# vlongle/pixie

Hardware: AMD Instinct MI355X
Metric: voxels/s (128^3 U-Net fwd) + MPM particle-steps/s (higher is better)
Workload: dtype f32 (operands split fp16 hi+lo, 3 f16 MFMAs/product, fp32 accumulate); 1 GPU; 128^3x64 feature grid -> SegmentationUNet+RegressionUNet forward (+argmax/one-hot combine), 1 scene per GPU per step; grid=128, feature_channels=64, parallelism=scene-parallel x1, executor=c+hip_graph

## Files before the change

include/pixie_hip.h:

```cpp
#ifndef PIXIE_HIP_H
#define PIXIE_HIP_H

#include <stdint.h>

#ifdef __cplusplus
extern "C" {
#endif

const char* pixie_last_error(void);
const char* pixie_build_arch(void);

typedef struct pixie_mpm pixie_mpm;

int pixie_mpm_create(pixie_mpm** out, int n_particles, int n_grid, double grid_lim);
int pixie_mpm_destroy(pixie_mpm* h);
int pixie_mpm_regrid(pixie_mpm* h, int n_grid, double grid_lim, void* stream);

int pixie_mpm_set_field(pixie_mpm* h, const char* name, const void* d_src, int64_t count, void* stream);
int pixie_mpm_get_field(pixie_mpm* h, const char* name, void* d_dst, int64_t count, void* stream);
int pixie_mpm_fill_field(pixie_mpm* h, const char* name, double value, void* stream);

int pixie_mpm_set_scalar(pixie_mpm* h, const char* key, double value);
int pixie_mpm_get_scalar(pixie_mpm* h, const char* key, double* value);

int pixie_mpm_update_mass(pixie_mpm* h, void* stream);
int pixie_mpm_finalize_mu_lam(pixie_mpm* h, int with_bulk, void* stream);
int pixie_mpm_apply_additional_params(pixie_mpm* h, const double point[3], const double size[3], double E,
                                      double nu, double density, int material, void* stream);
int pixie_mpm_apply_additional_params_batch(pixie_mpm* h, int64_t n_boxes, const float* d_boxes, const float* d_params,
                                            const int32_t* d_material, void* stream);

enum { PIXIE_BC_SURFACE = 0, PIXIE_BC_CUBOID = 1, PIXIE_BC_BBOX = 2 };
typedef struct pixie_bc_desc {
    int32_t type;
    int32_t surface_type;
    int32_t reset;
    int32_t pad_;
    double point[3], size[3], velocity[3], normal[3];
    double start_time, end_time, friction;
} pixie_bc_desc;
int pixie_mpm_add_bc(pixie_mpm* h, const pixie_bc_desc* bc);

enum { PIXIE_PM_IMPULSE = 0, PIXIE_PM_TRANSLATION = 1, PIXIE_PM_ROTATION = 2 };
typedef struct pixie_pmod_desc {
    int32_t type;
    int32_t pad_;
    double point[3], size[3];
    double force[3];
    double velocity[3];
    double normal[3], h1[3], h2[3];
    double half_height, radius, rotation_scale, translation_scale;
    double start_time, end_time;
} pixie_pmod_desc;
int pixie_mpm_add_particle_modifier(pixie_mpm* h, const pixie_pmod_desc* pm, void* stream);

int pixie_mpm_step(pixie_mpm* h, double dt, int n_substeps, void* stream);

typedef struct pixie_mpm_batch pixie_mpm_batch;
typedef struct pixie_batch_sched {
    double dt;
    int32_t steps_per_chunk;
    int32_t n_chunks;
    int32_t n_out;
    int32_t pad_;
    double shift[3], scale, mean[3];
    double inv_rotation[9];
    float* d_pos;
    float* d_cov;
} pixie_batch_sched;
int pixie_mpm_batch_create(pixie_mpm_batch** out, pixie_mpm* const* handles, int n_handles);
int pixie_mpm_batch_step(pixie_mpm_batch* b, double dt, int n_substeps, void* stream);
int pixie_mpm_batch_run(pixie_mpm_batch* b, const pixie_batch_sched* per_scene, int n_scenes, void* stream);
typedef struct pixie_batch_splat_out {
    float* d_log_scale;
    float* d_quat;
} pixie_batch_splat_out;
int pixie_mpm_batch_run_splats(pixie_mpm_batch* b, const pixie_batch_sched* per_scene, const pixie_batch_splat_out* splats ,
                               int n_scenes, void* stream);
int pixie_mpm_batch_destroy(pixie_mpm_batch* b);

int pixie_mpm_export_cov(pixie_mpm* h, float* d_cov , void* stream);
int pixie_mpm_export_R(pixie_mpm* h, float* d_R , void* stream);
int pixie_mpm_export_frame(pixie_mpm* h, int n_out, const double shift[3], double scale, const double mean[3],
                           const double inv_rotation[9], float* d_pos , float* d_cov ,
                           void* stream);
int pixie_splat_from_cov(const float* d_cov , int64_t n, float* d_log_scale , float* d_quat ,
                         void* stream);
int pixie_mpm_export_frame_splats(pixie_mpm* h, int n_out, const double shift[3], double scale, const double mean[3],
                                  const double inv_rotation[9], float* d_pos , float* d_cov ,
                                  float* d_log_scale , float* d_quat , void* stream);
int pixie_mpm_out_of_bounds(pixie_mpm* h, int64_t* count, void* stream);


typedef struct pixie_conv_desc {
    const float* d_in0; int32_t c0;
    const float* d_in1; int32_t c1;
    int32_t in_d, in_h, in_w;
    int32_t upsample;
    int32_t stride;
    int32_t ksize;
    const float* d_pro_a; const float* d_pro_b;
    const float* d_gamma; const float* d_beta;
    int32_t act;
    const float* d_w; const float* d_bias;
    int32_t c_out;
    const float* d_residual;
    float* d_out;
    const void* d_w16;
    const uint32_t* d_in_amax0; const uint32_t* d_in_amax1;
    float in_bound;
    float* d_out_stats;
    uint32_t* d_out_amax;
    void* d_workspace;
    int32_t out_d, out_h, out_w;
    const float* d_skip_in0; int32_t skip_c0;
    const float* d_skip_in1; int32_t skip_c1;
    const void* d_skip_w16; const float* d_skip_bias;
    const uint32_t* d_skip_amax0; const uint32_t* d_skip_amax1;
} pixie_conv_desc;

int pixie_conv_cout_padded(int c_out);
int pixie_conv_pack_weights(const float* d_w_oidhw, float* d_w_packed, int c_out, int c_in, int ksize, void* stream);
int64_t pixie_conv_packed16_bytes(int c_out, int c_in, int ksize);
int pixie_conv_pack_weights_f16x2(const float* d_w_oidhw, void* d_packed, int c_out, int c_in, int ksize, void* stream);
int pixie_conv3d_forward(const pixie_conv_desc* desc, void* stream);
int64_t pixie_conv_stats_floats(const pixie_conv_desc* desc);
int64_t pixie_conv_workspace_bytes(const pixie_conv_desc* desc);
int pixie_stats_finalize(const float* d_stats, const pixie_conv_desc* desc, double* d_sums, void* stream);
int pixie_conv_skip_foldable(const pixie_conv_desc* desc);

int pixie_channel_sums(const float* d_x, int channels, int64_t spatial, double* d_sums, void* stream);
int pixie_channel_stats(const float* d_x, int channels, int64_t spatial, double* d_sums, uint32_t* d_amax, void* stream);
int pixie_tensor_amax(const float* d_x, int64_t count, uint32_t* d_slot, void* stream);
int pixie_norm_finalize(const double* d_sums, int channels, int64_t spatial, int mode, int groups, double eps,
                        const float* d_weight, const float* d_bias, float* d_a, float* d_b, void* stream);

int pixie_attention_forward(const float* d_qkv, float* d_out, int channels, int tokens, void* stream);

int pixie_channel_affine(const float* d_x, const float* d_a, const float* d_b, float* d_y, int channels,
                         int64_t spatial, void* stream);

int pixie_voxel_grid_to_ncdhw(const void* d_feat_dhwc_f16, int d, int h, int w, int channels, float* d_out_cdhw, void* stream);

int pixie_projector_conv0(const void* d_feat_dhwc_f16, int64_t voxels, int channels, int n_networks, const void* const* d_w16,
                          const float* const* d_bias, float* const* d_out, int c_out, void* stream);

int pixie_pack_fields(const float* d_cont, const int32_t* d_seg_pred, int64_t n_scenes, int64_t spatial, void* d_wire, int64_t wire_bytes,
                      void* stream);

int pixie_combine_predictions(const float* d_logits, int num_classes, const float* d_cont, int64_t spatial,
                              float* d_combined, int32_t* d_argmax , void* stream);

int pixie_combine_class_ids(const int32_t* d_seg_pred, int num_classes, const float* d_cont, int64_t spatial, float* d_combined,
                            void* stream);

typedef struct pixie_unet pixie_unet;
typedef struct pixie_unet_config {
    int32_t feature_channels, cond_dim, model_channels, num_res_blocks;
    int32_t n_channel_mult; int32_t channel_mult[8];
    int32_t n_attention_resolutions; int32_t attention_resolutions[8];
    int32_t grid_size;
    int32_t out_channels;
    int32_t precision;
} pixie_unet_config;

int pixie_unet_create(pixie_unet** out, const pixie_unet_config* cfg);
int pixie_unet_destroy(pixie_unet* h);
int pixie_unet_param_count(const pixie_unet* h);
int pixie_unet_param_info(const pixie_unet* h, int index, const char** key, int64_t* numel, int32_t* ndim, int64_t shape[5]);
int pixie_unet_set_param(pixie_unet* h, const char* key, const float* d_values, int64_t numel);
int64_t pixie_unet_workspace_bytes(pixie_unet* h, int d, int hh, int w);
int pixie_unet_forward(pixie_unet* h, const float* d_feat, const float* d_proj0, int d, int hh, int w, float* d_out,
                       void* d_workspace, int64_t workspace_bytes, void* stream);
int pixie_unet_set_option(pixie_unet* h, const char* key, int value);

typedef struct pixie_field_desc {
    const float* d_pred;
    const uint8_t* d_mask;
    const float* d_axis_x; const float* d_axis_y; const float* d_axis_z;
    int32_t n_classes, d, h, w;
    double min_spacing;
    double density_min, density_max, E_min, E_max, nu_min, nu_max;
} pixie_field_desc;
int pixie_field_to_particles(const pixie_field_desc* field, const float* d_pos, int n, int k, double nn_distance_threshold,
                             int weighted, int default_material, int default_part_label, float* d_density, float* d_E,
                             float* d_nu, int32_t* d_material, int32_t* d_part_label, float* d_conf, float* d_nearest,
                             void* d_scratch, void* stream);

int pixie_unscale_prediction(const float* d_pred, int channels, int64_t spatial, double density_min, double density_max,
                             double E_min, double E_max, double nu_min, double nu_max, float* d_out, void* stream);
int64_t pixie_field_points_scratch_bytes(const pixie_field_desc* field);
int pixie_field_points(const pixie_field_desc* field, int64_t capacity, float* d_xyz , float* d_density, float* d_E,
                       float* d_nu, int32_t* d_material, float* d_conf, int64_t* d_count, void* d_scratch, void* stream);

int pixie_dbscan_roots(const float* d_pos_sorted, const int32_t* d_orig_index, const int32_t* d_cell_start, int n, int nx, int ny, int nz,
                       const double lo[3], double cell_size, double eps, int min_samples, int32_t* d_core_scratch,
                       int32_t* d_parent_scratch, int32_t* d_root, void* stream);

int pixie_fill_densify(const float* d_pos, const float* d_opacity, const float* d_cov6, int n, int grid_n, double grid_dx,
                       int32_t* d_grid_count, float* d_grid_density, void* stream);
int pixie_fill_dense_cells(int32_t* d_grid_count, const float* d_grid_density, int grid_n, double grid_dx, double density_thres,
                           int max_particles_per_cell, float* d_new_particles , int64_t max_samples,
                           uint64_t* d_counter, uint32_t seed, void* stream);
int pixie_fill_internal_cells(int32_t* d_grid_count, const float* d_grid_density, int grid_n, double grid_dx, int max_particles_per_cell,
                              int exclude_dir, int ray_cast_dir, double threshold, float* d_new_particles, int64_t max_samples,
                              uint64_t* d_counter, uint32_t seed, void* stream);
int pixie_particle_volume(const float* d_pos, int n, int grid_n, double grid_dx, int32_t* d_grid_count_scratch, float* d_vol, void* stream);
int pixie_nearest_particle(const float* d_pos, int n, const float* d_new_pos, int n_new, int32_t* d_nearest, void* stream);

#ifdef PIXIE_DIAG
int pixie_mpm_phase(pixie_mpm* h, int phase, double dt, void* stream);

int pixie_mpm_kernel_times(pixie_mpm* h, double* particle_ms, double* grid_ms, int64_t* n_launches);

int pixie_conv_kernel_variant(const pixie_conv_desc* desc, int* slices);
#endif

#ifdef __cplusplus
}
#endif
#endif
```

pixie_amd/_lib.py:

```python
from __future__ import annotations

import ctypes as C
import os

_HERE = os.path.dirname(os.path.abspath(__file__))
LIB_PATH = os.path.join(_HERE, "libpixie_hip.so")
DIAG_LIB_PATH = os.path.join(_HERE, "libpixie_hip_diag.so")


class PixieHipError(RuntimeError):
    pass


class BCDesc(C.Structure):
    _fields_ = [("type", C.c_int32), ("surface_type", C.c_int32), ("reset", C.c_int32), ("pad_", C.c_int32),
                ("point", C.c_double * 3), ("size", C.c_double * 3), ("velocity", C.c_double * 3),
                ("normal", C.c_double * 3), ("start_time", C.c_double), ("end_time", C.c_double),
                ("friction", C.c_double)]


class PModDesc(C.Structure):
    _fields_ = [("type", C.c_int32), ("pad_", C.c_int32),
                ("point", C.c_double * 3), ("size", C.c_double * 3), ("force", C.c_double * 3),
                ("velocity", C.c_double * 3), ("normal", C.c_double * 3), ("h1", C.c_double * 3),
                ("h2", C.c_double * 3), ("half_height", C.c_double), ("radius", C.c_double),
                ("rotation_scale", C.c_double), ("translation_scale", C.c_double),
                ("start_time", C.c_double), ("end_time", C.c_double)]


class ConvDesc(C.Structure):
    _fields_ = [("d_in0", C.c_void_p), ("c0", C.c_int32),
                ("d_in1", C.c_void_p), ("c1", C.c_int32),
                ("in_d", C.c_int32), ("in_h", C.c_int32), ("in_w", C.c_int32),
                ("upsample", C.c_int32), ("stride", C.c_int32), ("ksize", C.c_int32),
                ("d_pro_a", C.c_void_p), ("d_pro_b", C.c_void_p),
                ("d_gamma", C.c_void_p), ("d_beta", C.c_void_p),
                ("act", C.c_int32),
                ("d_w", C.c_void_p), ("d_bias", C.c_void_p),
                ("c_out", C.c_int32),
                ("d_residual", C.c_void_p), ("d_out", C.c_void_p),
                ("d_w16", C.c_void_p), ("d_in_amax0", C.c_void_p), ("d_in_amax1", C.c_void_p),
                ("in_bound", C.c_float),
                ("d_out_stats", C.c_void_p), ("d_out_amax", C.c_void_p),
                ("d_workspace", C.c_void_p),
                ("out_d", C.c_int32), ("out_h", C.c_int32), ("out_w", C.c_int32),
                ("d_skip_in0", C.c_void_p), ("skip_c0", C.c_int32),
                ("d_skip_in1", C.c_void_p), ("skip_c1", C.c_int32),
                ("d_skip_w16", C.c_void_p), ("d_skip_bias", C.c_void_p),
                ("d_skip_amax0", C.c_void_p), ("d_skip_amax1", C.c_void_p)]


class UNetConfigC(C.Structure):
    _fields_ = [("feature_channels", C.c_int32), ("cond_dim", C.c_int32), ("model_channels", C.c_int32), ("num_res_blocks", C.c_int32),
                ("n_channel_mult", C.c_int32), ("channel_mult", C.c_int32 * 8),
                ("n_attention_resolutions", C.c_int32), ("attention_resolutions", C.c_int32 * 8),
                ("grid_size", C.c_int32), ("out_channels", C.c_int32), ("precision", C.c_int32)]


class BatchSched(C.Structure):
    _fields_ = [("dt", C.c_double), ("steps_per_chunk", C.c_int32), ("n_chunks", C.c_int32), ("n_out", C.c_int32), ("pad_", C.c_int32),
                ("shift", C.c_double * 3), ("scale", C.c_double), ("mean", C.c_double * 3), ("inv_rotation", C.c_double * 9),
                ("d_pos", C.c_void_p), ("d_cov", C.c_void_p)]


class BatchSplatOut(C.Structure):
    _fields_ = [("d_log_scale", C.c_void_p), ("d_quat", C.c_void_p)]


class FieldDesc(C.Structure):
    _fields_ = [("d_pred", C.c_void_p), ("d_mask", C.c_void_p),
                ("d_axis_x", C.c_void_p), ("d_axis_y", C.c_void_p), ("d_axis_z", C.c_void_p),
                ("n_classes", C.c_int32), ("d", C.c_int32), ("h", C.c_int32), ("w", C.c_int32),
                ("min_spacing", C.c_double),
                ("density_min", C.c_double), ("density_max", C.c_double), ("E_min", C.c_double), ("E_max", C.c_double),
                ("nu_min", C.c_double), ("nu_max", C.c_double)]


_VP, _I, _I64, _D, _S = C.c_void_p, C.c_int, C.c_int64, C.c_double, C.c_char_p
_D3 = C.POINTER(C.c_double)
SIGNATURES = {
    "pixie_last_error": (C.c_char_p, []),
    "pixie_build_arch": (C.c_char_p, []),
    "pixie_mpm_create": (_I, [C.POINTER(_VP), _I, _I, _D]),
    "pixie_mpm_destroy": (_I, [_VP]),
    "pixie_mpm_regrid": (_I, [_VP, _I, _D, _VP]),
    "pixie_mpm_set_field": (_I, [_VP, _S, _VP, _I64, _VP]),
    "pixie_mpm_get_field": (_I, [_VP, _S, _VP, _I64, _VP]),
    "pixie_mpm_fill_field": (_I, [_VP, _S, _D, _VP]),
    "pixie_mpm_set_scalar": (_I, [_VP, _S, _D]),
    "pixie_mpm_get_scalar": (_I, [_VP, _S, C.POINTER(_D)]),
    "pixie_mpm_update_mass": (_I, [_VP, _VP]),
    "pixie_mpm_finalize_mu_lam": (_I, [_VP, _I, _VP]),
    "pixie_mpm_apply_additional_params": (_I, [_VP, _D3, _D3, _D, _D, _D, _I, _VP]),
    "pixie_mpm_apply_additional_params_batch": (_I, [_VP, _I64, _VP, _VP, _VP, _VP]),
    "pixie_mpm_add_bc": (_I, [_VP, C.POINTER(BCDesc)]),
    "pixie_mpm_add_particle_modifier": (_I, [_VP, C.POINTER(PModDesc), _VP]),
    "pixie_mpm_step": (_I, [_VP, _D, _I, _VP]),
    "pixie_mpm_export_cov": (_I, [_VP, _VP, _VP]),
    "pixie_mpm_export_R": (_I, [_VP, _VP, _VP]),
    "pixie_mpm_export_frame": (_I, [_VP, _I, _D3, _D, _D3, C.POINTER(C.c_double), _VP, _VP, _VP]),
    "pixie_mpm_out_of_bounds": (_I, [_VP, C.POINTER(_I64), _VP]),
    "pixie_mpm_batch_create": (_I, [C.POINTER(_VP), C.POINTER(_VP), _I]),
    "pixie_mpm_batch_step": (_I, [_VP, _D, _I, _VP]),
    "pixie_mpm_batch_run": (_I, [_VP, C.POINTER(BatchSched), _I, _VP]),
    "pixie_mpm_batch_run_splats": (_I, [_VP, C.POINTER(BatchSched), C.POINTER(BatchSplatOut), _I, _VP]),
    "pixie_splat_from_cov": (_I, [_VP, _I64, _VP, _VP, _VP]),
    "pixie_mpm_export_frame_splats": (_I, [_VP, _I, _D3, _D, _D3, C.POINTER(C.c_double), _VP, _VP, _VP, _VP, _VP]),
    "pixie_mpm_batch_destroy": (_I, [_VP]),
    "pixie_pack_fields": (_I, [_VP, _VP, _I64, _I64, _VP, _I64, _VP]),
    "pixie_conv_cout_padded": (_I, [_I]),
    "pixie_conv_pack_weights": (_I, [_VP, _VP, _I, _I, _I, _VP]),
    "pixie_conv_packed16_bytes": (_I64, [_I, _I, _I]),
    "pixie_conv_pack_weights_f16x2": (_I, [_VP, _VP, _I, _I, _I, _VP]),
    "pixie_conv3d_forward": (_I, [C.POINTER(ConvDesc), _VP]),
    "pixie_conv_stats_floats": (_I64, [C.POINTER(ConvDesc)]),
    "pixie_conv_workspace_bytes": (_I64, [C.POINTER(ConvDesc)]),
    "pixie_stats_finalize": (_I, [_VP, C.POINTER(ConvDesc), _VP, _VP]),
    "pixie_channel_stats": (_I, [_VP, _I, _I64, _VP, _VP, _VP]),
    "pixie_tensor_amax": (_I, [_VP, _I64, _VP, _VP]),
    "pixie_channel_sums": (_I, [_VP, _I, _I64, _VP, _VP]),
    "pixie_norm_finalize": (_I, [_VP, _I, _I64, _I, _I, _D, _VP, _VP, _VP, _VP, _VP]),
    "pixie_attention_forward": (_I, [_VP, _VP, _I, _I, _VP]),
    "pixie_channel_affine": (_I, [_VP, _VP, _VP, _VP, _I, _I64, _VP]),
    "pixie_projector_conv0": (_I, [_VP, _I64, _I, _I, C.POINTER(_VP), C.POINTER(_VP), C.POINTER(_VP), _I, _VP]),
    "pixie_conv_skip_foldable": (_I, [C.POINTER(ConvDesc)]),
    "pixie_unet_create": (_I, [C.POINTER(_VP), C.POINTER(UNetConfigC)]),
    "pixie_unet_destroy": (_I, [_VP]),
    "pixie_unet_param_count": (_I, [_VP]),
    "pixie_unet_param_info": (_I, [_VP, _I, C.POINTER(_S), C.POINTER(_I64), C.POINTER(C.c_int32), C.POINTER(_I64)]),
    "pixie_unet_set_param": (_I, [_VP, _S, _VP, _I64]),
    "pixie_unet_workspace_bytes": (_I64, [_VP, _I, _I, _I]),
    "pixie_unet_set_option": (_I, [_VP, _S, _I]),
    "pixie_unet_forward": (_I, [_VP, _VP, _VP, _I, _I, _I, _VP, _VP, _I64, _VP]),
    "pixie_combine_class_ids": (_I, [_VP, _I, _VP, _I64, _VP, _VP]),
    "pixie_combine_predictions": (_I, [_VP, _I, _VP, _I64, _VP, _VP, _VP]),
    "pixie_voxel_grid_to_ncdhw": (_I, [_VP, _I, _I, _I, _I, _VP, _VP]),
    "pixie_unscale_prediction": (_I, [_VP, _I, _I64, _D, _D, _D, _D, _D, _D, _VP, _VP]),
    "pixie_field_points_scratch_bytes": (_I64, [C.POINTER(FieldDesc)]),
    "pixie_field_points": (_I, [C.POINTER(FieldDesc), _I64, _VP, _VP, _VP, _VP, _VP, _VP, _VP, _VP, _VP]),
    "pixie_fill_densify": (_I, [_VP, _VP, _VP, _I, _I, _D, _VP, _VP, _VP]),
    "pixie_fill_dense_cells": (_I, [_VP, _VP, _I, _D, _D, _I, _VP, _I64, _VP, C.c_uint32, _VP]),
    "pixie_fill_internal_cells": (_I, [_VP, _VP, _I, _D, _I, _I, _I, _D, _VP, _I64, _VP, C.c_uint32, _VP]),
    "pixie_particle_volume": (_I, [_VP, _I, _I, _D, _VP, _VP, _VP]),
    "pixie_nearest_particle": (_I, [_VP, _I, _VP, _I, _VP, _VP]),
    "pixie_dbscan_roots": (_I, [_VP, _VP, _VP, _I, _I, _I, _I, C.POINTER(_D), _D, _D, _I, _VP, _VP, _VP, _VP]),
    "pixie_field_to_particles": (_I, [C.POINTER(FieldDesc), _VP, _I, _I, _D, _I, _I, _I, _VP, _VP, _VP, _VP, _VP, _VP, _VP, _VP, _VP]),
}

DIAG_SIGNATURES = {
    "pixie_mpm_phase": (_I, [_VP, _I, _D, _VP]),
    "pixie_mpm_kernel_times": (_I, [_VP, C.POINTER(_D), C.POINTER(_D), C.POINTER(_I64)]),
    "pixie_conv_kernel_variant": (C.c_int, [C.POINTER(ConvDesc), C.POINTER(C.c_int)]),
}

_libs = {}


def load(diag: bool = False):
    if diag in _libs:
        return _libs[diag]
    path = DIAG_LIB_PATH if diag else LIB_PATH
    if not os.path.exists(path):
        raise PixieHipError(
            f"{path} not found: build it with `python -m pixie_amd.build` (hipcc, gfx950). "
            "pixie_amd has no CPU fallback.")
    import torch
    lib = C.CDLL(path)
    for name, (res, args) in list(SIGNATURES.items()) + (list(DIAG_SIGNATURES.items()) if diag else []):
        fn = getattr(lib, name)
        fn.restype = res
        fn.argtypes = args
    _libs[diag] = lib
    return lib


def check(rc: int, what: str = "", lib=None):
    if rc != 0:
        msg = (lib or load()).pixie_last_error()
        raise PixieHipError(f"{what}: {msg.decode() if msg else 'unknown error'}")


def current_stream_ptr():
    import torch
    try:
        return C.c_void_p(torch._C._cuda_getCurrentRawStream(torch.cuda.current_device()))
    except AttributeError:
        return C.c_void_p(torch.cuda.current_stream().cuda_stream)


def d3(v):
    return (C.c_double * 3)(*[float(x) for x in v])
```

pixie_amd/csrc/conv3d_f16x3.hip:

```cpp
#include <hip/hip_runtime.h>

#include <cstdlib>
#include <map>
#include <string>
#include <type_traits>

#include "../../include/pixie_hip.h"
#include "common.h"

namespace pixie {

typedef float f32x16 __attribute__((ext_vector_type(16)));
typedef _Float16 f16x8 __attribute__((ext_vector_type(8)));

constexpr int kW16HeaderU4 = 4;

struct Conv16Args {
    const float* in0; const float* in1;
    int c0, cin;
    int ID, IH, IW;
    int LD, LH, LW;
    int ups;
    int stride;
    int OD, OH, OW;
    const float* pro_a; const float* pro_b; const float* gamma; const float* beta;
    int act;
    const uint4* w16;
    const float* wf;
    const float* bias;
    int cout, coutp;
    const float* residual; float* out;
    const unsigned* amax0; const unsigned* amax1;
    float in_bound;
    int TX, TY, TZ, lTX, lTY;
    int tiles_x, tiles_y, tiles_z, n_tiles;
    int HX, HY, HZ, HYX, CS;
    unsigned mHX, mHYX;
    float* stats; unsigned* out_amax;
    float* partial; int chunks_per_slice;
    int epi_lds;
    const float* sk_in0; const float* sk_in1;
    int sk_c0, sk_cin;
    const uint4* sk_w16; const float* sk_bias;
    const unsigned* sk_amax0; const unsigned* sk_amax1;
};

__device__ __forceinline__ int fast_div16(int n, int d, unsigned magic) {
    return (d == 1) ? n : (int)__umulhi((unsigned)n, magic);
}
__device__ __forceinline__ float act16(float t, int act) {
    if (act == 1) return t > 0.0f ? t : 0.02f * t;
    if (act == 2) return t / (1.0f + __expf(-t));
    return t;
}
__device__ __forceinline__ int scale_exponent(float bound) {
    const unsigned bits = __float_as_uint(bound);
    const int eb = (int)((bits >> 23) & 0xffu) - 127;
    if (!(bound > 0.0f) || eb > 100) return 0;
    int e = 14 - eb;
    return e > 100 ? 100 : (e < -100 ? -100 : e);
}
__device__ __forceinline__ float pow2i(int e) { return __uint_as_float((unsigned)(e + 127) << 23); }

template <int KS, int MB, int NB, bool EX = false>
__device__ __forceinline__ void conv3d_f16x3_body(const Conv16Args& A) {
    extern __shared__ uint4 smem16[];
    constexpr int PAD = (KS == 3) ? 1 : 0;
    constexpr int NW = 4, NT = 64 * NW;
    const int bufsz = 4 * A.CS;

    const int tid = threadIdx.x;
    const int lane = tid & 63;
    const int wave = tid >> 6;
    const int kh = lane >> 5;
    const int l31 = lane & 31;

    int t = blockIdx.x;
    {
        const int per = (A.n_tiles + 7) >> 3;
        const int cand = (t & 7) * per + (t >> 3);
        if ((A.n_tiles & 7) == 0) t = cand;
    }
    const int tx = t % A.tiles_x; t /= A.tiles_x;
    const int ty = t % A.tiles_y;
    const int tz = t / A.tiles_y;
    const int ox0 = tx * A.TX, oy0 = ty * A.TY, oz0 = tz * A.TZ;
    const int cout0 = blockIdx.y * (MB * 32);
    const int lx0 = ox0 * A.stride - PAD, ly0 = oy0 * A.stride - PAD, lz0 = oz0 * A.stride - PAD;
    const size_t ISP = (size_t)A.ID * A.IH * A.IW;
    const size_t OSP = (size_t)A.OD * A.OH * A.OW;

    int voff[NB];
    int ovox[NB];
    bool valid[NB];
#pragma unroll
    for (int nb = 0; nb < NB; ++nb) {
        const int j = (wave * NB + nb) * 32 + l31;
        int x = j & (A.TX - 1);
        int y = (j >> A.lTX) & (A.TY - 1);
        int z = j >> (A.lTX + A.lTY);
        const bool v = (z < A.TZ) && (ox0 + x < A.OW) && (oy0 + y < A.OH) && (oz0 + z < A.OD);
        if (!v) { x = 0; y = 0; z = 0; }
        voff[nb] = ((z * A.HY + y) * A.HX + x) * A.stride + kh * A.CS;
        ovox[nb] = ((oz0 + z) * A.OH + (oy0 + y)) * A.OW + ox0 + x;
        valid[nb] = v;
    }

    float bound = A.in_bound;
    if (A.amax0) {
        bound = __uint_as_float(*A.amax0);
        if (A.amax1) bound = fmaxf(bound, __uint_as_float(*A.amax1));
    }
    const int ex = EX ? 0 : scale_exponent(bound);
    const float sx = pow2i(ex);

    f32x16 acc[MB][NB];
#pragma unroll
    for (int mb = 0; mb < MB; ++mb)
#pragma unroll
        for (int nb = 0; nb < NB; ++nb)
#pragma unroll
            for (int r = 0; r < 16; ++r) acc[mb][nb][r] = 0.0f;

    const int KG = A.cin >> 3;
    const size_t tap_stride = (size_t)KG * A.coutp;
    const size_t plane = (size_t)(KS * KS * KS) * tap_stride;
    const uint4* wHi = A.w16 + kW16HeaderU4 + (size_t)kh * A.coutp + cout0 + l31;
    const uint4* wLo = wHi + plane;
    const float* wF = A.wf + (size_t)kh * A.coutp + cout0 + l31;

    constexpr int TAPS = KS * KS * KS;
    auto stage_chunk = [&](int c_base, uint4* buf, int stid, int nthr) {
        uint4* bHi = buf;
        uint4* bLo = buf + 2 * A.CS;
        float pa[16], pb[16];
        {
            float pv = 0.0f;
            if (A.pro_a) pv = (lane & 16) ? A.pro_b[c_base + (lane & 15)] : A.pro_a[c_base + (lane & 15)];
#pragma unroll
            for (int j = 0; j < 16; ++j) {
                pa[j] = __int_as_float(__builtin_amdgcn_readlane(__float_as_int(pv), j));
                pb[j] = __int_as_float(__builtin_amdgcn_readlane(__float_as_int(pv), 16 + j));
            }
        }
        const bool has_aff = A.gamma != nullptr;
        for (int v0 = stid; v0 < A.CS; v0 += 2 * nthr) {
            float val[2][16];
            float gm[2], bt[2];
            int sidx[2];
            bool ok[2];
#pragma unroll
            for (int u = 0; u < 2; ++u) {
                const int vox = v0 + u * nthr;
                int rem = vox;
                const int hz = fast_div16(rem, A.HYX, A.mHYX);
                rem -= hz * A.HYX;
                const int hy = fast_div16(rem, A.HX, A.mHX);
                const int hx = rem - hy * A.HX;
                const int lz = lz0 + hz, ly = ly0 + hy, lx = lx0 + hx;
                ok[u] = vox < A.CS && (unsigned)lz < (unsigned)A.LD && (unsigned)ly < (unsigned)A.LH && (unsigned)lx < (unsigned)A.LW;
                sidx[u] = ok[u] ? ((lz >> A.ups) * A.IH + (ly >> A.ups)) * A.IW + (lx >> A.ups) : 0;
            }
#pragma unroll
            for (int u = 0; u < 2; ++u) {
#pragma unroll
                for (int j = 0; j < 16; ++j) {
                    const int cg = c_base + j;
                    const float* src = (cg < A.c0) ? (A.in0 + (size_t)cg * ISP) : (A.in1 + (size_t)(cg - A.c0) * ISP);
                    val[u][j] = src[sidx[u]];
                }
                gm[u] = 1.0f; bt[u] = 0.0f;
                if (has_aff) { gm[u] = A.gamma[sidx[u]]; bt[u] = A.beta[sidx[u]]; }
            }
            auto convert = [&](auto has_pro, auto act_c) {
#pragma unroll
                for (int u = 0; u < 2; ++u) {
                    const int vox = v0 + u * nthr;
                    if (EX) {
                        float* bF = reinterpret_cast<float*>(buf);
#pragma unroll
                        for (int j = 0; j < 16; ++j) {
                            float t = val[u][j];
                            if (decltype(has_pro)::value) t = t * pa[j] + pb[j];
                            t = t * gm[u] + bt[u];
                            const float sc = ok[u] ? act16(t, decltype(act_c)::value) : 0.0f;
                            if (vox < A.CS) bF[j * A.CS + vox] = sc;
                        }
                        continue;
                    }
                    f16x8 vh[2], vl[2];
#pragma unroll
                    for (int j = 0; j < 16; ++j) {
                        float t = val[u][j];
                        if (decltype(has_pro)::value) t = t * pa[j] + pb[j];
                        t = t * gm[u] + bt[u];
                        const float sc = ok[u] ? act16(t, decltype(act_c)::value) * sx : 0.0f;
                        const _Float16 h = (_Float16)sc;
                        vh[j >> 3][j & 7] = h;
                        vl[j >> 3][j & 7] = (_Float16)(sc - (float)h);
                    }
                    if (vox < A.CS) {
                        bHi[vox] = __builtin_bit_cast(uint4, vh[0]);
                        bHi[A.CS + vox] = __builtin_bit_cast(uint4, vh[1]);
                        bLo[vox] = __builtin_bit_cast(uint4, vl[0]);
                        bLo[A.CS + vox] = __builtin_bit_cast(uint4, vl[1]);
                    }
                }
            };
            using T = std::true_type; using F = std::false_type;
            if (A.pro_a) {
                if (A.act == 1) convert(T{}, std::integral_constant<int, 1>{});
                else if (A.act == 2) convert(T{}, std::integral_constant<int, 2>{});
                else convert(T{}, std::integral_constant<int, 0>{});
            } else {
                if (A.act == 1) convert(F{}, std::integral_constant<int, 1>{});
                else if (A.act == 2) convert(F{}, std::integral_constant<int, 2>{});
                else convert(F{}, std::integral_constant<int, 0>{});
            }
        }
    };
    auto mfma_chunk = [&](int c_base, const uint4* buf) {
        __builtin_amdgcn_s_setprio(3);
        if constexpr (EX) {
            const float* ldsF = reinterpret_cast<const float*>(buf);
            const size_t tapw = (size_t)A.cin * A.coutp;
            const float* wc = wF + (size_t)c_base * A.coutp;
            float a[8][MB], an[8][MB];
#pragma unroll
            for (int kp = 0; kp < 8; ++kp)
#pragma unroll
                for (int mb = 0; mb < MB; ++mb) a[kp][mb] = wc[(size_t)(2 * kp) * A.coutp + mb * 32];
#pragma unroll 1
            for (int zy = 0; zy < KS * KS; ++zy) {
                const int dz = zy / KS, dy = zy - dz * KS;
                const int rowoff = (dz * A.HY + dy) * A.HX;
#pragma unroll
                for (int dx = 0; dx < KS; ++dx) {
                    const int tap = zy * KS + dx;
                    const int nxt = (tap + 1 < TAPS) ? tap + 1 : tap;
#pragma unroll
                    for (int kp = 0; kp < 8; ++kp)
#pragma unroll
                        for (int mb = 0; mb < MB; ++mb) an[kp][mb] = wc[(size_t)nxt * tapw + (size_t)(2 * kp) * A.coutp + mb * 32];
                    __builtin_amdgcn_sched_barrier(0);
#pragma unroll
                    for (int kp = 0; kp < 8; ++kp) {
                        float b[NB];
#pragma unroll
                        for (int nb = 0; nb < NB; ++nb) b[nb] = ldsF[voff[nb] + rowoff + dx + 2 * kp * A.CS];
#pragma unroll
                        for (int mb = 0; mb < MB; ++mb)
#pragma unroll
                            for (int nb = 0; nb < NB; ++nb)
                                acc[mb][nb] = __builtin_amdgcn_mfma_f32_32x32x2f32(a[kp][mb], b[nb], acc[mb][nb], 0, 0, 0);
                    }
#pragma unroll
                    for (int kp = 0; kp < 8; ++kp)
#pragma unroll
                        for (int mb = 0; mb < MB; ++mb) a[kp][mb] = an[kp][mb];
                }
            }
            __builtin_amdgcn_s_setprio(0);
            return;
        }
        const uint4* ldsHi = buf;
        const uint4* ldsLo = buf + 2 * A.CS;
        const uint4* wh = wHi + (size_t)(c_base >> 3) * A.coutp;
        const uint4* wl = wLo + (size_t)(c_base >> 3) * A.coutp;
        f16x8 ah[MB], al[MB];
#pragma unroll
        for (int mb = 0; mb < MB; ++mb) {
            ah[mb] = __builtin_bit_cast(f16x8, wh[mb * 32]);
            al[mb] = __builtin_bit_cast(f16x8, wl[mb * 32]);
        }
#pragma unroll 1
        for (int zy = 0; zy < KS * KS; ++zy) {
            const int dz = zy / KS, dy = zy - dz * KS;
            const int rowoff = (dz * A.HY + dy) * A.HX;
#pragma unroll
            for (int dx = 0; dx < KS; ++dx) {
                const int tap = zy * KS + dx;
                const int nxt = (tap + 1 < TAPS) ? tap + 1 : tap;
                f16x8 ahn[MB], aln[MB];
#pragma unroll
                for (int mb = 0; mb < MB; ++mb) {
                    ahn[mb] = __builtin_bit_cast(f16x8, wh[(size_t)nxt * tap_stride + mb * 32]);
                    aln[mb] = __builtin_bit_cast(f16x8, wl[(size_t)nxt * tap_stride + mb * 32]);
                }
                __builtin_amdgcn_sched_barrier(0);
                f16x8 bh[NB], bl[NB];
#pragma unroll
                for (int nb = 0; nb < NB; ++nb) {
                    bh[nb] = __builtin_bit_cast(f16x8, ldsHi[voff[nb] + rowoff + dx]);
                    bl[nb] = __builtin_bit_cast(f16x8, ldsLo[voff[nb] + rowoff + dx]);
                }
#pragma unroll
                for (int mb = 0; mb < MB; ++mb)
#pragma unroll
                    for (int nb = 0; nb < NB; ++nb)
                        acc[mb][nb] = __builtin_amdgcn_mfma_f32_32x32x16_f16(al[mb], bh[nb], acc[mb][nb], 0, 0, 0);
#pragma unroll
                for (int mb = 0; mb < MB; ++mb)
#pragma unroll
                    for (int nb = 0; nb < NB; ++nb)
                        acc[mb][nb] = __builtin_amdgcn_mfma_f32_32x32x16_f16(ah[mb], bl[nb], acc[mb][nb], 0, 0, 0);
#pragma unroll
                for (int mb = 0; mb < MB; ++mb)
#pragma unroll
                    for (int nb = 0; nb < NB; ++nb)
                        acc[mb][nb] = __builtin_amdgcn_mfma_f32_32x32x16_f16(ah[mb], bh[nb], acc[mb][nb], 0, 0, 0);
#pragma unroll
                for (int mb = 0; mb < MB; ++mb) { ah[mb] = ahn[mb]; al[mb] = aln[mb]; }
            }
        }
        __builtin_amdgcn_s_setprio(0);
    };

    float inv2 = 0.0f;
    {
        const int c_begin = A.partial ? (int)blockIdx.z * A.chunks_per_slice * 16 : 0;
        const int c_end = A.partial ? min(A.cin, c_begin + A.chunks_per_slice * 16) : A.cin;
        for (int c_base = c_begin; c_base < c_end; c_base += 16) {
            __syncthreads();
            stage_chunk(c_base, smem16, tid, NT);
            __syncthreads();
            mfma_chunk(c_base, smem16);
        }
        if (!EX && A.sk_w16) {
            float sb = __uint_as_float(*A.sk_amax0);
            if (A.sk_amax1) sb = fmaxf(sb, __uint_as_float(*A.sk_amax1));
            const int ex2 = scale_exponent(sb);
            const float sx2 = pow2i(ex2);
            const float inv_main = __uint_as_float(A.w16[0].x) * pow2i(-ex);
            inv2 = __uint_as_float(A.sk_w16[0].x) * pow2i(-ex2);
            const float ratio = inv_main / inv2;
#pragma unroll
            for (int mb = 0; mb < MB; ++mb)
#pragma unroll
                for (int nb = 0; nb < NB; ++nb)
#pragma unroll
                    for (int r = 0; r < 16; ++r) acc[mb][nb][r] *= ratio;
            const int KG2 = A.sk_cin >> 3;
            const uint4* w2Hi = A.sk_w16 + kW16HeaderU4 + (size_t)kh * A.coutp + cout0 + l31;
            const uint4* w2Lo = w2Hi + (size_t)KG2 * A.coutp;
            const int centre = (KS == 3) ? (A.HY + 1) * A.HX + 1 : 0;
            const int tvox = A.TX * A.TY * A.TZ;
            for (int c2 = 0; c2 < A.sk_cin; c2 += 16) {
                f16x8 ah[MB], al[MB];
#pragma unroll
                for (int mb = 0; mb < MB; ++mb) {
                    ah[mb] = __builtin_bit_cast(f16x8, w2Hi[(size_t)(c2 >> 3) * A.coutp + mb * 32]);
                    al[mb] = __builtin_bit_cast(f16x8, w2Lo[(size_t)(c2 >> 3) * A.coutp + mb * 32]);
                }
                __syncthreads();
                uint4* bHi = smem16;
                uint4* bLo = smem16 + 2 * A.CS;
                for (int j = tid; j < tvox; j += NT) {
                    const int x = j & (A.TX - 1), y = (j >> A.lTX) & (A.TY - 1), z = j >> (A.lTX + A.lTY);
                    const bool okv = (ox0 + x < A.OW) && (oy0 + y < A.OH) && (oz0 + z < A.OD);
                    const size_t sidx = okv ? ((size_t)(oz0 + z) * A.IH + (oy0 + y)) * A.IW + ox0 + x : 0;
                    float val[16];
#pragma unroll
                    for (int q = 0; q < 16; ++q) {
                        const int cg = c2 + q;
                        const float* src = (cg < A.sk_c0) ? (A.sk_in0 + (size_t)cg * ISP) : (A.sk_in1 + (size_t)(cg - A.sk_c0) * ISP);
                        val[q] = src[sidx];
                    }
                    f16x8 vh[2], vl[2];
#pragma unroll
                    for (int q = 0; q < 16; ++q) {
                        const float sc = okv ? val[q] * sx2 : 0.0f;
                        const _Float16 hq = (_Float16)sc;
                        vh[q >> 3][q & 7] = hq;
                        vl[q >> 3][q & 7] = (_Float16)(sc - (float)hq);
                    }
                    const int slot = (z * A.HY + y) * A.HX + x + centre;
                    bHi[slot] = __builtin_bit_cast(uint4, vh[0]);
                    bHi[A.CS + slot] = __builtin_bit_cast(uint4, vh[1]);
                    bLo[slot] = __builtin_bit_cast(uint4, vl[0]);
                    bLo[A.CS + slot] = __builtin_bit_cast(uint4, vl[1]);
                }
                __syncthreads();
                f16x8 bh[NB], bl[NB];
#pragma unroll
                for (int nb = 0; nb < NB; ++nb) {
                    bh[nb] = __builtin_bit_cast(f16x8, bHi[voff[nb] + centre]);
                    bl[nb] = __builtin_bit_cast(f16x8, bLo[voff[nb] + centre]);
                }
#pragma unroll
                for (int mb = 0; mb < MB; ++mb)
#pragma unroll
                    for (int nb = 0; nb < NB; ++nb)
                        acc[mb][nb] = __builtin_amdgcn_mfma_f32_32x32x16_f16(al[mb], bh[nb], acc[mb][nb], 0, 0, 0);
#pragma unroll
                for (int mb = 0; mb < MB; ++mb)
#pragma unroll
                    for (int nb = 0; nb < NB; ++nb)
                        acc[mb][nb] = __builtin_amdgcn_mfma_f32_32x32x16_f16(ah[mb], bl[nb], acc[mb][nb], 0, 0, 0);
#pragma unroll
                for (int mb = 0; mb < MB; ++mb)
#pragma unroll
                    for (int nb = 0; nb < NB; ++nb)
                        acc[mb][nb] = __builtin_amdgcn_mfma_f32_32x32x16_f16(ah[mb], bh[nb], acc[mb][nb], 0, 0, 0);
            }
        }
    }

    const float inv = EX ? 1.0f : (A.sk_w16 ? inv2 : __uint_as_float(A.w16[0].x) * pow2i(-ex));
    if (A.partial) {
        float* dst = A.partial + (size_t)blockIdx.z * A.cout * OSP;
#pragma unroll
        for (int mb = 0; mb < MB; ++mb)
#pragma unroll
            for (int r = 0; r < 16; ++r) {
                const int co = cout0 + mb * 32 + (r & 3) + 8 * (r >> 2) + 4 * kh;
                if (co < A.cout) {
#pragma unroll
                    for (int nb = 0; nb < NB; ++nb)
                        if (valid[nb]) dst[(size_t)co * OSP + ovox[nb]] = acc[mb][nb][r] * inv;
                }
            }
        return;
    }
    float* red = reinterpret_cast<float*>(smem16);
    float wmax = 0.0f;
    const bool full = A.epi_lds && cout0 + MB * 32 <= A.cout && (A.TX & 3) == 0 && (A.OW & 3) == 0 && NW * NB * 32 <= A.TX * A.TY * A.TZ &&
                      ox0 + A.TX <= A.OW && oy0 + A.TY <= A.OH && oz0 + A.TZ <= A.OD;
    if (full) {
        __syncthreads();
        constexpr int LDO = NB * 32 + 4;
        float* ldsO = reinterpret_cast<float*>(smem16) + wave * (32 * LDO);
        red = reinterpret_cast<float*>(smem16) + NW * 32 * LDO;
        constexpr int LPR = NB * 8;
        constexpr int RPI = 32 / LPR;
        const int rsub = l31 / LPR, colq = 4 * (l31 % LPR), nbq = colq >> 5;
        const int jq = (wave * NB + nbq) * 32 + (colq & 31);
        const int xq = jq & (A.TX - 1), yq = (jq >> A.lTX) & (A.TY - 1), zq = jq >> (A.lTX + A.lTY);
        const size_t ovq = ((size_t)(oz0 + zq) * A.OH + (oy0 + yq)) * A.OW + ox0 + xq;
        const bool has_res = A.residual != nullptr, has_stats = A.stats != nullptr;
#pragma unroll
        for (int mb = 0; mb < MB; ++mb) {
#pragma unroll
            for (int r = 0; r < 16; ++r)
#pragma unroll
                for (int nb = 0; nb < NB; ++nb) ldsO[((r & 3) + 8 * (r >> 2) + 4 * kh) * LDO + nb * 32 + l31] = acc[mb][nb][r];
#pragma unroll 4
            for (int it = 0; it < 16 / RPI; ++it) {
                const int rowl = (2 * it + kh) * RPI + rsub;
                const int co = cout0 + mb * 32 + rowl;
                const float4 a4 = *reinterpret_cast<const float4*>(ldsO + rowl * LDO + colq);
                const float bv = (A.bias ? A.bias[co] : 0.0f) + (A.sk_bias ? A.sk_bias[co] : 0.0f);
                const size_t o = (size_t)co * OSP + ovq;
                float4 v4;
                v4.x = a4.x * inv + bv; v4.y = a4.y * inv + bv; v4.z = a4.z * inv + bv; v4.w = a4.w * inv + bv;
                if (has_res) {
                    const float4 r4 = *reinterpret_cast<const float4*>(A.residual + o);
                    v4.x += r4.x; v4.y += r4.y; v4.z += r4.z; v4.w += r4.w;
                }
                *reinterpret_cast<float4*>(A.out + o) = v4;
                if (has_stats) {
                    float s1 = (v4.x + v4.y) + (v4.z + v4.w);
                    float s2 = (v4.x * v4.x + v4.y * v4.y) + (v4.z * v4.z + v4.w * v4.w);
                    wmax = fmaxf(fmaxf(wmax, fmaxf(fabsf(v4.x), fabsf(v4.y))), fmaxf(fabsf(v4.z), fabsf(v4.w)));
#pragma unroll
                    for (int off = LPR / 2; off > 0; off >>= 1) { s1 += __shfl_xor(s1, off, 64); s2 += __shfl_xor(s2, off, 64); }
                    if ((l31 % LPR) == 0) { red[(wave * MB * 32 + mb * 32 + rowl) * 2] = s1; red[(wave * MB * 32 + mb * 32 + rowl) * 2 + 1] = s2; }
                }
            }
        }
    } else {
    if (A.stats) __syncthreads();
#pragma unroll
    for (int mb = 0; mb < MB; ++mb) {
#pragma unroll
        for (int r = 0; r < 16; ++r) {
            const int row = mb * 32 + (r & 3) + 8 * (r >> 2) + 4 * kh;
            const int co = cout0 + row;
            float s1 = 0.0f, s2 = 0.0f;
            if (co < A.cout) {
                const float bv = (A.bias ? A.bias[co] : 0.0f) + (A.sk_bias ? A.sk_bias[co] : 0.0f);
#pragma unroll
                for (int nb = 0; nb < NB; ++nb) {
                    if (valid[nb]) {
                        const size_t o = (size_t)co * OSP + ovox[nb];
                        float val = acc[mb][nb][r] * inv + bv;
                        if (A.residual) val += A.residual[o];
                        A.out[o] = val;
                        s1 += val; s2 += val * val; wmax = fmaxf(wmax, fabsf(val));
                    }
                }
            }
            if (A.stats) {
#pragma unroll
                for (int off = 16; off > 0; off >>= 1) { s1 += __shfl_xor(s1, off, 64); s2 += __shfl_xor(s2, off, 64); }
                if (l31 == 0) { red[(wave * MB * 32 + row) * 2] = s1; red[(wave * MB * 32 + row) * 2 + 1] = s2; }
            }
        }
    }
    }
    if (A.stats) {
        __syncthreads();
        if (tid < MB * 32 * 2) {
            float t = red[tid];
#pragma unroll
            for (int w = 1; w < NW; ++w) t += red[w * MB * 64 + tid];
            A.stats[((size_t)blockIdx.x * A.coutp + cout0) * 2 + tid] = t;
        }
        if (A.out_amax) {
#pragma unroll
            for (int off = 32; off > 0; off >>= 1) wmax = fmaxf(wmax, __shfl_xor(wmax, off, 64));
            if (lane == 0 && wmax > 0.0f) atomicMax(A.out_amax, __float_as_uint(wmax));
        }
    }
}

template <int KS, int MB, int NB>
__global__ __launch_bounds__(256, 2) void conv3d_f16x3_kernel(Conv16Args A) {
    conv3d_f16x3_body<KS, MB, NB>(A);
}
template <int KS, int MB, int NB>
__global__ __launch_bounds__(256, 2) void conv3d_exact_kernel(Conv16Args A) {
    conv3d_f16x3_body<KS, MB, NB, true>(A);
}
__global__ __launch_bounds__(256, 2) void conv3d_f16x3_c64_fullres_kernel(Conv16Args A) {
    conv3d_f16x3_body<3, 2, 4>(A);
}

__global__ __launch_bounds__(256) void stats_finalize_kernel(const float* __restrict__ stats, int n_tiles, int coutp, double* __restrict__ sums) {
    const int c = blockIdx.x;
    double s1 = 0.0, s2 = 0.0;
    for (int t = threadIdx.x; t < n_tiles; t += 256) {
        const float2 v = *reinterpret_cast<const float2*>(stats + ((size_t)t * coutp + c) * 2);
        s1 += v.x; s2 += v.y;
    }
    for (int off = 32; off > 0; off >>= 1) { s1 += __shfl_down(s1, off, 64); s2 += __shfl_down(s2, off, 64); }
    __shared__ double r[8];
    if ((threadIdx.x & 63) == 0) { r[2 * (threadIdx.x >> 6)] = s1; r[2 * (threadIdx.x >> 6) + 1] = s2; }
    __syncthreads();
    if (threadIdx.x == 0) { sums[2 * c] = r[0] + r[2] + r[4] + r[6]; sums[2 * c + 1] = r[1] + r[3] + r[5] + r[7]; }
}

__global__ __launch_bounds__(256) void splitk_reduce_kernel(const float* __restrict__ partial, int slices, long n_elems, long osp,
                                                            const float* __restrict__ bias, const float* residual, float* out) {
    const long i = (long)blockIdx.x * 256 + threadIdx.x;
    if (i >= n_elems) return;
    float v = partial[i];
    for (int s = 1; s < slices; ++s) v += partial[(size_t)s * n_elems + i];
    if (bias) v += bias[i / osp];
    if (residual) v += residual[i];
    out[i] = v;
}

__global__ __launch_bounds__(256) void amax_kernel(const float* __restrict__ x, long n, unsigned* __restrict__ slot) {
    float m = 0.0f;
    const long stride = (long)gridDim.x * 256 * 4;
    long i = ((long)blockIdx.x * 256 + threadIdx.x) * 4;
    if ((reinterpret_cast<size_t>(x) & 15) == 0) {
        for (; i + 3 < n; i += stride) {
            const float4 v = *reinterpret_cast<const float4*>(x + i);
            m = fmaxf(fmaxf(m, fabsf(v.x)), fmaxf(fabsf(v.y), fmaxf(fabsf(v.z), fabsf(v.w))));
        }
        for (long k = i; k < n && k < i + 4; ++k) m = fmaxf(m, fabsf(x[k]));
    } else {
        for (long k = (long)blockIdx.x * 256 + threadIdx.x; k < n; k += (long)gridDim.x * 256) m = fmaxf(m, fabsf(x[k]));
    }
    for (int off = 32; off > 0; off >>= 1) m = fmaxf(m, __shfl_down(m, off, 64));
    if ((threadIdx.x & 63) == 0 && m > 0.0f) atomicMax(slot, __float_as_uint(m));
}

__global__ void pack_weights_f16x2_kernel(const float* __restrict__ src, uint4* __restrict__ dst, int cout, int cin, int taps,
                                          int coutp, const unsigned* __restrict__ amax_bits) {
    const int KG = cin >> 3;
    const long total = (long)taps * KG * coutp;
    const long i = (long)blockIdx.x * blockDim.x + threadIdx.x;
    const int e = scale_exponent(__uint_as_float(*amax_bits));
    if (i == 0) dst[0] = make_uint4(__float_as_uint(pow2i(-e)), (unsigned)cout, (unsigned)cin, (unsigned)taps);
    if (i >= total) return;
    const float s = pow2i(e);
    const int co = (int)(i % coutp);
    const long row = i / coutp;
    const int kg = (int)(row % KG);
    const int tap = (int)(row / KG);
    f16x8 vh, vl;
#pragma unroll
    for (int j = 0; j < 8; ++j) {
        float w = 0.0f;
        if (co < cout) w = src[((long)co * cin + kg * 8 + j) * taps + tap] * s;
        const _Float16 h = (_Float16)w;
        vh[j] = h;
        vl[j] = (_Float16)(w - (float)h);
    }
    dst[kW16HeaderU4 + i] = __builtin_bit_cast(uint4, vh);
    dst[kW16HeaderU4 + total + i] = __builtin_bit_cast(uint4, vl);
}

static unsigned magic_of16(int d) { return d <= 1 ? 0u : (unsigned)((0x100000000ull + (unsigned long long)d - 1) / (unsigned long long)d); }
static int ilog2_16(int v) { int l = 0; while ((1 << l) < v) ++l; return l; }
static int pow2_le16(int v, int cap) { int p = 1; while (p * 2 <= v && p * 2 <= cap) p *= 2; return p; }

template <int KS, int MB, int NB>
static int launch_f16x3(const Conv16Args& a, size_t lds_bytes, dim3 grid, hipStream_t st) {
    auto kern = conv3d_f16x3_kernel<KS, MB, NB>;
    PX_CHECK_HIP(allow_max_dynamic_lds(reinterpret_cast<const void*>(kern)));
    hipLaunchKernelGGL(kern, grid, dim3(256), lds_bytes, st, a);
    PX_CHECK_HIP(hipGetLastError());
    return 0;
}

static void conv16_tiling(const pixie_conv_desc* d, Conv16Args& a, int& MB_out, int& NB_out, int* slices_out = nullptr) {
    a.ID = d->in_d; a.IH = d->in_h; a.IW = d->in_w;
    a.ups = d->upsample;
    a.LD = a.ID << a.ups; a.LH = a.IH << a.ups; a.LW = a.IW << a.ups;
    const int pad = d->ksize == 3 ? 1 : 0;
    a.stride = d->stride;
    a.OD = (a.LD + 2 * pad - d->ksize) / a.stride + 1; a.OH = (a.LH + 2 * pad - d->ksize) / a.stride + 1; a.OW = (a.LW + 2 * pad - d->ksize) / a.stride + 1;
    if (d->out_d > 0) a.OD = std::min(a.OD, (int)d->out_d);
    if (d->out_h > 0) a.OH = std::min(a.OH, (int)d->out_h);
    if (d->out_w > 0) a.OW = std::min(a.OW, (int)d->out_w);
    a.cout = d->c_out; a.coutp = pixie_conv_cout_padded(d->c_out);
    const long ovol = (long)a.OD * a.OH * a.OW;
    int MB = (a.coutp >= 64) ? 2 : 1;
    int NB = (a.stride == 2) ? 1 : 4;
    auto n_wg = [&](int mb, int nb) {
        const long tiles = (ovol + 128L * nb - 1) / (128L * nb);
        return tiles * ((a.coutp + mb * 32 - 1) / (mb * 32));
    };
    int slices = 1;
    const int chunks = (d->c0 + d->c1) / 16;
    const int smax = d->d_workspace ? std::min(8, chunks / 2) : 1;
    if (smax >= 2 && n_wg(MB, NB) < 512) {
        bool found = false;
        for (int nb = NB; nb >= 1 && !found; nb /= 2) {
            for (int sl = 1; sl <= smax; sl *= 2)
                if (n_wg(MB, nb) * sl >= 512) { NB = nb; slices = sl; found = true; break; }
        }
        if (!found) { NB = 1; slices = 1; while (slices * 2 <= smax) slices *= 2; }
    } else {
        while (n_wg(MB, NB) < 512 && NB > 1) NB /= 2;
        if (n_wg(MB, NB) < 512 && MB > 1) MB = 1;
    }
    if (slices_out) *slices_out = slices;
    const int tile_vox = 128 * NB;
    a.TX = pow2_le16(a.OW, 32);
    a.TY = pow2_le16(a.OH, std::max(1, std::min(4, tile_vox / a.TX)));
    a.TZ = std::max(1, std::min(a.OD, tile_vox / (a.TX * a.TY)));
    a.lTX = ilog2_16(a.TX); a.lTY = ilog2_16(a.TY);
    a.tiles_x = (a.OW + a.TX - 1) / a.TX; a.tiles_y = (a.OH + a.TY - 1) / a.TY; a.tiles_z = (a.OD + a.TZ - 1) / a.TZ;
    a.n_tiles = a.tiles_x * a.tiles_y * a.tiles_z;
    a.HX = (a.TX - 1) * a.stride + d->ksize; a.HY = (a.TY - 1) * a.stride + d->ksize; a.HZ = (a.TZ - 1) * a.stride + d->ksize;
    a.HYX = a.HY * a.HX; a.CS = a.HZ * a.HYX;
    a.mHX = magic_of16(a.HX); a.mHYX = magic_of16(a.HYX);

    MB_out = MB; NB_out = NB;
}

int conv3d_f16x3_forward(const pixie_conv_desc* d, hipStream_t st) {
    PX_REQUIRE(d->stride == 1 || (d->stride == 2 && d->ksize == 3 && !d->upsample), "f16x3 conv: stride must be 1, or 2 for a 3^3 kernel");
    const int cin = d->c0 + d->c1;
    PX_REQUIRE(cin % 16 == 0 && d->c0 % 8 == 0, "f16x3 conv: c_in must be a multiple of 16 (got %d+%d)", d->c0, d->c1);
    PX_REQUIRE(d->d_in_amax0 != nullptr || d->in_bound > 0.0f, "f16x3 conv: needs d_in_amax0 or a positive in_bound");
    PX_REQUIRE(d->c1 == 0 || d->d_in_amax0 == nullptr || d->d_in_amax1 != nullptr, "f16x3 conv: second input needs its own amax slot");
    Conv16Args a{};
    a.in0 = d->d_in0; a.in1 = d->d_in1; a.c0 = d->c0; a.cin = cin;
    a.ID = d->in_d; a.IH = d->in_h; a.IW = d->in_w;
    a.ups = d->upsample;
    a.LD = a.ID << a.ups; a.LH = a.IH << a.ups; a.LW = a.IW << a.ups;
    const int pad = d->ksize == 3 ? 1 : 0;
    a.stride = d->stride;
    a.OD = (a.LD + 2 * pad - d->ksize) / a.stride + 1; a.OH = (a.LH + 2 * pad - d->ksize) / a.stride + 1; a.OW = (a.LW + 2 * pad - d->ksize) / a.stride + 1;
    if (d->out_d > 0) a.OD = std::min(a.OD, (int)d->out_d);
    if (d->out_h > 0) a.OH = std::min(a.OH, (int)d->out_h);
    if (d->out_w > 0) a.OW = std::min(a.OW, (int)d->out_w);
    a.pro_a = d->d_pro_a; a.pro_b = d->d_pro_b; a.gamma = d->d_gamma; a.beta = d->d_beta; a.act = d->act;
    a.w16 = reinterpret_cast<const uint4*>(d->d_w16); a.bias = d->d_bias; a.cout = d->c_out; a.coutp = pixie_conv_cout_padded(d->c_out);
    a.residual = d->d_residual; a.out = d->d_out;
    a.amax0 = d->d_in_amax0; a.amax1 = (d->c1 > 0) ? d->d_in_amax1 : nullptr; a.in_bound = d->in_bound;
    a.stats = d->d_out_stats; a.out_amax = d->d_out_amax;

    int MB = 0, NB = 0, slices = 1;
    conv16_tiling(d, a, MB, NB, &slices);
    if (d->d_skip_w16) {
        const int scin = d->skip_c0 + d->skip_c1;
        PX_REQUIRE(pixie_conv_skip_foldable(d), "f16x3 conv: this launch cannot fold a skip convolution (pixie_conv_skip_foldable)");
        PX_REQUIRE(d->d_skip_in0 && d->d_skip_amax0 && (d->skip_c1 == 0 || (d->d_skip_in1 && d->d_skip_amax1)), "f16x3 conv: folded skip needs its inputs and their amax slots");
        a.sk_in0 = d->d_skip_in0; a.sk_in1 = d->d_skip_in1; a.sk_c0 = d->skip_c0; a.sk_cin = scin;
        a.sk_w16 = reinterpret_cast<const uint4*>(d->d_skip_w16); a.sk_bias = d->d_skip_bias;
        a.sk_amax0 = d->d_skip_amax0; a.sk_amax1 = d->skip_c1 > 0 ? d->d_skip_amax1 : nullptr;
    }
    if (slices > 1) {
        a.partial = static_cast<float*>(d->d_workspace);
        a.chunks_per_slice = (cin / 16 + slices - 1) / slices;
        a.stats = nullptr; a.out_amax = nullptr;
    }

    size_t lds = (size_t)4 * a.CS * sizeof(uint4);
    PX_REQUIRE(lds <= 160 * 1024, "f16x3 conv: tile needs %zu B of LDS", lds);
    {
        const size_t epi = ((size_t)4 * 32 * (NB * 32 + 4) + (size_t)4 * MB * 32 * 2) * sizeof(float);
        if (slices == 1 && epi <= 80 * 1024) { a.epi_lds = 1; if (lds < epi) lds = epi; }
    }
    const dim3 grid((unsigned)a.n_tiles, (unsigned)((a.coutp + MB * 32 - 1) / (MB * 32)), (unsigned)slices);
    if (slices > 1) {
        int rc = 1;
#define PX_CONV16_SK(KS_, MB_, NB_) \
        if (d->ksize == KS_ && MB == MB_ && NB == NB_) rc = launch_f16x3<KS_, MB_, NB_>(a, lds, grid, st);
        PX_CONV16_SK(3, 2, 4) PX_CONV16_SK(3, 2, 2) PX_CONV16_SK(3, 2, 1) PX_CONV16_SK(3, 1, 4) PX_CONV16_SK(3, 1, 2) PX_CONV16_SK(3, 1, 1)
        PX_CONV16_SK(1, 2, 4) PX_CONV16_SK(1, 2, 2) PX_CONV16_SK(1, 2, 1) PX_CONV16_SK(1, 1, 4) PX_CONV16_SK(1, 1, 2) PX_CONV16_SK(1, 1, 1)
#undef PX_CONV16_SK
        if (rc) return rc;
        const long osp = (long)a.OD * a.OH * a.OW, n_elems = (long)a.cout * osp;
        hipLaunchKernelGGL(splitk_reduce_kernel, dim3((unsigned)((n_elems + 255) / 256)), dim3(256), 0, st, a.partial, slices, n_elems, osp,
                           a.bias, a.residual, a.out);
        PX_CHECK_HIP(hipGetLastError());
        return 0;
    }
    if (d->ksize == 3 && MB == 2 && NB == 4 && cin == 64 && d->c_out == 64 && d->stride == 1 && !d->upsample && d->c1 == 0 && !a.sk_w16 &&
        (long)a.OD * a.OH * a.OW >= 128L * 128 * 128) {
        auto kern = conv3d_f16x3_c64_fullres_kernel;
        PX_CHECK_HIP(allow_max_dynamic_lds(reinterpret_cast<const void*>(kern)));
        hipLaunchKernelGGL(kern, grid, dim3(256), lds, st, a);
        PX_CHECK_HIP(hipGetLastError());
        return 0;
    }
#define PX_CONV16_CASE(KS_, MB_, NB_) \
    if (d->ksize == KS_ && MB == MB_ && NB == NB_) return launch_f16x3<KS_, MB_, NB_>(a, lds, grid, st);
    PX_CONV16_CASE(3, 2, 4) PX_CONV16_CASE(3, 2, 2) PX_CONV16_CASE(3, 2, 1)
    PX_CONV16_CASE(3, 1, 4) PX_CONV16_CASE(3, 1, 2) PX_CONV16_CASE(3, 1, 1)
    PX_CONV16_CASE(1, 2, 4) PX_CONV16_CASE(1, 2, 2) PX_CONV16_CASE(1, 2, 1)
    PX_CONV16_CASE(1, 1, 4) PX_CONV16_CASE(1, 1, 2) PX_CONV16_CASE(1, 1, 1)
#undef PX_CONV16_CASE
    return set_error("f16x3 conv: no kernel variant for ksize=%d MB=%d NB=%d", d->ksize, MB, NB);
}

template <int KS, int MB, int NB>
static int launch_exact(const Conv16Args& a, size_t lds_bytes, dim3 grid, hipStream_t st) {
    auto kern = conv3d_exact_kernel<KS, MB, NB>;
    PX_CHECK_HIP(allow_max_dynamic_lds(reinterpret_cast<const void*>(kern)));
    hipLaunchKernelGGL(kern, grid, dim3(256), lds_bytes, st, a);
    PX_CHECK_HIP(hipGetLastError());
    return 0;
}

bool conv3d_exact_tiled_ok(const pixie_conv_desc* d) {
    const int cin = d->c0 + d->c1;
    return cin % 16 == 0 && (d->stride == 1 || (d->stride == 2 && d->ksize == 3 && !d->upsample)) && getenv("PIXIE_CONV_EXACT_V1") == nullptr;
}

int conv3d_exact_forward(const pixie_conv_desc* d, hipStream_t st) {
    Conv16Args a{};
    a.in0 = d->d_in0; a.in1 = d->d_in1; a.c0 = d->c0; a.cin = d->c0 + d->c1;
    a.pro_a = d->d_pro_a; a.pro_b = d->d_pro_b; a.gamma = d->d_gamma; a.beta = d->d_beta; a.act = d->act;
    a.wf = d->d_w; a.bias = d->d_bias;
    a.residual = d->d_residual; a.out = d->d_out;
    a.in_bound = 1.0f;
    pixie_conv_desc probe = *d;
    probe.d_workspace = nullptr;
    int MB = 0, NB = 0, slices = 1;
    conv16_tiling(&probe, a, MB, NB, &slices);
    size_t lds = (size_t)4 * a.CS * sizeof(uint4);
    PX_REQUIRE(lds <= 160 * 1024, "exact conv: tile needs %zu B of LDS", lds);
    {
        const size_t epi = ((size_t)4 * 32 * (NB * 32 + 4) + (size_t)4 * MB * 32 * 2) * sizeof(float);
        if (epi <= 80 * 1024) { a.epi_lds = 1; if (lds < epi) lds = epi; }
    }
    const dim3 grid((unsigned)a.n_tiles, (unsigned)((a.coutp + MB * 32 - 1) / (MB * 32)), 1u);
#define PX_CONVEX_CASE(KS_, MB_, NB_) \
    if (d->ksize == KS_ && MB == MB_ && NB == NB_) return launch_exact<KS_, MB_, NB_>(a, lds, grid, st);
    PX_CONVEX_CASE(3, 2, 4) PX_CONVEX_CASE(3, 2, 2) PX_CONVEX_CASE(3, 2, 1)
    PX_CONVEX_CASE(3, 1, 4) PX_CONVEX_CASE(3, 1, 2) PX_CONVEX_CASE(3, 1, 1)
    PX_CONVEX_CASE(1, 2, 4) PX_CONVEX_CASE(1, 2, 2) PX_CONVEX_CASE(1, 2, 1)
    PX_CONVEX_CASE(1, 1, 4) PX_CONVEX_CASE(1, 1, 2) PX_CONVEX_CASE(1, 1, 1)
#undef PX_CONVEX_CASE
    return set_error("exact conv: no kernel variant for ksize=%d MB=%d NB=%d", d->ksize, MB, NB);
}

}

using namespace pixie;

extern "C" int64_t pixie_conv_stats_floats(const pixie_conv_desc* d) {
    if (!d || !d->d_w16 || !(d->stride == 1 || (d->stride == 2 && d->ksize == 3)) || (d->ksize != 1 && d->ksize != 3)) return 0;
    Conv16Args a{};
    int MB = 0, NB = 0, slices = 1;
    conv16_tiling(d, a, MB, NB, &slices);
    return slices > 1 ? 0 : (int64_t)a.n_tiles * a.coutp * 2;
}

extern "C" int64_t pixie_conv_workspace_bytes(const pixie_conv_desc* d) {
    if (!d || !d->d_w16 || !(d->stride == 1 || (d->stride == 2 && d->ksize == 3)) || (d->ksize != 1 && d->ksize != 3)) return 0;
    pixie_conv_desc probe = *d;
    probe.d_workspace = reinterpret_cast<void*>(1);
    Conv16Args a{};
    int MB = 0, NB = 0, slices = 1;
    conv16_tiling(&probe, a, MB, NB, &slices);
    return slices > 1 ? (int64_t)slices * a.cout * a.OD * a.OH * a.OW * (int64_t)sizeof(float) : 0;
}

#ifdef PIXIE_DIAG
extern "C" int pixie_conv_kernel_variant(const pixie_conv_desc* d, int* slices_out) {
    if (slices_out) *slices_out = 1;
    if (!d || !d->d_w16 || !(d->stride == 1 || (d->stride == 2 && d->ksize == 3)) || (d->ksize != 1 && d->ksize != 3)) return 0;
    Conv16Args a{};
    int MB = 0, NB = 0, slices = 1;
    conv16_tiling(d, a, MB, NB, &slices);
    if (slices_out) *slices_out = slices;
    if (d->ksize == 3 && MB == 2 && NB == 4 && d->c0 + d->c1 == 64 && d->c_out == 64 && d->stride == 1 && !d->upsample && d->c1 == 0 && !d->d_skip_w16 &&
        (long)a.OD * a.OH * a.OW >= 128L * 128 * 128)
        return 9324;
    return d->ksize * 100 + MB * 10 + NB;
}
#endif

extern "C" int pixie_conv_skip_foldable(const pixie_conv_desc* d) {
    if (!d || !d->d_w16 || d->stride != 1 || d->upsample || (d->ksize != 1 && d->ksize != 3)) return 0;
    const int scin = d->skip_c0 + d->skip_c1;
    if (scin <= 0 || scin % 16 != 0 || d->skip_c0 % 8 != 0 || (d->c0 + d->c1) % 16 != 0 || d->c0 % 8 != 0) return 0;
    Conv16Args a{};
    int MB = 0, NB = 0, slices = 1;
    conv16_tiling(d, a, MB, NB, &slices);
    return slices == 1 ? 1 : 0;
}

extern "C" int pixie_stats_finalize(const float* d_stats, const pixie_conv_desc* d, double* d_sums, void* stream) {
    PX_REQUIRE(d_stats && d && d_sums, "pixie_stats_finalize: null argument");
    Conv16Args a{};
    int MB = 0, NB = 0;
    conv16_tiling(d, a, MB, NB);
    hipLaunchKernelGGL(stats_finalize_kernel, dim3((unsigned)d->c_out), dim3(256), 0, as_stream(stream), d_stats, a.n_tiles, a.coutp, d_sums);
    PX_CHECK_HIP(hipGetLastError());
    return 0;
}

extern "C" int64_t pixie_conv_packed16_bytes(int c_out, int c_in, int ksize) {
    if (c_out <= 0 || c_in <= 0 || c_in % 8 != 0 || (ksize != 1 && ksize != 3)) return 0;
    const int64_t taps = (int64_t)ksize * ksize * ksize;
    return ((int64_t)kW16HeaderU4 + 2 * taps * (c_in / 8) * pixie_conv_cout_padded(c_out)) * (int64_t)sizeof(uint4);
}

extern "C" int pixie_tensor_amax(const float* d_x, int64_t count, uint32_t* d_slot, void* stream) {
    PX_REQUIRE(d_x && d_slot && count > 0, "pixie_tensor_amax: bad arguments");
    const int blocks = (int)std::min<int64_t>(2048, (count + 1023) / 1024);
    hipLaunchKernelGGL(amax_kernel, dim3(blocks), dim3(256), 0, as_stream(stream), d_x, (long)count, d_slot);
    PX_CHECK_HIP(hipGetLastError());
    return 0;
}

extern "C" int pixie_conv_pack_weights_f16x2(const float* d_w, void* d_packed, int c_out, int c_in, int ksize, void* stream) {
    PX_REQUIRE(d_w && d_packed && c_out > 0 && c_in > 0 && c_in % 8 == 0 && (ksize == 1 || ksize == 3),
               "pixie_conv_pack_weights_f16x2: bad arguments (c_in must be a multiple of 8)");
    hipStream_t st = as_stream(stream);
    const int taps = ksize * ksize * ksize;
    const int coutp = pixie_conv_cout_padded(c_out);
    unsigned* slot = reinterpret_cast<unsigned*>(d_packed) + 15;
    PX_CHECK_HIP(hipMemsetAsync(d_packed, 0, kW16HeaderU4 * sizeof(uint4), st));
    if (pixie_tensor_amax(d_w, (int64_t)c_out * c_in * taps, slot, stream)) return 1;
    const long total = (long)taps * (c_in / 8) * coutp;
    hipLaunchKernelGGL(pack_weights_f16x2_kernel, dim3(cdiv(total, 256)), dim3(256), 0, st, d_w, reinterpret_cast<uint4*>(d_packed), c_out,
                       c_in, taps, coutp, slot);
    PX_CHECK_HIP(hipGetLastError());
    return 0;
}
```

pixie_amd/csrc/conv3d_mfma.hip:

```cpp
#include <hip/hip_runtime.h>

#include "../../include/pixie_hip.h"
#include "common.h"

namespace pixie {

typedef float f32x16 __attribute__((ext_vector_type(16)));

struct ConvArgs {
    const float* in0; const float* in1;
    int c0, cin;
    int ID, IH, IW;
    int LD, LH, LW;
    int ups;
    int stride;
    int OD, OH, OW;
    const float* pro_a; const float* pro_b; const float* gamma; const float* beta;
    int act;
    const float* w; const float* bias;
    int cout, coutp;
    const float* residual; float* out;
    int TX, TY, TZ, lTX, lTY;
    int tiles_x, tiles_y, tiles_z;
    int HX, HY, HZ, HYX, CS;
    unsigned mHX, mHYX, mCS;
};

__device__ __forceinline__ int fast_div(int n, int d, unsigned magic) {
    return (d == 1) ? n : (int)__umulhi((unsigned)n, magic);
}

__device__ __forceinline__ float apply_act(float t, int act) {
    if (act == 1) return t > 0.0f ? t : 0.02f * t;
    if (act == 2) return t / (1.0f + __expf(-t));
    return t;
}

template <int KS, int MB, int NB, int CK>
__global__ __launch_bounds__(256, 2) void conv3d_mfma_kernel(ConvArgs A) {
    extern __shared__ __attribute__((aligned(16))) float smem[];
    constexpr int MBW = MB * 32;
    constexpr int TAPS = KS * KS * KS;
    constexpr int PAD = (KS == 3) ? 1 : 0;
    float* ldsX = smem;
    float* ldsW = smem + ((CK * A.CS + 3) & ~3);

    const int tid = threadIdx.x;
    const int lane = tid & 63;
    const int wave = tid >> 6;
    const int half = lane >> 5;
    const int l31 = lane & 31;

    int t = blockIdx.x;
    const int tx = t % A.tiles_x; t /= A.tiles_x;
    const int ty = t % A.tiles_y;
    const int tz = t / A.tiles_y;
    const int ox0 = tx * A.TX, oy0 = ty * A.TY, oz0 = tz * A.TZ;
    const int cout0 = blockIdx.y * MBW;
    const int lx0 = ox0 * A.stride - PAD, ly0 = oy0 * A.stride - PAD, lz0 = oz0 * A.stride - PAD;
    const size_t ISP = (size_t)A.ID * A.IH * A.IW;
    const size_t OSP = (size_t)A.OD * A.OH * A.OW;

    int voff[NB];
    int ovox[NB];
    bool valid[NB];
#pragma unroll
    for (int nb = 0; nb < NB; ++nb) {
        const int j = (wave * NB + nb) * 32 + l31;
        int x = j & (A.TX - 1);
        int y = (j >> A.lTX) & (A.TY - 1);
        int z = j >> (A.lTX + A.lTY);
        const bool v = (z < A.TZ) && (ox0 + x < A.OW) && (oy0 + y < A.OH) && (oz0 + z < A.OD);
        if (!v) { x = 0; y = 0; z = 0; }
        voff[nb] = ((z * A.stride) * A.HY + y * A.stride) * A.HX + x * A.stride + half * A.CS;
        ovox[nb] = ((oz0 + z) * A.OH + (oy0 + y)) * A.OW + ox0 + x;
        valid[nb] = v;
    }
    const int laneA = half * MBW + l31;

    f32x16 acc[MB][NB];
#pragma unroll
    for (int mb = 0; mb < MB; ++mb)
#pragma unroll
        for (int nb = 0; nb < NB; ++nb)
#pragma unroll
            for (int r = 0; r < 16; ++r) acc[mb][nb][r] = 0.0f;

    const int tileX = CK * A.CS;
    for (int c_base = 0; c_base < A.cin; c_base += CK) {
        __syncthreads();
        for (int idx = tid; idx < tileX; idx += 256) {
            const int c = fast_div(idx, A.CS, A.mCS);
            int rem = idx - c * A.CS;
            const int hz = fast_div(rem, A.HYX, A.mHYX);
            rem -= hz * A.HYX;
            const int hy = fast_div(rem, A.HX, A.mHX);
            const int hx = rem - hy * A.HX;
            const int lz = lz0 + hz, ly = ly0 + hy, lx = lx0 + hx;
            const int cg = c_base + c;
            float val = 0.0f;
            if (cg < A.cin && (unsigned)lz < (unsigned)A.LD && (unsigned)ly < (unsigned)A.LH && (unsigned)lx < (unsigned)A.LW) {
                const int sidx = ((lz >> A.ups) * A.IH + (ly >> A.ups)) * A.IW + (lx >> A.ups);
                const float* src = (cg < A.c0) ? (A.in0 + (size_t)cg * ISP) : (A.in1 + (size_t)(cg - A.c0) * ISP);
                val = src[sidx];
                if (A.pro_a) val = val * A.pro_a[cg] + A.pro_b[cg];
                if (A.gamma) val = val * A.gamma[sidx] + A.beta[sidx];
                val = apply_act(val, A.act);
            }
            ldsX[idx] = val;
        }
        constexpr int WE4 = TAPS * CK * MBW / 4;
        for (int i4 = tid; i4 < WE4; i4 += 256) {
            const int idx = i4 * 4;
            const int m = idx & (MBW - 1);
            const int row = idx / MBW;
            const int c = row % CK;
            const int tap = row / CK;
            const int cg = c_base + c;
            const int co = cout0 + m;
            float4 wv = make_float4(0.f, 0.f, 0.f, 0.f);
            if (cg < A.cin && co < A.coutp)
                wv = *reinterpret_cast<const float4*>(A.w + ((size_t)tap * A.cin + cg) * A.coutp + co);
            *reinterpret_cast<float4*>(ldsW + idx) = wv;
        }
        __syncthreads();
#pragma unroll 1
        for (int dz = 0; dz < KS; ++dz) {
#pragma unroll 1
            for (int dy = 0; dy < KS; ++dy) {
#pragma unroll
                for (int dx = 0; dx < KS; ++dx) {
                    const int tap = (dz * KS + dy) * KS + dx;
                    const int tapoff = (dz * A.HY + dy) * A.HX + dx;
#pragma unroll
                    for (int kp = 0; kp < CK / 2; ++kp) {
                        float a[MB], b[NB];
#pragma unroll
                        for (int mb = 0; mb < MB; ++mb) a[mb] = ldsW[(tap * CK + 2 * kp) * MBW + mb * 32 + laneA];
#pragma unroll
                        for (int nb = 0; nb < NB; ++nb) b[nb] = ldsX[voff[nb] + 2 * kp * A.CS + tapoff];
#pragma unroll
                        for (int mb = 0; mb < MB; ++mb)
#pragma unroll
                            for (int nb = 0; nb < NB; ++nb)
                                acc[mb][nb] = __builtin_amdgcn_mfma_f32_32x32x2f32(a[mb], b[nb], acc[mb][nb], 0, 0, 0);
                    }
                }
            }
        }
    }

#pragma unroll
    for (int mb = 0; mb < MB; ++mb) {
#pragma unroll
        for (int r = 0; r < 16; ++r) {
            const int co = cout0 + mb * 32 + (r & 3) + 8 * (r >> 2) + 4 * half;
            if (co < A.cout) {
                const float bv = A.bias ? A.bias[co] : 0.0f;
#pragma unroll
                for (int nb = 0; nb < NB; ++nb) {
                    if (valid[nb]) {
                        const size_t o = (size_t)co * OSP + ovox[nb];
                        float val = acc[mb][nb][r] + bv;
                        if (A.residual) val += A.residual[o];
                        A.out[o] = val;
                    }
                }
            }
        }
    }
}

__global__ void pack_weights_kernel(const float* __restrict__ src, float* __restrict__ dst, int cout, int cin, int taps, int coutp) {
    const long total = (long)taps * cin * coutp;
    const long i = (long)blockIdx.x * blockDim.x + threadIdx.x;
    if (i >= total) return;
    const int co = (int)(i % coutp);
    const long row = i / coutp;
    const int ci = (int)(row % cin);
    const int tap = (int)(row / cin);
    dst[i] = (co < cout) ? src[((long)co * cin + ci) * taps + tap] : 0.0f;
}

static unsigned magic_of(int d) { return d <= 1 ? 0u : (unsigned)((0x100000000ull + (unsigned long long)d - 1) / (unsigned long long)d); }
static int ilog2(int v) { int l = 0; while ((1 << l) < v) ++l; return l; }
static int pow2_le(int v, int cap) { int p = 1; while (p * 2 <= v && p * 2 <= cap) p *= 2; return p; }

template <int KS, int MB, int NB, int CK>
static int launch_variant(const ConvArgs& a, size_t lds_bytes, dim3 grid, hipStream_t st) {
    auto kern = conv3d_mfma_kernel<KS, MB, NB, CK>;
    PX_CHECK_HIP(allow_max_dynamic_lds(reinterpret_cast<const void*>(kern)));
    hipLaunchKernelGGL(kern, grid, dim3(256), lds_bytes, st, a);
    PX_CHECK_HIP(hipGetLastError());
    return 0;
}

}

namespace pixie {
int conv3d_f16x3_forward(const pixie_conv_desc* d, hipStream_t st);
bool conv3d_exact_tiled_ok(const pixie_conv_desc* d);
int conv3d_exact_forward(const pixie_conv_desc* d, hipStream_t st);
}
using namespace pixie;

extern "C" int pixie_conv_cout_padded(int c_out) { return (c_out + 31) / 32 * 32; }

extern "C" int pixie_conv_pack_weights(const float* d_w, float* d_packed, int c_out, int c_in, int ksize, void* stream) {
    PX_REQUIRE(d_w && d_packed && c_out > 0 && c_in > 0 && (ksize == 1 || ksize == 3), "pixie_conv_pack_weights: bad arguments");
    const int taps = ksize * ksize * ksize;
    const int coutp = pixie_conv_cout_padded(c_out);
    const long total = (long)taps * c_in * coutp;
    hipLaunchKernelGGL(pack_weights_kernel, dim3(cdiv(total, 256)), dim3(256), 0, as_stream(stream), d_w, d_packed, c_out, c_in, taps, coutp);
    PX_CHECK_HIP(hipGetLastError());
    return 0;
}

extern "C" int pixie_conv3d_forward(const pixie_conv_desc* d, void* stream) {
    PX_REQUIRE(d && d->d_in0 && (d->d_w || d->d_w16) && d->d_out, "pixie_conv3d_forward: null pointer in descriptor");
    PX_REQUIRE(d->ksize == 1 || d->ksize == 3, "pixie_conv3d_forward: ksize must be 1 or 3 (got %d)", d->ksize);
    PX_REQUIRE(d->stride == 1 || d->stride == 2, "pixie_conv3d_forward: stride must be 1 or 2 (got %d)", d->stride);
    PX_REQUIRE(d->upsample == 0 || d->upsample == 1, "pixie_conv3d_forward: upsample must be 0 or 1");
    PX_REQUIRE(d->c0 > 0 && d->c1 >= 0 && (d->c1 == 0 || d->d_in1), "pixie_conv3d_forward: bad channel split");
    PX_REQUIRE(d->c_out > 0 && d->in_d > 0 && d->in_h > 0 && d->in_w > 0, "pixie_conv3d_forward: bad sizes");
    PX_REQUIRE((d->d_pro_a == nullptr) == (d->d_pro_b == nullptr), "pixie_conv3d_forward: pro_a/pro_b must come together");
    PX_REQUIRE((d->d_gamma == nullptr) == (d->d_beta == nullptr), "pixie_conv3d_forward: gamma/beta must come together");
    PX_REQUIRE(!(d->d_gamma && d->upsample), "pixie_conv3d_forward: spatial affine with upsample is not in the reference graph");

    if (d->d_w16) return conv3d_f16x3_forward(d, as_stream(stream));
    PX_REQUIRE(!d->d_skip_w16, "pixie_conv3d_forward: a folded skip convolution needs the f16x3 path (d_w16)");
    if (conv3d_exact_tiled_ok(d)) return conv3d_exact_forward(d, as_stream(stream));

    ConvArgs a{};
    a.in0 = d->d_in0; a.in1 = d->d_in1; a.c0 = d->c0; a.cin = d->c0 + d->c1;
    a.ID = d->in_d; a.IH = d->in_h; a.IW = d->in_w;
    a.ups = d->upsample;
    a.LD = a.ID << a.ups; a.LH = a.IH << a.ups; a.LW = a.IW << a.ups;
    a.stride = d->stride;
    const int pad = d->ksize == 3 ? 1 : 0;
    a.OD = (a.LD + 2 * pad - d->ksize) / a.stride + 1;
    a.OH = (a.LH + 2 * pad - d->ksize) / a.stride + 1;
    a.OW = (a.LW + 2 * pad - d->ksize) / a.stride + 1;
    if (d->out_d > 0) a.OD = std::min(a.OD, (int)d->out_d);
    if (d->out_h > 0) a.OH = std::min(a.OH, (int)d->out_h);
    if (d->out_w > 0) a.OW = std::min(a.OW, (int)d->out_w);
    a.pro_a = d->d_pro_a; a.pro_b = d->d_pro_b; a.gamma = d->d_gamma; a.beta = d->d_beta; a.act = d->act;
    a.w = d->d_w; a.bias = d->d_bias; a.cout = d->c_out; a.coutp = pixie_conv_cout_padded(d->c_out);
    a.residual = d->d_residual; a.out = d->d_out;

    const long ovol = (long)a.OD * a.OH * a.OW;
    int MB = (a.coutp >= 64) ? 2 : 1;
    int NB = 4;
    auto n_wg = [&](int mb, int nb) {
        const long tiles = (ovol + 128L * nb - 1) / (128L * nb);
        return tiles * ((a.coutp + mb * 32 - 1) / (mb * 32));
    };
    while (n_wg(MB, NB) < 512 && NB > 1) NB /= 2;
    if (n_wg(MB, NB) < 512 && MB > 1) MB = 1;
    if (a.stride == 2 && NB > 2) NB = 2;

    const int tile_vox = 128 * NB;
    a.TX = pow2_le(a.OW, 32);
    a.TY = pow2_le(a.OH, std::max(1, tile_vox / a.TX));
    a.TZ = std::max(1, std::min(a.OD, tile_vox / (a.TX * a.TY)));
    a.lTX = ilog2(a.TX); a.lTY = ilog2(a.TY);
    a.tiles_x = (a.OW + a.TX - 1) / a.TX; a.tiles_y = (a.OH + a.TY - 1) / a.TY; a.tiles_z = (a.OD + a.TZ - 1) / a.TZ;
    a.HX = (a.TX - 1) * a.stride + d->ksize; a.HY = (a.TY - 1) * a.stride + d->ksize; a.HZ = (a.TZ - 1) * a.stride + d->ksize;
    a.HYX = a.HY * a.HX; a.CS = a.HZ * a.HYX;
    a.mHX = magic_of(a.HX); a.mHYX = magic_of(a.HYX); a.mCS = magic_of(a.CS);

    const int CK = d->ksize == 3 ? 4 : 16;
    const int taps = d->ksize * d->ksize * d->ksize;
    const size_t lds = ((size_t)((CK * a.CS + 3) & ~3) + (size_t)taps * CK * MB * 32) * sizeof(float);
    PX_REQUIRE(lds <= 160 * 1024, "pixie_conv3d_forward: tile needs %zu B of LDS", lds);
    const dim3 grid((unsigned)(a.tiles_x * a.tiles_y * a.tiles_z), (unsigned)((a.coutp + MB * 32 - 1) / (MB * 32)));
    hipStream_t st = as_stream(stream);

#define PX_CONV_CASE(KS_, MB_, NB_, CK_) \
    if (d->ksize == KS_ && MB == MB_ && NB == NB_) return launch_variant<KS_, MB_, NB_, CK_>(a, lds, grid, st);
    PX_CONV_CASE(3, 2, 4, 4) PX_CONV_CASE(3, 2, 2, 4) PX_CONV_CASE(3, 2, 1, 4)
    PX_CONV_CASE(3, 1, 4, 4) PX_CONV_CASE(3, 1, 2, 4) PX_CONV_CASE(3, 1, 1, 4)
    PX_CONV_CASE(1, 2, 4, 16) PX_CONV_CASE(1, 2, 2, 16) PX_CONV_CASE(1, 2, 1, 16)
    PX_CONV_CASE(1, 1, 4, 16) PX_CONV_CASE(1, 1, 2, 16) PX_CONV_CASE(1, 1, 1, 16)
#undef PX_CONV_CASE
    return set_error("pixie_conv3d_forward: no kernel variant for ksize=%d MB=%d NB=%d", d->ksize, MB, NB);
}
```

pixie_amd/csrc/unet_exec.hip:

```cpp
#include <hip/hip_runtime.h>

#include <algorithm>
#include <cmath>
#include <cstdlib>
#include <cstring>
#include <map>
#include <memory>
#include <stdexcept>
#include <string>
#include <tuple>
#include <unordered_map>
#include <vector>

#include "../../include/pixie_hip.h"
#include "common.h"

namespace pixie {
int channel_stats_prezeroed(const float* d_x, int channels, int64_t spatial, double* d_sums, uint32_t* d_amax, hipStream_t st);
int norm_finalize_cat(const double* d_sums0, int c0, const double* d_sums1, int c1, int64_t spatial, int mode, int groups, double eps,
                      const float* d_weight, const float* d_bias, float* d_a, float* d_b, hipStream_t st);
namespace {

enum { ACT_NONE = 0, ACT_LEAKY = 1, ACT_SILU = 2 };
enum Kind { CONV_IN, RES, DOWN, ATTN, UP };

struct Blk { Kind kind; std::string prefix; int cin, cout, sp; };
struct Plan {
    std::vector<std::vector<Blk>> in_blocks, out_blocks;
    std::vector<Blk> middle;
    int out_sp = 0;
};

struct Err : std::runtime_error { using std::runtime_error::runtime_error; };
[[noreturn]] void fail(const char* fmt, ...) {
    char buf[512];
    va_list ap; va_start(ap, fmt); vsnprintf(buf, sizeof buf, fmt, ap); va_end(ap);
    throw Err(buf);
}
void ok(int rc, const char* what) { if (rc != 0) fail("%s: %s", what, pixie_last_error()); }

bool has(const std::vector<int>& v, int x) { for (int e : v) if (e == x) return true; return false; }

struct Cfg {
    int feature_channels, cond_dim, model_channels, num_res_blocks;
    std::vector<int> mult, attn;
    int grid_size, out_channels, precision;
    bool has_projector() const { return feature_channels != cond_dim; }
    int projector_hidden() const { return feature_channels > cond_dim ? 128 : 0; }
};

Plan build_plan(const Cfg& c) {
    Plan p;
    const int mc = c.model_channels, nrb = c.num_res_blocks;
    auto name = [](const char* part, int idx, int sub) { return std::string("unet.") + part + "." + std::to_string(idx) + "." + std::to_string(sub); };
    p.in_blocks.push_back({Blk{CONV_IN, "unet.input_blocks.0.0", c.cond_dim, mc, c.grid_size}});
    std::vector<int> chans{mc}, sizes{c.grid_size};
    int ch = mc, ds = 1, sp = c.grid_size;
    for (size_t level = 0; level < c.mult.size(); ++level) {
        const int m = c.mult[level];
        for (int r = 0; r < nrb; ++r) {
            const int idx = (int)p.in_blocks.size();
            std::vector<Blk> seq{Blk{RES, name("input_blocks", idx, 0), ch, m * mc, sp}};
            ch = m * mc;
            if (has(c.attn, ds)) seq.push_back(Blk{ATTN, name("input_blocks", idx, 1), ch, ch, sp});
            p.in_blocks.push_back(seq);
            chans.push_back(ch);
        }
        if (level + 1 != c.mult.size()) {
            const int idx = (int)p.in_blocks.size();
            p.in_blocks.push_back({Blk{DOWN, name("input_blocks", idx, 0), ch, ch, sp}});
            chans.push_back(ch);
            sizes.push_back(sp);
            ds *= 2;
            sp = (sp + 1) / 2;
        }
    }
    p.middle = {Blk{RES, "unet.middle_block.0", ch, ch, sp}, Blk{ATTN, "unet.middle_block.1", ch, ch, sp}, Blk{RES, "unet.middle_block.2", ch, ch, sp}};
    for (int level = (int)c.mult.size() - 1; level >= 0; --level) {
        const int m = c.mult[level];
        for (int i = 0; i <= nrb; ++i) {
            const int idx = (int)p.out_blocks.size();
            const int ich = chans.back(); chans.pop_back();
            std::vector<Blk> seq{Blk{RES, name("output_blocks", idx, 0), ch + ich, mc * m, sp}};
            ch = mc * m;
            if (has(c.attn, ds)) seq.push_back(Blk{ATTN, name("output_blocks", idx, (int)seq.size()), ch, ch, sp});
            if (level && i == nrb) {
                seq.push_back(Blk{UP, name("output_blocks", idx, (int)seq.size()), ch, ch, sp});
                ds /= 2;
                sp = sizes.back(); sizes.pop_back();
            }
            p.out_blocks.push_back(seq);
        }
    }
    p.out_sp = sp;
    return p;
}

struct Param {
    std::string key;
    std::vector<int64_t> shape;
    int64_t numel = 1;
    bool norm = false;
    const float* d = nullptr;
    uint64_t version = 0;
};

std::vector<Param> param_table(const Cfg& c, const Plan& plan) {
    std::vector<Param> out;
    auto add = [&](const std::string& key, std::vector<int64_t> shape, bool norm) {
        Param p; p.key = key; p.shape = shape; p.norm = norm;
        for (int64_t s : shape) p.numel *= s;
        out.push_back(p);
    };
    auto conv = [&](const std::string& prefix, int cout, int cin, int k, int dims = 3) {
        std::vector<int64_t> s{cout, cin};
        for (int i = 0; i < dims; ++i) s.push_back(k);
        add(prefix + ".weight", s, false);
        add(prefix + ".bias", {cout}, false);
    };
    auto norm = [&](const std::string& prefix, std::vector<int64_t> shape) {
        add(prefix + ".weight", shape, true);
        add(prefix + ".bias", shape, true);
    };
    if (c.has_projector()) {
        const int hid = c.projector_hidden();
        if (!hid) {
            conv("projector.net.0", c.cond_dim, c.feature_channels, 1);
            norm("projector.net.1", {c.cond_dim});
        } else {
            conv("projector.net.0", hid, c.feature_channels, 1);
            norm("projector.net.1", {hid});
            conv("projector.net.3", hid, hid, 3);
            norm("projector.net.4", {hid});
            conv("projector.net.6", c.cond_dim, hid, 1);
            norm("projector.net.7", {c.cond_dim});
        }
    }
    auto emit = [&](const Blk& b) {
        const std::vector<int64_t> vol{b.sp, b.sp, b.sp};
        switch (b.kind) {
            case CONV_IN: conv(b.prefix, b.cout, b.cin, 3); break;
            case RES:
                norm(b.prefix + ".in_layers.0", vol);
                conv(b.prefix + ".in_layers.2", b.cout, b.cin, 3);
                norm(b.prefix + ".out_layers.0", vol);
                conv(b.prefix + ".out_layers.3", b.cout, b.cout, 3);
                if (b.cin != b.cout) conv(b.prefix + ".skip_connection", b.cout, b.cin, 1);
                break;
            case DOWN: conv(b.prefix + ".op", b.cout, b.cin, 3); break;
            case UP:   conv(b.prefix + ".conv", b.cout, b.cin, 3); break;
            case ATTN:
                norm(b.prefix + ".norm", {b.cin});
                conv(b.prefix + ".qkv", 3 * b.cin, b.cin, 1, 1);
                conv(b.prefix + ".proj_out", b.cin, b.cin, 1, 1);
                break;
        }
    };
    for (auto& seq : plan.in_blocks) for (auto& b : seq) emit(b);
    for (auto& b : plan.middle) emit(b);
    for (auto& seq : plan.out_blocks) for (auto& b : seq) emit(b);
    norm("unet.out.0", {plan.out_sp, plan.out_sp, plan.out_sp});
    conv("unet.out.2", c.out_channels, c.model_channels, 3);
    return out;
}

struct Arena {
    static constexpr int64_t kAlign = 256;
    char* base = nullptr;
    int64_t capacity = 0, peak = 0;
    std::map<int64_t, int64_t> free_;
    std::map<int64_t, int64_t> used_;

    void reset(char* b, int64_t cap) {
        base = b; capacity = cap; peak = 0;
        free_.clear(); used_.clear();
        free_[0] = cap;
    }
    int64_t alloc(int64_t bytes) {
        bytes = (bytes + kAlign - 1) / kAlign * kAlign;
        if (bytes == 0) bytes = kAlign;
        for (auto it = free_.begin(); it != free_.end(); ++it) {
            if (it->second < bytes) continue;
            const int64_t off = it->first, rest = it->second - bytes;
            free_.erase(it);
            if (rest > 0) free_[off + bytes] = rest;
            used_[off] = bytes;
            if (off + bytes > peak) peak = off + bytes;
            return off;
        }
        fail("pixie_unet_forward: the workspace is too small (%lld bytes; ask pixie_unet_workspace_bytes for this grid size)", (long long)capacity);
    }
    void release(int64_t off) {
        auto u = used_.find(off);
        if (u == used_.end()) return;
        int64_t size = u->second;
        used_.erase(u);
        auto next = free_.lower_bound(off);
        if (next != free_.end() && off + size == next->first) { size += next->second; next = free_.erase(next); }
        if (next != free_.begin()) {
            auto prev = std::prev(next);
            if (prev->first + prev->second == off) { prev->second += size; return; }
        }
        free_[off] = size;
    }
    template <class T> T* ptr(int64_t off) const { return reinterpret_cast<T*>(base + off); }
};

struct Exec;
struct Tens {
    Exec* ex = nullptr;
    float* p = nullptr;
    int64_t off = -1;
    int c = 0, d = 0, h = 0, w = 0;
    int64_t sums_off = -1;
    bool has_sums = false;
    double* sums = nullptr;
    uint32_t* slot = nullptr;
    int64_t spatial() const { return (int64_t)d * h * w; }
    ~Tens();
};
using TP = std::shared_ptr<Tens>;

struct Packed { void* d = nullptr; uint64_t version = ~0ull; };
struct Sized { int64_t bytes; int slots; int64_t zsum_doubles; };
struct Bound { float wmax = 0, bmax = 0; uint64_t wver = ~0ull, bver = ~0ull; };

}
}

using namespace pixie;

struct pixie_unet {
    Cfg cfg;
    Plan plan;
    std::vector<Param> params;
    std::unordered_map<std::string, int> index;
    std::unordered_map<std::string, Packed> packed32, packed16;
    std::unordered_map<std::string, Bound> bounds;
    uint32_t* d_bound_slots = nullptr;
    std::vector<uint32_t> h_bound_slots;
    std::map<std::tuple<int, int, int, bool>, Sized> sized;
    bool fuse_stats = true, split_k = true, fold_skip = true;
    struct Replay { const float* feat; const float* proj0; float* out; void* ws; int d; uint64_t epoch; hipGraph_t graph; hipGraphExec_t exec; };
    bool use_graph = false;
    uint64_t epoch = 0;
    std::vector<Replay> replays;
    static constexpr size_t kMaxReplays = 4;
    void drop_replay(size_t i) {
        (void)hipGraphExecDestroy(replays[i].exec);
        (void)hipGraphDestroy(replays[i].graph);
        replays.erase(replays.begin() + (long)i);
    }

    const Param& param(const std::string& key) const {
        auto it = index.find(key);
        if (it == index.end()) fail("pixie_unet: no parameter named '%s'", key.c_str());
        return params[it->second];
    }
};

namespace pixie {
namespace {

struct Exec {
    pixie_unet* net = nullptr;
    Arena arena;
    bool dry = false;
    void* stream = nullptr;
    uint32_t* slots = nullptr;
    int slot_next = 0, slot_cap = 0;
    double* zsums = nullptr;
    int64_t zsum_next = 0, zsum_cap = 0;

    TP make(int c, int d, int h, int w) {
        auto t = std::make_shared<Tens>();
        t->ex = this; t->c = c; t->d = d; t->h = h; t->w = w;
        t->off = arena.alloc((int64_t)c * d * h * w * sizeof(float));
        t->p = arena.ptr<float>(t->off);
        return t;
    }
    TP external(const float* p, int c, int d, int h, int w) {
        auto t = std::make_shared<Tens>();
        t->ex = this; t->p = const_cast<float*>(p); t->c = c; t->d = d; t->h = h; t->w = w;
        return t;
    }
    uint32_t* new_slot() {
        if (!dry && slot_next >= slot_cap) fail("pixie_unet_forward: out of |x|max slots (internal sizing error)");
        return dry ? (slot_next++, nullptr) : slots + slot_next++;
    }
    struct Scratch {
        Exec* ex; int64_t off;
        Scratch(Exec* e, int64_t bytes) : ex(e), off(e->arena.alloc(bytes)) {}
        ~Scratch() { ex->arena.release(off); }
        template <class T> T* as() const { return ex->arena.ptr<T>(off); }
    };

    const float* P(const std::string& key) {
        const Param& p = net->param(key);
        if (!dry && !p.d) fail("pixie_unet_forward: parameter '%s' was never set", key.c_str());
        return p.d;
    }
    const void* w16(const std::string& key) {
        const Param& p = net->param(key + ".weight");
        if (dry) return nullptr;
        Packed& e = net->packed16[key];
        if (e.version != p.version) {
            const int cout = (int)p.shape[0], cin = (int)p.shape[1], k = (int)p.shape[2];
            const int64_t nb = pixie_conv_packed16_bytes(cout, cin, k);
            if (nb <= 0) fail("pixie_unet: '%s' cannot take the f16x3 packing (c_in %d)", key.c_str(), cin);
            if (!e.d && hipMalloc(&e.d, (size_t)nb) != hipSuccess) fail("pixie_unet: hipMalloc of %lld bytes failed", (long long)nb);
            if (!p.d) fail("pixie_unet_forward: parameter '%s.weight' was never set", key.c_str());
            ok(pixie_conv_pack_weights_f16x2(p.d, e.d, cout, cin, k, stream), "pixie_conv_pack_weights_f16x2");
            e.version = p.version;
        }
        return e.d;
    }
    const float* w32(const std::string& key) {
        const Param& p = net->param(key + ".weight");
        if (dry) return nullptr;
        Packed& e = net->packed32[key];
        if (e.version != p.version) {
            const int cout = (int)p.shape[0], cin = (int)p.shape[1], k = (int)p.shape[2];
            int64_t taps = 1;
            for (size_t i = 2; i < p.shape.size(); ++i) taps *= p.shape[i];
            const int64_t nb = taps * cin * pixie_conv_cout_padded(cout) * (int64_t)sizeof(float);
            if (!e.d && hipMalloc(&e.d, (size_t)nb) != hipSuccess) fail("pixie_unet: hipMalloc of %lld bytes failed", (long long)nb);
            if (!p.d) fail("pixie_unet_forward: parameter '%s.weight' was never set", key.c_str());
            ok(pixie_conv_pack_weights(p.d, static_cast<float*>(e.d), cout, cin, k, stream), "pixie_conv_pack_weights");
            e.version = p.version;
        }
        return static_cast<const float*>(e.d);
    }
    float norm_bound(const std::string& key, int64_t count) {
        if (dry) return 1.0f;
        const Bound& b = net->bounds[key];
        return (float)(std::sqrt((double)count) * (double)b.wmax + (double)b.bmax + 1e-30);
    }

    void stats(const TP& t) {
        if (t->has_sums) return;
        t->has_sums = true;
        if (!dry && zsum_next + 2 * t->c > zsum_cap) fail("pixie_unet_forward: out of statistics space (internal sizing error)");
        t->sums = dry ? nullptr : zsums + zsum_next;
        zsum_next += 2 * t->c;
        t->slot = new_slot();
        if (!dry) ok(channel_stats_prezeroed(t->p, t->c, t->spatial(), t->sums, t->slot, as_stream(stream)), "pixie_channel_stats");
    }
    struct AB { std::shared_ptr<Scratch> mem; float* a; float* b; };
    AB norm_finalize(const double* sums, int c, int64_t spatial, int mode, int groups, const float* w, const float* b) {
        AB r;
        const int cpad = (c + 63) / 64 * 64;
        r.mem = std::make_shared<Scratch>(this, (int64_t)(cpad + c) * sizeof(float));
        r.a = r.mem->as<float>();
        r.b = r.a + cpad;
        if (!dry) ok(pixie_norm_finalize(sums, c, spatial, mode, groups, 1e-5, w, b, r.a, r.b, stream), "pixie_norm_finalize");
        return r;
    }

    bool f16_ok(const std::vector<TP>& parts, int stride) const {
        int cin = 0;
        for (auto& t : parts) cin += t->c;
        return net->cfg.precision == 0 && (stride == 1 || stride == 2) && cin % 16 == 0 && parts[0]->c % 8 == 0;
    }
    bool skip_foldable(const TP& x, int cout, int ksize, const std::vector<TP>& sp) const {
        pixie_conv_desc d;
        std::memset(&d, 0, sizeof d);
        d.c0 = x->c; d.in_d = x->d; d.in_h = x->h; d.in_w = x->w;
        d.stride = 1; d.ksize = ksize; d.c_out = cout;
        d.d_w16 = reinterpret_cast<const void*>(0x100);
        d.d_workspace = net->split_k ? reinterpret_cast<void*>(0x100) : nullptr;
        d.skip_c0 = sp[0]->c; d.skip_c1 = sp.size() > 1 ? sp[1]->c : 0;
        return pixie_conv_skip_foldable(&d) != 0;
    }

    struct ConvOpt {
        int stride = 1; bool upsample = false;
        const AB* pro = nullptr; std::string affine_store;
        int act = ACT_NONE; TP residual; float bound = 0.0f;
        int out_d = 0, out_h = 0, out_w = 0;
        float* out_ptr = nullptr;
        const std::vector<TP>* skip_parts = nullptr; std::string skip_key;
    };
    TP conv(const std::vector<TP>& parts, const std::string& wkey, int cout, int ksize, const ConvOpt& o) {
        const TP& x0 = parts[0];
        const Tens* x1 = parts.size() > 1 ? parts[1].get() : nullptr;
        const int up = o.upsample ? 2 : 1, pad = ksize == 3 ? 1 : 0;
        int od = (x0->d * up + 2 * pad - ksize) / o.stride + 1;
        int oh = (x0->h * up + 2 * pad - ksize) / o.stride + 1;
        int ow = (x0->w * up + 2 * pad - ksize) / o.stride + 1;
        pixie_conv_desc desc;
        std::memset(&desc, 0, sizeof desc);
        if (o.out_d) {
            od = std::min(od, o.out_d); oh = std::min(oh, o.out_h); ow = std::min(ow, o.out_w);
            desc.out_d = od; desc.out_h = oh; desc.out_w = ow;
        }
        const bool f16 = f16_ok(parts, o.stride);
        const bool raw = !o.pro && o.affine_store.empty();
        if (f16 && raw) for (auto& t : parts) stats(t);

        TP out = o.out_ptr ? external(o.out_ptr, cout, od, oh, ow) : make(cout, od, oh, ow);
        desc.d_in0 = x0->p; desc.c0 = x0->c;
        desc.d_in1 = x1 ? x1->p : nullptr; desc.c1 = x1 ? x1->c : 0;
        desc.in_d = x0->d; desc.in_h = x0->h; desc.in_w = x0->w;
        desc.upsample = o.upsample ? 1 : 0;
        desc.stride = o.stride;
        desc.ksize = ksize;
        if (o.pro) { desc.d_pro_a = o.pro->a; desc.d_pro_b = o.pro->b; }
        if (!o.affine_store.empty()) { desc.d_gamma = P(o.affine_store + ".weight"); desc.d_beta = P(o.affine_store + ".bias"); }
        desc.act = o.act;
        desc.d_bias = P(wkey + ".bias");
        desc.c_out = cout;
        desc.d_residual = o.residual ? o.residual->p : nullptr;
        desc.d_out = out->p;
        if (!f16) {
            desc.d_w = w32(wkey);
            if (!dry) ok(pixie_conv3d_forward(&desc, stream), "pixie_conv3d_forward");
            return out;
        }
        desc.d_w16 = w16(wkey);
        if (o.skip_parts) {
            const std::vector<TP>& sp = *o.skip_parts;
            desc.d_skip_in0 = sp[0]->p; desc.skip_c0 = sp[0]->c;
            desc.d_skip_in1 = sp.size() > 1 ? sp[1]->p : nullptr; desc.skip_c1 = sp.size() > 1 ? sp[1]->c : 0;
            desc.d_skip_w16 = w16(o.skip_key);
            desc.d_skip_bias = P(o.skip_key + ".bias");
            desc.d_skip_amax0 = sp[0]->slot; desc.d_skip_amax1 = sp.size() > 1 ? sp[1]->slot : nullptr;
            if (dry) desc.d_skip_w16 = reinterpret_cast<const void*>(0x100);
        }
        if (raw) {
            desc.d_in_amax0 = parts[0]->slot;
            desc.d_in_amax1 = x1 ? parts[1]->slot : nullptr;
        } else {
            desc.in_bound = o.bound;
        }
        std::unique_ptr<Scratch> workspace, tile_stats;
        if (dry) { desc.d_w16 = reinterpret_cast<const void*>(0x100); }
        if (net->split_k) {
            const int64_t wsb = pixie_conv_workspace_bytes(&desc);
            if (wsb > 0) { workspace.reset(new Scratch(this, wsb)); desc.d_workspace = workspace->as<void>(); if (dry) desc.d_workspace = reinterpret_cast<void*>(0x100); }
        }
        bool have_stats = false;
        if (net->fuse_stats) {
            uint32_t* slot = new_slot();
            const int64_t nfl = pixie_conv_stats_floats(&desc);
            if (nfl > 0) {
                tile_stats.reset(new Scratch(this, nfl * (int64_t)sizeof(float)));
                desc.d_out_stats = tile_stats->as<float>();
                desc.d_out_amax = slot;
                have_stats = true;
                out->slot = slot;
            }
        }
        if (!dry) ok(pixie_conv3d_forward(&desc, stream), "pixie_conv3d_forward");
        if (have_stats) {
            out->sums_off = arena.alloc((int64_t)cout * 2 * sizeof(double));
            out->sums = arena.ptr<double>(out->sums_off);
            out->has_sums = true;
            if (!dry) ok(pixie_stats_finalize(desc.d_out_stats, &desc, out->sums, stream), "pixie_stats_finalize");
        }
        return out;
    }

    AB norm_finalize_parts(const std::vector<TP>& parts, int64_t spatial) {
        for (auto& t : parts) stats(t);
        if (parts.size() == 1) return norm_finalize(parts[0]->sums, parts[0]->c, spatial, 0, 1, nullptr, nullptr);
        const int c0 = parts[0]->c, c1 = parts[1]->c, c = c0 + c1;
        AB r;
        const int cpad = (c + 63) / 64 * 64;
        r.mem = std::make_shared<Scratch>(this, (int64_t)(cpad + c) * sizeof(float));
        r.a = r.mem->as<float>();
        r.b = r.a + cpad;
        if (!dry) ok(norm_finalize_cat(parts[0]->sums, c0, parts[1]->sums, c1, spatial, 0, 1, 1e-5, nullptr, nullptr, r.a, r.b, as_stream(stream)),
                     "pixie_norm_finalize");
        return r;
    }
    TP res(const Blk& b, const std::vector<TP>& parts) {
        const std::string& p = b.prefix;
        const int64_t spatial = parts[0]->spatial();
        AB pro = norm_finalize_parts(parts, spatial);
        ConvOpt o1; o1.pro = &pro; o1.affine_store = p + ".in_layers.0"; o1.act = ACT_LEAKY; o1.bound = norm_bound(p + ".in_layers.0", spatial);
        TP h = conv(parts, p + ".in_layers.2", b.cout, 3, o1);
        stats(h);
        AB pro2 = norm_finalize(h->sums, b.cout, spatial, 0, 1, nullptr, nullptr);
        TP skip = parts[0];
        ConvOpt o2; o2.pro = &pro2; o2.affine_store = p + ".out_layers.0"; o2.act = ACT_LEAKY; o2.bound = norm_bound(p + ".out_layers.0", spatial);
        if (b.cin != b.cout) {
            if (net->fold_skip && f16_ok({h}, 1) && f16_ok(parts, 1) && skip_foldable(h, b.cout, 3, parts)) {
                skip.reset();
                for (auto& t : parts) stats(t);
                o2.skip_parts = &parts; o2.skip_key = p + ".skip_connection";
            } else {
                skip = conv(parts, p + ".skip_connection", b.cout, 1, ConvOpt{});
            }
        }
        o2.residual = skip;
        return conv({h}, p + ".out_layers.3", b.cout, 3, o2);
    }
    TP attn(const Blk& b, const TP& x) {
        const std::string& p = b.prefix;
        const int c = x->c;
        const int64_t spatial = x->spatial();
        stats(x);
        AB pro = norm_finalize(x->sums, c, spatial, 1, 32, P(p + ".norm.weight"), P(p + ".norm.bias"));
        ConvOpt o; o.pro = &pro; o.bound = norm_bound(p + ".norm", spatial * (c / 32));
        TP qkv = conv({x}, p + ".qkv", 3 * c, 1, o);
        TP att = make(c, x->d, x->h, x->w);
        if (!dry) ok(pixie_attention_forward(qkv->p, att->p, c, (int)spatial, stream), "pixie_attention_forward");
        qkv.reset();
        ConvOpt o2; o2.residual = x;
        return conv({att}, p + ".proj_out", c, 1, o2);
    }
    TP block(const Blk& b, const std::vector<TP>& parts, const Tens* up_to) {
        if (b.kind == RES) return res(b, parts);
        const TP& x = parts[0];
        if (b.kind == ATTN) return attn(b, x);
        if (b.kind == DOWN) { ConvOpt o; o.stride = 2; return conv({x}, b.prefix + ".op", b.cout, 3, o); }
        if (b.kind == UP) {
            ConvOpt o; o.upsample = true;
            if (up_to) { o.out_d = up_to->d; o.out_h = up_to->h; o.out_w = up_to->w; }
            return conv({x}, b.prefix + ".conv", b.cout, 3, o);
        }
        fail("pixie_unet: unexpected block kind");
    }

    TP forward(const float* d_feat, const float* d_proj0, int D, int H, int W, float* d_out) {
        const Cfg& c = net->cfg;
        const int64_t spatial = (int64_t)D * H * W;
        TP x;
        AB pro_in; const AB* pro_in_p = nullptr;
        int act_in = ACT_NONE; float bound_in = 0.0f;
        if (c.has_projector()) {
            const std::string q = "projector.net.";
            const int hid = c.projector_hidden();
            if (!hid) {
                const int g = std::max(c.cond_dim / 2, 1);
                x = conv({external(d_feat, c.feature_channels, D, H, W)}, q + "0", c.cond_dim, 1, ConvOpt{});
                stats(x);
                pro_in = norm_finalize(x->sums, c.cond_dim, spatial, 1, g, P(q + "1.weight"), P(q + "1.bias"));
                act_in = ACT_SILU;
                bound_in = norm_bound(q + "1", spatial * (c.cond_dim / g));
            } else {
                if (d_proj0) x = external(d_proj0, hid, D, H, W);
                else x = conv({external(d_feat, c.feature_channels, D, H, W)}, q + "0", hid, 1, ConvOpt{});
                stats(x);
                AB pro = norm_finalize(x->sums, hid, spatial, 1, 32, P(q + "1.weight"), P(q + "1.bias"));
                ConvOpt o; o.pro = &pro; o.act = ACT_SILU; o.bound = norm_bound(q + "1", spatial * (hid / 32));
                x = conv({x}, q + "3", hid, 3, o);
                stats(x);
                AB pro2 = norm_finalize(x->sums, hid, spatial, 1, 32, P(q + "4.weight"), P(q + "4.bias"));
                ConvOpt o2; o2.pro = &pro2; o2.act = ACT_SILU; o2.bound = norm_bound(q + "4", spatial * (hid / 32));
                x = conv({x}, q + "6", c.cond_dim, 1, o2);
                stats(x);
                pro_in = norm_finalize(x->sums, c.cond_dim, spatial, 1, 32, P(q + "7.weight"), P(q + "7.bias"));
                bound_in = norm_bound(q + "7", spatial * std::max(c.cond_dim / 32, 1));
            }
            pro_in_p = &pro_in;
        } else {
            x = external(d_feat, c.feature_channels, D, H, W);
        }
        const Plan& plan = net->plan;
        std::vector<TP> hs;
        const Blk& first = plan.in_blocks[0][0];
        ConvOpt of; of.pro = pro_in_p; of.act = act_in; of.bound = bound_in;
        TP h = conv({x}, first.prefix, first.cout, 3, of);
        x.reset();
        pro_in = AB{};
        hs.push_back(h);
        for (size_t i = 1; i < plan.in_blocks.size(); ++i) {
            for (const Blk& b : plan.in_blocks[i]) h = block(b, {h}, nullptr);
            hs.push_back(h);
        }
        for (const Blk& b : plan.middle) h = block(b, {h}, nullptr);
        for (auto& seq : plan.out_blocks) {
            TP skip = hs.back(); hs.pop_back();
            if (skip->d != h->d || skip->h != h->h || skip->w != h->w) fail("pixie_unet_forward: skip tensor and decoder tensor differ in size");
            std::vector<TP> parts{h, skip};
            h.reset(); skip.reset();
            for (const Blk& b : seq) {
                TP nh = block(b, parts, (b.kind == UP && !hs.empty()) ? hs.back().get() : nullptr);
                parts.clear();
                parts.push_back(nh);
            }
            h = parts[0];
        }
        stats(h);
        AB pro = norm_finalize(h->sums, h->c, h->spatial(), 0, 1, nullptr, nullptr);
        ConvOpt oo; oo.pro = &pro; oo.affine_store = "unet.out.0"; oo.act = ACT_LEAKY; oo.bound = norm_bound("unet.out.0", h->spatial());
        oo.out_ptr = d_out;
        return conv({h}, "unet.out.2", c.out_channels, 3, oo);
    }
};

Tens::~Tens() {
    if (!ex) return;
    if (off >= 0) ex->arena.release(off);
    if (sums_off >= 0) ex->arena.release(sums_off);
}

void refresh_bounds(pixie_unet* net, void* stream) {
    std::vector<std::pair<std::string, int>> todo;
    int n_norm = 0;
    for (const Param& p : net->params) {
        if (!p.norm || p.key.size() < 7 || p.key.compare(p.key.size() - 7, 7, ".weight") != 0) continue;
        const std::string key = p.key.substr(0, p.key.size() - 7);
        const Param& pb = net->param(key + ".bias");
        Bound& b = net->bounds[key];
        if (b.wver != p.version || b.bver != pb.version) todo.push_back({key, 2 * n_norm});
        ++n_norm;
    }
    if (todo.empty()) return;
    const size_t bytes = (size_t)2 * n_norm * sizeof(uint32_t);
    if (!net->d_bound_slots && hipMalloc(&net->d_bound_slots, bytes) != hipSuccess) fail("pixie_unet: hipMalloc failed");
    net->h_bound_slots.assign((size_t)2 * n_norm, 0u);
    hipStream_t s = as_stream(stream);
    if (hipMemsetAsync(net->d_bound_slots, 0, bytes, s) != hipSuccess) fail("pixie_unet: hipMemsetAsync failed");
    for (auto& t : todo) {
        const Param& pw = net->param(t.first + ".weight");
        const Param& pb = net->param(t.first + ".bias");
        if (!pw.d || !pb.d) fail("pixie_unet_forward: parameter '%s' was never set", t.first.c_str());
        ok(pixie_tensor_amax(pw.d, pw.numel, net->d_bound_slots + t.second, stream), "pixie_tensor_amax");
        ok(pixie_tensor_amax(pb.d, pb.numel, net->d_bound_slots + t.second + 1, stream), "pixie_tensor_amax");
    }
    if (hipMemcpyAsync(net->h_bound_slots.data(), net->d_bound_slots, bytes, hipMemcpyDeviceToHost, s) != hipSuccess ||
        hipStreamSynchronize(s) != hipSuccess)
        fail("pixie_unet: reading the normalisation bounds back failed: %s", hipGetErrorString(hipGetLastError()));
    for (auto& t : todo) {
        Bound& b = net->bounds[t.first];
        std::memcpy(&b.wmax, &net->h_bound_slots[t.second], 4);
        std::memcpy(&b.bmax, &net->h_bound_slots[t.second + 1], 4);
        b.wver = net->param(t.first + ".weight").version;
        b.bver = net->param(t.first + ".bias").version;
    }
}

__global__ void zero_head_kernel(uint4* p, int64_t n16) {
    const int64_t i = (int64_t)blockIdx.x * 256 + threadIdx.x;
    if (i < n16) p[i] = make_uint4(0u, 0u, 0u, 0u);
}

constexpr int64_t kSlotAlign = 256;
int64_t slot_region_bytes(int n_slots) { return ((int64_t)n_slots * 4 + kSlotAlign - 1) / kSlotAlign * kSlotAlign; }
int64_t zsum_region_bytes(int64_t n_doubles) { return (n_doubles * 8 + kSlotAlign - 1) / kSlotAlign * kSlotAlign; }

Sized size_pass(pixie_unet* net, int D, int H, int W, bool from_proj0) {
    auto key = std::make_tuple(D, H, W, from_proj0);
    auto it = net->sized.find(key);
    if (it != net->sized.end()) return it->second;
    Exec ex;
    ex.net = net; ex.dry = true; ex.stream = nullptr;
    ex.arena.reset(reinterpret_cast<char*>(0x10000000), (int64_t)1 << 50);
    {
        const float* fake = reinterpret_cast<const float*>(0x100);
        TP out = ex.forward(from_proj0 ? nullptr : fake, from_proj0 ? fake : nullptr, D, H, W, reinterpret_cast<float*>(0x100));
    }
    Sized r{ex.arena.peak + slot_region_bytes(ex.slot_next) + zsum_region_bytes(ex.zsum_next), ex.slot_next, ex.zsum_next};
    net->sized[key] = r;
    return r;
}

template <class F> int guarded(F f) {
    try { return f(); }
    catch (const std::exception& e) { return set_error("%s", e.what()); }
}

}
}

extern "C" int pixie_unet_create(pixie_unet** out, const pixie_unet_config* c) {
    PX_REQUIRE(out && c, "pixie_unet_create: null argument");
    PX_REQUIRE(c->n_channel_mult >= 1 && c->n_channel_mult <= 8 && c->n_attention_resolutions >= 0 && c->n_attention_resolutions <= 8,
               "pixie_unet_create: channel_mult needs 1..8 entries, attention_resolutions 0..8");
    PX_REQUIRE(c->feature_channels > 0 && c->cond_dim > 0 && c->model_channels > 0 && c->num_res_blocks > 0 && c->grid_size > 0 && c->out_channels > 0,
               "pixie_unet_create: non-positive size");
    PX_REQUIRE(c->precision == 0 || c->precision == 1, "pixie_unet_create: precision is 0 (f16x3) or 1 (exact fp32)");
    return guarded([&] {
        std::unique_ptr<pixie_unet> n(new pixie_unet);
        n->cfg.feature_channels = c->feature_channels; n->cfg.cond_dim = c->cond_dim; n->cfg.model_channels = c->model_channels;
        n->cfg.num_res_blocks = c->num_res_blocks; n->cfg.grid_size = c->grid_size; n->cfg.out_channels = c->out_channels;
        n->cfg.precision = c->precision;
        n->cfg.mult.assign(c->channel_mult, c->channel_mult + c->n_channel_mult);
        n->cfg.attn.assign(c->attention_resolutions, c->attention_resolutions + c->n_attention_resolutions);
        n->plan = build_plan(n->cfg);
        n->params = param_table(n->cfg, n->plan);
        for (size_t i = 0; i < n->params.size(); ++i) n->index[n->params[i].key] = (int)i;
        const char* fs = getenv("PIXIE_FUSE_STATS"); n->fuse_stats = !(fs && fs[0] == '0');
        const char* sk = getenv("PIXIE_CONV_SPLIT_K"); n->split_k = !(sk && sk[0] == '0');
        const char* fk = getenv("PIXIE_FOLD_SKIP"); n->fold_skip = !(fk && fk[0] == '0');
        *out = n.release();
        return 0;
    });
}

extern "C" int pixie_unet_destroy(pixie_unet* h) {
    if (!h) return 0;
    for (auto& kv : h->packed16) if (kv.second.d) (void)hipFree(kv.second.d);
    for (auto& kv : h->packed32) if (kv.second.d) (void)hipFree(kv.second.d);
    if (h->d_bound_slots) (void)hipFree(h->d_bound_slots);
    while (!h->replays.empty()) h->drop_replay(0);
    delete h;
    return 0;
}

extern "C" int pixie_unet_param_count(const pixie_unet* h) { return h ? (int)h->params.size() : 0; }

extern "C" int pixie_unet_param_info(const pixie_unet* h, int i, const char** key, int64_t* numel, int32_t* ndim, int64_t shape[5]) {
    PX_REQUIRE(h && i >= 0 && i < (int)h->params.size(), "pixie_unet_param_info: index out of range");
    const Param& p = h->params[i];
    if (key) *key = p.key.c_str();
    if (numel) *numel = p.numel;
    if (ndim) *ndim = (int32_t)p.shape.size();
    if (shape) for (size_t k = 0; k < p.shape.size() && k < 5; ++k) shape[k] = p.shape[k];
    return 0;
}

extern "C" int pixie_unet_set_param(pixie_unet* h, const char* key, const float* d_values, int64_t numel) {
    PX_REQUIRE(h && key && d_values, "pixie_unet_set_param: null argument");
    auto it = h->index.find(key);
    PX_REQUIRE(it != h->index.end(), "pixie_unet_set_param: unexpected key '%s' (the reference's load_state_dict(strict=True) raises here too)", key);
    Param& p = h->params[it->second];
    PX_REQUIRE(numel == p.numel, "pixie_unet_set_param: '%s' has %lld elements, got %lld", key, (long long)p.numel, (long long)numel);
    p.d = d_values;
    ++p.version;
    ++h->epoch;
    return 0;
}

extern "C" int64_t pixie_unet_workspace_bytes(pixie_unet* h, int d, int hh, int w) {
    if (!h || d <= 0 || hh <= 0 || w <= 0) { set_error("pixie_unet_workspace_bytes: bad argument"); return -1; }
    int64_t bytes = -1;
    const int rc = guarded([&] {
        bytes = size_pass(h, d, hh, w, false).bytes;
        if (h->cfg.projector_hidden() > 0) bytes = std::max(bytes, size_pass(h, d, hh, w, true).bytes);
        return 0;
    });
    return rc == 0 ? bytes : -1;
}

extern "C" int pixie_unet_forward(pixie_unet* h, const float* d_feat, const float* d_proj0, int d, int hh, int w, float* d_out,
                                  void* d_workspace, int64_t workspace_bytes, void* stream) {
    PX_REQUIRE(h && d_out && d_workspace && (d_feat || d_proj0), "pixie_unet_forward: null argument");
    PX_REQUIRE(d == h->cfg.grid_size && hh == d && w == d,
               "pixie_unet_forward: the network was built for a %d^3 grid (its LayerNorm parameters have that shape), got %d x %d x %d", h->cfg.grid_size, d, hh, w);
    PX_REQUIRE(!d_proj0 || h->cfg.projector_hidden() > 0, "pixie_unet_forward: d_proj0 needs the hidden-128 projector (feature_channels > cond_dim)");
    PX_REQUIRE(d_feat || (d_proj0 && h->cfg.has_projector()), "pixie_unet_forward: d_feat is null");
    return guarded([&] {
        const auto sized = size_pass(h, d, hh, w, d_proj0 != nullptr);
        if (workspace_bytes < sized.bytes)
            fail("pixie_unet_forward: workspace of %lld bytes, this grid needs %lld (pixie_unet_workspace_bytes)", (long long)workspace_bytes, (long long)sized.bytes);
        auto launch_all = [&] {
            Exec ex;
            ex.net = h; ex.dry = false; ex.stream = stream;
            const int64_t slot_bytes = slot_region_bytes(sized.slots), head_bytes = slot_bytes + zsum_region_bytes(sized.zsum_doubles);
            ex.slots = static_cast<uint32_t*>(d_workspace);
            ex.slot_cap = sized.slots;
            ex.zsums = reinterpret_cast<double*>(static_cast<char*>(d_workspace) + slot_bytes);
            ex.zsum_cap = sized.zsum_doubles;
            hipLaunchKernelGGL(zero_head_kernel, dim3((unsigned)((head_bytes / 16 + 255) / 256)), dim3(256), 0, as_stream(stream),
                               static_cast<uint4*>(d_workspace), head_bytes / 16);
            if (hipGetLastError() != hipSuccess) fail("pixie_unet_forward: clearing the workspace head failed");
            ex.arena.reset(static_cast<char*>(d_workspace) + head_bytes, workspace_bytes - head_bytes);
            TP out = ex.forward(d_feat, d_proj0, d, hh, w, d_out);
        };
        if (h->use_graph) {
            for (size_t i = 0; i < h->replays.size(); ++i) {
                const pixie_unet::Replay& r = h->replays[i];
                if (r.feat != d_feat || r.proj0 != d_proj0 || r.out != d_out || r.ws != d_workspace || r.d != d) continue;
                if (r.epoch != h->epoch) { h->drop_replay(i); break; }
                if (hipGraphLaunch(r.exec, as_stream(stream)) != hipSuccess) fail("pixie_unet_forward: hipGraphLaunch failed: %s", hipGetErrorString(hipGetLastError()));
                if (i + 1 != h->replays.size()) std::rotate(h->replays.begin() + (long)i, h->replays.begin() + (long)i + 1, h->replays.end());
                return 0;
            }
        }
        if (h->use_graph && as_stream(stream) == nullptr)
            fail("pixie_unet_forward: option \"graph\" needs a non-default stream (the legacy stream cannot be captured); pass a created stream or set graph = 0");
        refresh_bounds(h, stream);
        launch_all();
        if (h->use_graph) {
            hipStream_t st = as_stream(stream);
            if (hipStreamBeginCapture(st, hipStreamCaptureModeThreadLocal) != hipSuccess)
                fail("pixie_unet_forward: cannot capture on this stream (graph replay needs a non-default stream): %s", hipGetErrorString(hipGetLastError()));
            hipGraph_t graph = nullptr;
            try { launch_all(); }
            catch (...) { (void)hipStreamEndCapture(st, &graph); if (graph) (void)hipGraphDestroy(graph); throw; }
            if (hipStreamEndCapture(st, &graph) != hipSuccess || !graph) fail("pixie_unet_forward: hipStreamEndCapture failed: %s", hipGetErrorString(hipGetLastError()));
            hipGraphExec_t exec = nullptr;
            if (hipGraphInstantiate(&exec, graph, nullptr, nullptr, 0) != hipSuccess) { (void)hipGraphDestroy(graph); fail("pixie_unet_forward: hipGraphInstantiate failed"); }
            if (h->replays.size() >= pixie_unet::kMaxReplays) h->drop_replay(0);
            h->replays.push_back(pixie_unet::Replay{d_feat, d_proj0, d_out, d_workspace, d, h->epoch, graph, exec});
        }
        return 0;
    });
}

extern "C" int pixie_unet_set_option(pixie_unet* h, const char* key, int value) {
    PX_REQUIRE(h && key, "pixie_unet_set_option: null argument");
    const std::string k(key);
    if (k == "graph") {
        h->use_graph = value != 0;
        if (!h->use_graph) while (!h->replays.empty()) h->drop_replay(0);
        return 0;
    }
    return set_error("pixie_unet_set_option: unknown key '%s' (known: graph)", key);
}
```

pixie_amd/unet.py:

```python
from __future__ import annotations

import ctypes as C
import math
import os
import warnings
import weakref
from typing import Dict, List, Optional, Sequence, Tuple

import torch
import torch.nn as nn

from . import _lib
from ._lib import ConvDesc, check
from .unet_plan import Block, UNetConfig, UNetPlan, build_plan, param_shapes, is_norm_key

ACT_NONE, ACT_LEAKY, ACT_SILU = 0, 1, 2
DEFAULT_PRECISION = os.environ.get("PIXIE_CONV_PRECISION", "f16x3")
_ZERO_INIT_SUFFIXES = (".out_layers.3.weight", ".out_layers.3.bias", ".proj_out.weight", ".proj_out.bias",
                       "unet.out.2.weight", "unet.out.2.bias")


def _ptr(t: Optional[torch.Tensor]):
    return C.c_void_p(t.data_ptr()) if t is not None else C.c_void_p(0)


class HipOps:

    def __init__(self, device: torch.device):
        if device.type != "cuda":
            raise _lib.PixieHipError("pixie_amd U-Net operators run on a HIP device only (no CPU fallback)")
        self.device = device
        self.lib = _lib.load()
        self.split_k = os.environ.get("PIXIE_CONV_SPLIT_K", "1") != "0"
        self.record_variant = False
        self.last_variant = (0, 1)

    @property
    def stream(self):
        return _lib.current_stream_ptr()

    def pack_conv(self, weight: torch.Tensor) -> torch.Tensor:
        cout, cin = weight.shape[0], weight.shape[1]
        k = weight.shape[2]
        coutp = self.lib.pixie_conv_cout_padded(cout)
        w = weight.detach().to(self.device, torch.float32).contiguous()
        taps = 1
        for s in weight.shape[2:]:
            taps *= int(s)
        packed = torch.empty((taps, cin, coutp), device=self.device, dtype=torch.float32)
        check(self.lib.pixie_conv_pack_weights(_ptr(w), _ptr(packed), cout, cin, k, self.stream), "pixie_conv_pack_weights")
        return packed

    def pack_conv16(self, weight: torch.Tensor) -> torch.Tensor:
        cout, cin, k = weight.shape[0], weight.shape[1], weight.shape[2]
        nbytes = self.lib.pixie_conv_packed16_bytes(cout, cin, k)
        if nbytes <= 0:
            raise _lib.PixieHipError(f"f16x3 packing needs c_in % 8 == 0 (got {cin})")
        w = weight.detach().to(self.device, torch.float32).contiguous()
        packed = torch.empty(nbytes, device=self.device, dtype=torch.uint8)
        check(self.lib.pixie_conv_pack_weights_f16x2(_ptr(w), _ptr(packed), cout, cin, k, self.stream), "pixie_conv_pack_weights_f16x2")
        return packed

    @staticmethod
    def f16x3_ok(parts: Sequence[torch.Tensor], stride: int) -> bool:
        cin = sum(int(p.shape[0]) for p in parts)
        return stride in (1, 2) and cin % 16 == 0 and int(parts[0].shape[0]) % 8 == 0

    def conv(self, parts: Sequence[torch.Tensor], packed_w: Optional[torch.Tensor], bias: Optional[torch.Tensor], cout: int, ksize: int,
             stride: int = 1, upsample: bool = False, pro: Optional[Tuple[torch.Tensor, torch.Tensor]] = None,
             affine: Optional[Tuple[torch.Tensor, torch.Tensor]] = None, act: int = ACT_NONE,
             residual: Optional[torch.Tensor] = None, w16: Optional[torch.Tensor] = None,
             in_amax: Optional[Sequence[torch.Tensor]] = None, in_bound: float = 0.0,
             out_amax: Optional[torch.Tensor] = None, out_size: Optional[Tuple[int, int, int]] = None,
             skip: Optional[dict] = None):
        x0 = parts[0]
        x1 = parts[1] if len(parts) > 1 else None
        cin0, d, h, w = x0.shape
        up = 2 if upsample else 1
        pad = 1 if ksize == 3 else 0
        od = (d * up + 2 * pad - ksize) // stride + 1
        oh = (h * up + 2 * pad - ksize) // stride + 1
        ow = (w * up + 2 * pad - ksize) // stride + 1
        desc = ConvDesc()
        if out_size is not None:
            od, oh, ow = min(od, int(out_size[0])), min(oh, int(out_size[1])), min(ow, int(out_size[2]))
            desc.out_d, desc.out_h, desc.out_w = od, oh, ow
        out = torch.empty((cout, od, oh, ow), device=self.device, dtype=torch.float32)
        desc.d_in0 = x0.data_ptr(); desc.c0 = cin0
        desc.d_in1 = x1.data_ptr() if x1 is not None else None
        desc.c1 = x1.shape[0] if x1 is not None else 0
        desc.in_d, desc.in_h, desc.in_w = d, h, w
        desc.upsample = 1 if upsample else 0
        desc.stride = stride
        desc.ksize = ksize
        desc.d_pro_a = pro[0].data_ptr() if pro is not None else None
        desc.d_pro_b = pro[1].data_ptr() if pro is not None else None
        desc.d_gamma = affine[0].data_ptr() if affine is not None else None
        desc.d_beta = affine[1].data_ptr() if affine is not None else None
        desc.act = act
        desc.d_w = packed_w.data_ptr() if packed_w is not None else None
        desc.d_w16 = w16.data_ptr() if w16 is not None else None
        desc.d_in_amax0 = in_amax[0].data_ptr() if in_amax else None
        desc.d_in_amax1 = in_amax[1].data_ptr() if in_amax and len(in_amax) > 1 else None
        desc.in_bound = float(in_bound)
        desc.d_bias = bias.data_ptr() if bias is not None else None
        desc.c_out = cout
        desc.d_residual = residual.data_ptr() if residual is not None else None
        desc.d_out = out.data_ptr()
        if skip is not None:
            sp = skip["parts"]
            desc.d_skip_in0 = sp[0].data_ptr(); desc.skip_c0 = sp[0].shape[0]
            desc.d_skip_in1 = sp[1].data_ptr() if len(sp) > 1 else None
            desc.skip_c1 = sp[1].shape[0] if len(sp) > 1 else 0
            desc.d_skip_w16 = skip["w16"].data_ptr()
            desc.d_skip_bias = skip["bias"].data_ptr() if skip["bias"] is not None else None
            desc.d_skip_amax0 = skip["amax"][0].data_ptr()
            desc.d_skip_amax1 = skip["amax"][1].data_ptr() if len(sp) > 1 else None
        sums = None
        if w16 is not None and self.split_k:
            wsb = self.lib.pixie_conv_workspace_bytes(C.byref(desc))
            if wsb > 0:
                workspace = torch.empty(wsb, device=self.device, dtype=torch.uint8)
                desc.d_workspace = workspace.data_ptr()
        if out_amax is not None and w16 is not None:
            nfl = self.lib.pixie_conv_stats_floats(C.byref(desc))
            if nfl > 0:
                stats = torch.empty(nfl, device=self.device, dtype=torch.float32)
                desc.d_out_stats = stats.data_ptr()
                desc.d_out_amax = out_amax.data_ptr()
        if self.record_variant:
            sl = C.c_int(1)
            self.last_variant = (int(_lib.load(diag=True).pixie_conv_kernel_variant(C.byref(desc), C.byref(sl))), int(sl.value))
        check(self.lib.pixie_conv3d_forward(C.byref(desc), self.stream), "pixie_conv3d_forward")
        if desc.d_out_stats:
            sums = torch.empty((cout, 2), device=self.device, dtype=torch.float64)
            check(self.lib.pixie_stats_finalize(_ptr(stats), C.byref(desc), _ptr(sums), self.stream), "pixie_stats_finalize")
        if out_amax is not None:
            return out, sums
        return out

    def skip_foldable(self, x: torch.Tensor, cout: int, ksize: int, skip_parts: Sequence[torch.Tensor]) -> bool:
        desc = ConvDesc()
        desc.c0 = x.shape[0]
        desc.in_d, desc.in_h, desc.in_w = (int(v) for v in x.shape[1:])
        desc.stride, desc.ksize, desc.c_out = 1, ksize, cout
        desc.d_w16 = 1
        desc.d_workspace = 1 if self.split_k else None
        desc.skip_c0 = skip_parts[0].shape[0]
        desc.skip_c1 = skip_parts[1].shape[0] if len(skip_parts) > 1 else 0
        return bool(self.lib.pixie_conv_skip_foldable(C.byref(desc)))

    def channel_sums(self, x: torch.Tensor) -> torch.Tensor:
        c = x.shape[0]
        spatial = x.numel() // c
        sums = torch.empty((c, 2), device=self.device, dtype=torch.float64)
        check(self.lib.pixie_channel_sums(_ptr(x), c, spatial, _ptr(sums), self.stream), "pixie_channel_sums")
        return sums

    def channel_stats(self, x: torch.Tensor, amax_slot: torch.Tensor) -> torch.Tensor:
        c = x.shape[0]
        spatial = x.numel() // c
        sums = torch.empty((c, 2), device=self.device, dtype=torch.float64)
        check(self.lib.pixie_channel_stats(_ptr(x), c, spatial, _ptr(sums), _ptr(amax_slot), self.stream), "pixie_channel_stats")
        return sums

    def norm_finalize(self, sums: torch.Tensor, spatial: int, mode: int, groups: int = 1, eps: float = 1e-5,
                      weight: Optional[torch.Tensor] = None, bias: Optional[torch.Tensor] = None):
        c = sums.shape[0]
        a = torch.empty(c, device=self.device, dtype=torch.float32)
        b = torch.empty(c, device=self.device, dtype=torch.float32)
        check(self.lib.pixie_norm_finalize(_ptr(sums), c, spatial, mode, groups, eps, _ptr(weight), _ptr(bias), _ptr(a), _ptr(b),
                                           self.stream), "pixie_norm_finalize")
        return a, b

    def attention(self, qkv: torch.Tensor, channels: int, tokens: int) -> torch.Tensor:
        out = torch.empty((channels, tokens), device=self.device, dtype=torch.float32)
        check(self.lib.pixie_attention_forward(_ptr(qkv), _ptr(out), channels, tokens, self.stream), "pixie_attention_forward")
        return out

    def projector_conv0(self, grid_dhwc_f16: torch.Tensor, nets: Sequence[Tuple[torch.Tensor, Optional[torch.Tensor]]], cout: int):
        d, h, w, c = (int(v) for v in grid_dhwc_f16.shape)
        g = grid_dhwc_f16.contiguous()
        outs = [torch.empty((cout, d, h, w), device=self.device, dtype=torch.float32) for _ in nets]
        n = len(nets)
        w_arr = (C.c_void_p * n)(*[t[0].data_ptr() for t in nets])
        b_arr = (C.c_void_p * n)(*[(t[1].data_ptr() if t[1] is not None else None) for t in nets])
        o_arr = (C.c_void_p * n)(*[o.data_ptr() for o in outs])
        check(self.lib.pixie_projector_conv0(_ptr(g), d * h * w, c, n, w_arr, b_arr, o_arr, cout, self.stream), "pixie_projector_conv0")
        return outs

    def combine(self, logits: torch.Tensor, cont: torch.Tensor):
        ncls = logits.shape[0]
        spatial = logits.numel() // ncls
        combined = torch.empty((3 + ncls,) + tuple(logits.shape[1:]), device=self.device, dtype=torch.float32)
        amax = torch.empty(tuple(logits.shape[1:]), device=self.device, dtype=torch.int32)
        check(self.lib.pixie_combine_predictions(_ptr(logits), ncls, _ptr(cont), spatial, _ptr(combined), _ptr(amax), self.stream),
              "pixie_combine_predictions")
        return combined, amax


class UNetRunner:

    def __init__(self, cfg: UNetConfig, params: Dict[str, torch.Tensor], ops, precision: Optional[str] = None):
        self.cfg = cfg
        self.plan: UNetPlan = build_plan(cfg)
        self.p = params
        self.ops = ops
        self.precision = precision or DEFAULT_PRECISION
        if self.precision not in ("f16x3", "f32"):
            raise ValueError(f"unknown conv precision {self.precision!r}")
        self._packed: Dict[str, Tuple[int, int, torch.Tensor]] = {}
        self._packed16: Dict[str, Tuple[int, int, torch.Tensor]] = {}
        self._bounds: Dict[str, Tuple[int, int, float, float]] = {}
        self.fuse_stats = os.environ.get("PIXIE_FUSE_STATS", "1") != "0"
        self.fold_skip = os.environ.get("PIXIE_FOLD_SKIP", "1") != "0"

    @property
    def _f16x3(self) -> bool:
        return self.precision == "f16x3" and hasattr(self.ops, "pack_conv16")

    def _w(self, key: str) -> torch.Tensor:
        t = self.p[key + ".weight"]
        ent = self._packed.get(key)
        if ent is None or ent[0] != t.data_ptr() or ent[1] != t._version:
            self._packed[key] = (t.data_ptr(), t._version, self.ops.pack_conv(t))
        return self._packed[key][2]

    def _w16(self, key: str) -> torch.Tensor:
        t = self.p[key + ".weight"]
        ent = self._packed16.get(key)
        if ent is None or ent[0] != t.data_ptr() or ent[1] != t._version:
            self._packed16[key] = (t.data_ptr(), t._version, self.ops.pack_conv16(t))
        return self._packed16[key][2]

    def _b(self, key: str) -> torch.Tensor:
        return self.p[key + ".bias"]

    def _absmax(self, key: str) -> Tuple[float, float]:
        w, bb = self.p[key + ".weight"], self.p[key + ".bias"]
        ent = self._bounds.get(key)
        if ent is None or ent[0] != w._version or ent[1] != bb._version:
            self._bounds[key] = (w._version, bb._version, float(w.abs().max()), float(bb.abs().max()))
            ent = self._bounds[key]
        return ent[2], ent[3]

    def _norm_bound(self, key: str, count: int) -> float:
        wmax, bmax = self._absmax(key)
        return math.sqrt(float(count)) * wmax + bmax + 1e-30

    _SLOT_POOL = 1024

    @classmethod
    def _new_slot(cls, cache: dict, device) -> torch.Tensor:
        pool = cache.get("_slots")
        if pool is None or cache["_next"] >= pool.numel():
            pool = cache["_slots"] = torch.zeros(cls._SLOT_POOL, dtype=torch.int32, device=device)
            cache["_next"] = 0
        i = cache["_next"]
        cache["_next"] = i + 1
        return pool[i:i + 1]

    @staticmethod
    def _remember(cache: dict, t: torch.Tensor, sums, slot) -> None:
        k = id(t)
        cache[k] = (sums, slot)
        weakref.finalize(t, cache.pop, k, None)

    def _stats(self, cache: dict, t: torch.Tensor):
        k = id(t)
        if k not in cache:
            if hasattr(self.ops, "channel_stats"):
                slot = self._new_slot(cache, t.device)
                self._remember(cache, t, self.ops.channel_stats(t, slot), slot)
            else:
                self._remember(cache, t, self.ops.channel_sums(t), None)
        return cache[k]

    def _sums(self, cache: dict, t: torch.Tensor) -> torch.Tensor:
        return self._stats(cache, t)[0]

    def _amax(self, cache: dict, t: torch.Tensor) -> torch.Tensor:
        return self._stats(cache, t)[1]

    def _conv(self, cache: dict, parts: List[torch.Tensor], wkey: str, cout: int, ksize: int, *, stride: int = 1,
              upsample: bool = False, pro=None, affine_key: Optional[str] = None, act: int = ACT_NONE,
              residual: Optional[torch.Tensor] = None, bound: float = 0.0, out_size=None, skip=None) -> torch.Tensor:
        ops = self.ops
        affine = (self.p[affine_key + ".weight"], self.p[affine_key + ".bias"]) if affine_key else None
        if not (self._f16x3 and ops.f16x3_ok(parts, stride)):
            return ops.conv(parts, self._w(wkey), self._b(wkey), cout, ksize, stride=stride, upsample=upsample, pro=pro,
                            affine=affine, act=act, residual=residual, **({"out_size": out_size} if out_size is not None else {}))
        if pro is None and affine is None:
            kw = dict(in_amax=[self._amax(cache, t) for t in parts])
        else:
            kw = dict(in_bound=bound)
        if out_size is not None:
            kw["out_size"] = out_size
        if skip is not None:
            kw["skip"] = skip
        if self.fuse_stats:
            slot = self._new_slot(cache, parts[0].device)
            out, sums = ops.conv(parts, None, self._b(wkey), cout, ksize, stride=stride, upsample=upsample, pro=pro, affine=affine,
                                 act=act, residual=residual, w16=self._w16(wkey), out_amax=slot, **kw)
            if sums is not None:
                self._remember(cache, out, sums, slot)
            return out
        return ops.conv(parts, None, self._b(wkey), cout, ksize, stride=stride, upsample=upsample, pro=pro, affine=affine,
                        act=act, residual=residual, w16=self._w16(wkey), **kw)

    def _res(self, b: Block, parts: List[torch.Tensor], cache: dict) -> torch.Tensor:
        ops, p = self.ops, b.prefix
        spatial = parts[0][0].numel()
        sums = torch.cat([self._sums(cache, t) for t in parts], dim=0) if len(parts) > 1 else self._sums(cache, parts[0])
        pro = ops.norm_finalize(sums, spatial, 0)
        h = self._conv(cache, parts, p + ".in_layers.2", b.cout, 3, pro=pro, affine_key=p + ".in_layers.0", act=ACT_LEAKY,
                       bound=self._norm_bound(p + ".in_layers.0", spatial))
        pro2 = ops.norm_finalize(self._sums(cache, h), spatial, 0)
        fold = None
        if b.cin != b.cout:
            if (self.fold_skip and self._f16x3 and ops.f16x3_ok([h], 1) and ops.f16x3_ok(parts, 1)
                    and ops.skip_foldable(h, b.cout, 3, parts)):
                skip = None
                fold = dict(parts=parts, w16=self._w16(p + ".skip_connection"), bias=self._b(p + ".skip_connection"),
                            amax=[self._amax(cache, t) for t in parts])
            else:
                skip = self._conv(cache, parts, p + ".skip_connection", b.cout, 1)
        else:
            skip = parts[0]
        return self._conv(cache, [h], p + ".out_layers.3", b.cout, 3, pro=pro2, affine_key=p + ".out_layers.0", act=ACT_LEAKY,
                          residual=skip, bound=self._norm_bound(p + ".out_layers.0", spatial), skip=fold)

    def _attn(self, b: Block, x: torch.Tensor, cache: dict) -> torch.Tensor:
        ops, p = self.ops, b.prefix
        c = x.shape[0]
        spatial = x[0].numel()
        pro = ops.norm_finalize(self._sums(cache, x), spatial, 1, groups=32, weight=self.p[p + ".norm.weight"],
                                bias=self.p[p + ".norm.bias"])
        qkv = self._conv(cache, [x], p + ".qkv", 3 * c, 1, pro=pro, bound=self._norm_bound(p + ".norm", spatial * (c // 32)))
        att = ops.attention(qkv.reshape(3 * c, spatial), c, spatial).reshape(x.shape)
        return self._conv(cache, [att], p + ".proj_out", c, 1, residual=x)

    def _block(self, b: Block, parts: List[torch.Tensor], cache: dict, up_size=None) -> torch.Tensor:
        if b.kind == "res":
            return self._res(b, parts, cache)
        assert len(parts) == 1
        x = parts[0]
        if b.kind == "attn":
            return self._attn(b, x, cache)
        if b.kind == "down":
            return self._conv(cache, [x], b.prefix + ".op", b.cout, 3, stride=2)
        if b.kind == "up":
            return self._conv(cache, [x], b.prefix + ".conv", b.cout, 3, upsample=True, out_size=up_size)
        raise ValueError(b.kind)

    def _stem(self, feat: Optional[torch.Tensor], cache: dict, proj0: Optional[torch.Tensor] = None) -> torch.Tensor:
        cfg, ops = self.cfg, self.ops
        spatial = (proj0 if proj0 is not None else feat)[0].numel()
        x = feat
        pro_in, act_in, bound_in = None, ACT_NONE, 0.0
        if cfg.has_projector:
            q = "projector.net."
            if cfg.projector_hidden is None:
                g = max(cfg.cond_dim // 2, 1)
                x = self._conv(cache, [x], q + "0", cfg.cond_dim, 1)
                pro_in = ops.norm_finalize(self._sums(cache, x), spatial, 1, groups=g,
                                           weight=self.p[q + "1.weight"], bias=self.p[q + "1.bias"])
                act_in = ACT_SILU
                bound_in = self._norm_bound(q + "1", spatial * (cfg.cond_dim // g))
            else:
                hid = cfg.projector_hidden
                x = proj0 if proj0 is not None else self._conv(cache, [x], q + "0", hid, 1)
                pro = ops.norm_finalize(self._sums(cache, x), spatial, 1, groups=32, weight=self.p[q + "1.weight"], bias=self.p[q + "1.bias"])
                x = self._conv(cache, [x], q + "3", hid, 3, pro=pro, act=ACT_SILU, bound=self._norm_bound(q + "1", spatial * (hid // 32)))
                pro = ops.norm_finalize(self._sums(cache, x), spatial, 1, groups=32, weight=self.p[q + "4.weight"], bias=self.p[q + "4.bias"])
                x = self._conv(cache, [x], q + "6", cfg.cond_dim, 1, pro=pro, act=ACT_SILU, bound=self._norm_bound(q + "4", spatial * (hid // 32)))
                pro_in = ops.norm_finalize(self._sums(cache, x), spatial, 1, groups=32, weight=self.p[q + "7.weight"], bias=self.p[q + "7.bias"])
                bound_in = self._norm_bound(q + "7", spatial * max(cfg.cond_dim // 32, 1))
        first = self.plan.input_blocks[0][0]
        return self._conv(cache, [x], first.prefix, first.cout, 3, pro=pro_in, act=act_in, bound=bound_in)

    def _head(self, h: torch.Tensor, cache: dict) -> torch.Tensor:
        pro = self.ops.norm_finalize(self._sums(cache, h), h[0].numel(), 0)
        return self._conv(cache, [h], "unet.out.2", self.cfg.out_channels, 3, pro=pro, affine_key="unet.out.0", act=ACT_LEAKY,
                          bound=self._norm_bound("unet.out.0", h[0].numel()))

    def forward(self, feat: Optional[torch.Tensor], taps: Optional[dict] = None, proj0: Optional[torch.Tensor] = None) -> torch.Tensor:
        cache: dict = {}
        only = set(taps) if taps else None

        def tap(key, t):
            if taps is not None and (only is None or key in only):
                taps[key] = t

        plan = self.plan
        hs: List[torch.Tensor] = []
        h = self._stem(feat, cache, proj0)
        hs.append(h)
        tap("unet.input_blocks.0", h)
        for seq in plan.input_blocks[1:]:
            for b in seq:
                h = self._block(b, [h], cache)
            hs.append(h)
            tap(seq[0].prefix.rsplit(".", 1)[0], h)
        for b in plan.middle:
            h = self._block(b, [h], cache)
            tap(b.prefix, h)
        for seq in plan.output_blocks:
            skip = hs.pop()
            assert tuple(skip.shape[1:]) == tuple(h.shape[1:]), (skip.shape, h.shape)
            parts = [h, skip]
            for b in seq:
                h = self._block(b, parts, cache, up_size=tuple(hs[-1].shape[1:]) if (b.kind == "up" and hs) else None)
                parts = [h]
            tap(seq[0].prefix.rsplit(".", 1)[0], h)
        return self._head(h, cache)


class UNetHandle:

    def __init__(self, cfg: UNetConfig, precision: str, device: torch.device):
        if device.type != "cuda":
            raise _lib.PixieHipError("pixie_amd U-Net runs on a HIP device only (no CPU fallback)")
        if precision not in ("f16x3", "f32"):
            raise ValueError(f"unknown conv precision {precision!r}")
        self.lib = _lib.load()
        self.cfg, self.precision, self.device = cfg, precision, device
        c = _lib.UNetConfigC()
        c.feature_channels, c.cond_dim, c.model_channels, c.num_res_blocks = cfg.feature_channels, cfg.cond_dim, cfg.model_channels, cfg.num_res_blocks
        c.n_channel_mult = len(cfg.channel_mult)
        for i, m in enumerate(cfg.channel_mult):
            c.channel_mult[i] = int(m)
        c.n_attention_resolutions = len(cfg.attention_resolutions)
        for i, m in enumerate(cfg.attention_resolutions):
            c.attention_resolutions[i] = int(m)
        c.grid_size, c.out_channels, c.precision = cfg.grid_size, cfg.out_channels, 0 if precision == "f16x3" else 1
        self._h = C.c_void_p()
        check(self.lib.pixie_unet_create(C.byref(self._h), C.byref(c)), "pixie_unet_create")
        weakref.finalize(self, self.lib.pixie_unet_destroy, self._h)
        self._seen: Dict[str, Tuple[int, int]] = {}
        self._keep: Dict[str, torch.Tensor] = {}

    def keys(self) -> List[str]:
        out = []
        for i in range(self.lib.pixie_unet_param_count(self._h)):
            key = C.c_char_p()
            check(self.lib.pixie_unet_param_info(self._h, i, C.byref(key), None, None, None), "pixie_unet_param_info")
            out.append(key.value.decode())
        return out

    def load(self, params: Dict[str, torch.Tensor]) -> None:
        for key, t in params.items():
            tag = (t.data_ptr(), t._version)
            if self._seen.get(key) == tag:
                continue
            v = t.detach()
            if v.device != self.device or v.dtype != torch.float32 or not v.is_contiguous():
                v = v.to(self.device, torch.float32).contiguous()
            self._keep[key] = v
            check(self.lib.pixie_unet_set_param(self._h, key.encode(), _ptr(v), v.numel()), "pixie_unet_set_param")
            self._seen[key] = tag

    def workspace_bytes(self, d: int, h: int, w: int) -> int:
        n = int(self.lib.pixie_unet_workspace_bytes(self._h, d, h, w))
        if n < 0:
            raise _lib.PixieHipError(self.lib.pixie_last_error().decode())
        return n

    def forward(self, feat: Optional[torch.Tensor], proj0: Optional[torch.Tensor] = None, workspace: Optional[torch.Tensor] = None) -> torch.Tensor:
        src = proj0 if proj0 is not None else feat
        d, h, w = (int(v) for v in src.shape[1:])
        out = torch.empty((self.cfg.out_channels, d, h, w), device=self.device, dtype=torch.float32)
        nbytes = self.workspace_bytes(d, h, w)
        if workspace is None:
            workspace = torch.empty(nbytes, device=self.device, dtype=torch.uint8)
        elif workspace.dtype != torch.uint8 or workspace.device != self.device or workspace.numel() < nbytes or not workspace.is_contiguous():
            raise ValueError(f"workspace must be a contiguous uint8 tensor of >= {nbytes} bytes on {self.device}")
        check(self.lib.pixie_unet_forward(self._h, _ptr(feat), _ptr(proj0), d, h, w, _ptr(out), _ptr(workspace), nbytes,
                                          _lib.current_stream_ptr()), "pixie_unet_forward")
        return out


class _Node(nn.Module):
    """Empty container used to reproduce the reference's state_dict key hierarchy."""


class _PixieUNet(nn.Module):
    def __init__(self, cfg: UNetConfig):
        super().__init__()
        self.cfg = cfg
        shapes = param_shapes(cfg)
        gen = torch.Generator().manual_seed(0)
        for key, shape in shapes.items():
            parts = key.split(".")
            node = self
            for name in parts[:-1]:
                if name not in node._modules:
                    node.add_module(name, _Node())
                node = node._modules[name]
            node.register_parameter(parts[-1], nn.Parameter(self._init(key, shape, shapes, gen), requires_grad=False))
        self._runner: Optional[UNetRunner] = None
        self._handle: Optional[UNetHandle] = None
        self.executor = os.environ.get("PIXIE_UNET_EXECUTOR", "c")
        self.conv_precision = DEFAULT_PRECISION
        self.use_graph = os.environ.get("PIXIE_UNET_GRAPH", "1") == "1"
        self._graphs: dict = {}
        self._plist = None

    @staticmethod
    def _init(key, shape, shapes, gen) -> torch.Tensor:
        if is_norm_key(key):
            return torch.ones(shape) if key.endswith(".weight") else torch.zeros(shape)
        if key.endswith(_ZERO_INIT_SUFFIXES):
            return torch.zeros(shape)
        wshape = shapes[key[: key.rfind(".")] + ".weight"]
        bound = 1.0 / math.sqrt(float(torch.tensor(wshape[1:]).prod()))
        return (torch.rand(shape, generator=gen) * 2.0 - 1.0) * bound

    def _params(self) -> Dict[str, torch.Tensor]:
        return {k: v for k, v in self.named_parameters()}

    def load_numpy_state(self, sd) -> None:
        self.load_state_dict({k: torch.from_numpy(v) for k, v in sd.items()}, strict=True)

    @torch.no_grad()
    def forward(self, feat_grid: torch.Tensor, taps: Optional[dict] = None) -> torch.Tensor:
        if feat_grid.dim() != 5 or feat_grid.shape[1] != self.cfg.feature_channels:
            raise ValueError(f"expected (N,{self.cfg.feature_channels},D,H,W), got {tuple(feat_grid.shape)}")
        dev = next(self.parameters()).device
        if dev.type != "cuda" or feat_grid.device != dev:
            raise _lib.PixieHipError("model and input must live on the same HIP device (no CPU fallback)")
        with torch.cuda.device(dev):
            self._prepare(dev)
            x = feat_grid.detach().to(torch.float32).contiguous()
            if self.use_graph and taps is None:
                return torch.stack([self._forward_graphed(x[n]) for n in range(x.shape[0])], dim=0)
            outs = [self._forward_one(x[n], taps=taps if n == 0 else None) for n in range(x.shape[0])]
            return torch.stack(outs, dim=0)

    def _prepare(self, dev) -> None:
        params = self._params()
        if self._runner is None or self._runner.ops.device != dev or self._runner.precision != self.conv_precision:
            self._runner = UNetRunner(self.cfg, params, HipOps(dev), precision=self.conv_precision)
        else:
            self._runner.p = params
        if self.executor == "c":
            if self._handle is None or self._handle.device != dev or self._handle.precision != self.conv_precision:
                self._handle = UNetHandle(self.cfg, self.conv_precision, dev)
            self._handle.load(params)
        elif self.executor != "python":
            raise ValueError(f"unknown executor {self.executor!r} (PIXIE_UNET_EXECUTOR is 'c' or 'python')")

    def _forward_one(self, x: Optional[torch.Tensor], taps: Optional[dict] = None, proj0: Optional[torch.Tensor] = None) -> torch.Tensor:
        if self.executor == "c" and taps is None:
            return self._handle.forward(x, proj0)
        return self._runner.forward(x, taps, proj0)

    def _apply(self, fn, *args, **kwargs):
        self._plist = None
        return super()._apply(fn, *args, **kwargs)

    def _param_list(self) -> List[torch.Tensor]:
        refs = self.__dict__.get("_plist")
        if refs is None:
            refs = self._plist = [(m._parameters, name) for m in self.modules() for name, p in m._parameters.items() if p is not None]
        return [d[name] for d, name in refs]

    def load_state_dict(self, state_dict, strict: bool = True, assign: bool = False):
        self._plist = None
        return super().load_state_dict(state_dict, strict=strict, assign=assign)

    def _forward_graphed(self, x: Optional[torch.Tensor], proj0: Optional[torch.Tensor] = None) -> torch.Tensor:
        src = proj0 if proj0 is not None else x
        base = (tuple(src.shape), tuple(src.stride()), src.dtype, proj0 is not None, self.executor, self.conv_precision, src.device.index,
                tuple((id(p), p.data_ptr(), p._version) for p in self._param_list()))
        run = (lambda t: self._forward_one(None, proj0=t)) if proj0 is not None else (lambda t: self._forward_one(t))
        if self._graphs.get("base") != base:
            self._graphs = {"base": base, "first_ptr": None}
        ent = self._graphs.get(src.data_ptr()) or self._graphs.get("copy")
        if ent is None:
            out = run(src)
            if self._graphs["first_ptr"] is None:
                self._graphs["first_ptr"] = src.data_ptr()
                return out
            in_place = (proj0 is None and self._graphs["first_ptr"] == src.data_ptr() and "copy" not in self._graphs
                        and os.environ.get("PIXIE_UNET_GRAPH_INPLACE", "1") == "1")
            try:
                static_in = src if in_place else src.clone()
                side = torch.cuda.Stream(src.device)
                side.wait_stream(torch.cuda.current_stream())
                with torch.cuda.stream(side):
                    run(static_in)
                torch.cuda.current_stream().wait_stream(side)
                graph = torch.cuda.CUDAGraph()
                with torch.cuda.graph(graph, capture_error_mode="thread_local"):
                    static_out = run(static_in)
            except RuntimeError as exc:
                warnings.warn(f"pixie_amd: HIP-graph capture of the U-Net forward failed ({exc}); continuing with eager launches",
                              RuntimeWarning)
                self.use_graph = False
                return out
            if in_place:
                ent = self._graphs[src.data_ptr()] = (graph, None, static_out)
            else:
                ent = self._graphs["copy"] = (graph, static_in, static_out)
        graph, static_in, static_out = ent
        if static_in is not None:
            static_in.copy_(src)
        graph.replay()
        return static_out.clone()


class SegmentationUNet(_PixieUNet):

    def __init__(self, feature_channels: int, cond_dim: int, model_channels: int, num_res_blocks: int,
                 channel_mult: Tuple[int, ...], attention_resolutions: Tuple[int, ...], grid_size: int, num_classes: int):
        super().__init__(UNetConfig(feature_channels, cond_dim, model_channels, num_res_blocks, tuple(channel_mult),
                                    tuple(attention_resolutions), grid_size, num_classes))


class RegressionUNet(_PixieUNet):

    def __init__(self, feature_channels: int, cond_dim: int, model_channels: int, num_res_blocks: int,
                 channel_mult: Tuple[int, ...], attention_resolutions: Tuple[int, ...], grid_size: int, out_channels: int = 3):
        super().__init__(UNetConfig(feature_channels, cond_dim, model_channels, num_res_blocks, tuple(channel_mult),
                                    tuple(attention_resolutions), grid_size, out_channels))


@torch.no_grad()
def predict_material_field_from_voxel_grid(seg_network: "SegmentationUNet", cont_network: "RegressionUNet", grid_dhwc_f16: torch.Tensor,
                                           dual_stream: Optional[bool] = None):
    dev = next(seg_network.parameters()).device
    g = grid_dhwc_f16
    if g.dim() != 4 or g.dtype != torch.float16 or g.device != dev or dev.type != "cuda":
        raise ValueError("expected a (D, H, W, C) float16 tensor on the networks' HIP device")
    nets = (seg_network, cont_network)
    for net in nets:
        if net.cfg.projector_hidden is None or net.cfg.feature_channels != g.shape[3] or net.conv_precision != "f16x3":
            raise ValueError("the fused grid path needs the hidden-128 projector, matching feature_channels and conv_precision 'f16x3'")
        net._prepare(dev)
    ops = seg_network._runner.ops
    q = "projector.net.0"
    packed = [(net._runner._w16(q), net._runner._b(q)) for net in nets]
    x_seg, x_cont = ops.projector_conv0(g, packed, seg_network.cfg.projector_hidden)
    if dual_stream is None:
        dual_stream = _dual_stream_default(seg_network, cont_network, int(g.shape[0]) * int(g.shape[1]) * int(g.shape[2]))

    def fwd(net, p0):
        return net._forward_graphed(None, p0) if net.use_graph else net._forward_one(None, proj0=p0)

    if dual_stream:
        cur = torch.cuda.current_stream()
        s1, s2 = _side_streams(dev)
        s1.wait_stream(cur); s2.wait_stream(cur)
        with torch.cuda.stream(s1):
            seg_logits = fwd(seg_network, x_seg)[None]
        with torch.cuda.stream(s2):
            cont_pred = fwd(cont_network, x_cont)[None]
        x_seg.record_stream(s1); x_cont.record_stream(s2)
        cur.wait_stream(s1); cur.wait_stream(s2)
        seg_logits.record_stream(cur); cont_pred.record_stream(cur)
    else:
        seg_logits = fwd(seg_network, x_seg)[None]
        cont_pred = fwd(cont_network, x_cont)[None]
    combined, seg_pred = ops.combine(seg_logits[0].contiguous(), cont_pred[0].contiguous())
    return combined[None], seg_pred[None], seg_logits, cont_pred


_SIDE_STREAMS: Dict[str, Tuple[torch.cuda.Stream, torch.cuda.Stream]] = {}


def _dual_stream_default(seg_network, cont_network, voxels: int) -> bool:
    env = os.environ.get("PIXIE_DUAL_STREAM")
    if env is not None:
        return env == "1"
    return not (seg_network.use_graph and cont_network.use_graph and voxels >= 128 ** 3)


def _side_streams(device):
    key = str(device)
    if key not in _SIDE_STREAMS:
        _SIDE_STREAMS[key] = (torch.cuda.Stream(device), torch.cuda.Stream(device))
    return _SIDE_STREAMS[key]


@torch.no_grad()
def predict_material_field(seg_network: SegmentationUNet, cont_network: RegressionUNet, feat_grid: torch.Tensor,
                           dual_stream: Optional[bool] = None):
    if feat_grid.is_cuda and feat_grid.device.index != torch.cuda.current_device():
        with torch.cuda.device(feat_grid.device):
            return predict_material_field(seg_network, cont_network, feat_grid, dual_stream)
    if dual_stream is None:
        dual_stream = _dual_stream_default(seg_network, cont_network, int(feat_grid[0, 0].numel()))
    if dual_stream and feat_grid.is_cuda:
        cur = torch.cuda.current_stream()
        s1, s2 = _side_streams(feat_grid.device)
        s1.wait_stream(cur); s2.wait_stream(cur)
        with torch.cuda.stream(s1):
            seg_logits = seg_network(feat_grid)
        with torch.cuda.stream(s2):
            cont_pred = cont_network(feat_grid)
        feat_grid.record_stream(s1); feat_grid.record_stream(s2)
        cur.wait_stream(s1); cur.wait_stream(s2)
        seg_logits.record_stream(cur); cont_pred.record_stream(cur)
    else:
        seg_logits = seg_network(feat_grid)
        cont_pred = cont_network(feat_grid)
    ops = seg_network._runner.ops
    combined, seg_pred = [], []
    for n in range(feat_grid.shape[0]):
        cmb, am = ops.combine(seg_logits[n].contiguous(), cont_pred[n].contiguous())
        combined.append(cmb)
        seg_pred.append(am)
    return torch.stack(combined), torch.stack(seg_pred), seg_logits, cont_pred
```

Measured before the change: 23.48 million voxels/s.

## Fold nearest-upsample into 3x3x3 conv via sub-pixel 2x2x2 weight decomposition

Adds a sub-pixel path for the conv that follows a 2x nearest upsample. Each output parity class becomes a 2x2x2 convolution on the low-resolution input, with per-parity summed weights packed into f16 hi/lo form. This cuts the MAC count per output from 27 taps to 8 and avoids reading the upsampled grid. It adds a new kernel variant, a weight-packing kernel, a new tiling and epilogue mapping, and a desc field. It risks extra rounding from summed weights and exposure to edge-case bugs.

```diff
diff --git a/include/pixie_hip.h b/include/pixie_hip.h
--- a/include/pixie_hip.h
+++ b/include/pixie_hip.h
@@ -117,12 +117,15 @@
     const float* d_skip_in1; int32_t skip_c1;
     const void* d_skip_w16; const float* d_skip_bias;
     const uint32_t* d_skip_amax0; const uint32_t* d_skip_amax1;
+    int32_t w16_subpixel;
 } pixie_conv_desc;
 
 int pixie_conv_cout_padded(int c_out);
 int pixie_conv_pack_weights(const float* d_w_oidhw, float* d_w_packed, int c_out, int c_in, int ksize, void* stream);
 int64_t pixie_conv_packed16_bytes(int c_out, int c_in, int ksize);
 int pixie_conv_pack_weights_f16x2(const float* d_w_oidhw, void* d_packed, int c_out, int c_in, int ksize, void* stream);
+int64_t pixie_conv_subpixel_bytes(int c_out, int c_in);
+int pixie_conv_pack_weights_subpixel(const float* d_w_oidhw, void* d_packed, int c_out, int c_in, void* stream);
 int pixie_conv3d_forward(const pixie_conv_desc* desc, void* stream);
 int64_t pixie_conv_stats_floats(const pixie_conv_desc* desc);
 int64_t pixie_conv_workspace_bytes(const pixie_conv_desc* desc);
diff --git a/pixie_amd/_lib.py b/pixie_amd/_lib.py
--- a/pixie_amd/_lib.py
+++ b/pixie_amd/_lib.py
@@ -47,7 +47,8 @@
                 ("d_skip_in0", C.c_void_p), ("skip_c0", C.c_int32),
                 ("d_skip_in1", C.c_void_p), ("skip_c1", C.c_int32),
                 ("d_skip_w16", C.c_void_p), ("d_skip_bias", C.c_void_p),
-                ("d_skip_amax0", C.c_void_p), ("d_skip_amax1", C.c_void_p)]
+                ("d_skip_amax0", C.c_void_p), ("d_skip_amax1", C.c_void_p),
+                ("w16_subpixel", C.c_int32)]
 
 
 class UNetConfigC(C.Structure):
@@ -112,6 +113,8 @@
     "pixie_conv_pack_weights": (_I, [_VP, _VP, _I, _I, _I, _VP]),
     "pixie_conv_packed16_bytes": (_I64, [_I, _I, _I]),
     "pixie_conv_pack_weights_f16x2": (_I, [_VP, _VP, _I, _I, _I, _VP]),
+    "pixie_conv_subpixel_bytes": (_I64, [_I, _I]),
+    "pixie_conv_pack_weights_subpixel": (_I, [_VP, _VP, _I, _I, _VP]),
     "pixie_conv3d_forward": (_I, [C.POINTER(ConvDesc), _VP]),
     "pixie_conv_stats_floats": (_I64, [C.POINTER(ConvDesc)]),
     "pixie_conv_workspace_bytes": (_I64, [C.POINTER(ConvDesc)]),
diff --git a/pixie_amd/csrc/conv3d_f16x3.hip b/pixie_amd/csrc/conv3d_f16x3.hip
--- a/pixie_amd/csrc/conv3d_f16x3.hip
+++ b/pixie_amd/csrc/conv3d_f16x3.hip
@@ -62,8 +62,9 @@
 }
 __device__ __forceinline__ float pow2i(int e) { return __uint_as_float((unsigned)(e + 127) << 23); }
 
-template <int KS, int MB, int NB, bool EX = false>
+template <int KS, int MB, int NB, bool EX = false, bool SP = false>
 __device__ __forceinline__ void conv3d_f16x3_body(const Conv16Args& A) {
+    static_assert(!SP || (KS == 3 && NB == 4 && !EX), "sub-pixel path: 3^3, two x parities x two voxel blocks per wave");
     extern __shared__ uint4 smem16[];
     constexpr int PAD = (KS == 3) ? 1 : 0;
     constexpr int NW = 4, NT = 64 * NW;
@@ -81,12 +82,17 @@
         const int cand = (t & 7) * per + (t >> 3);
         if ((A.n_tiles & 7) == 0) t = cand;
     }
+    int par = 0;
+    if constexpr (SP) { par = t & 3; t >>= 2; }
+    const int py = par & 1, pz = par >> 1;
     const int tx = t % A.tiles_x; t /= A.tiles_x;
     const int ty = t % A.tiles_y;
     const int tz = t / A.tiles_y;
     const int ox0 = tx * A.TX, oy0 = ty * A.TY, oz0 = tz * A.TZ;
     const int cout0 = blockIdx.y * (MB * 32);
-    const int lx0 = ox0 * A.stride - PAD, ly0 = oy0 * A.stride - PAD, lz0 = oz0 * A.stride - PAD;
+    const int lx0 = SP ? ox0 - 1 : ox0 * A.stride - PAD;
+    const int ly0 = SP ? oy0 - 1 + py : oy0 * A.stride - PAD;
+    const int lz0 = SP ? oz0 - 1 + pz : oz0 * A.stride - PAD;
     const size_t ISP = (size_t)A.ID * A.IH * A.IW;
     const size_t OSP = (size_t)A.OD * A.OH * A.OW;
 
@@ -95,6 +101,20 @@
     bool valid[NB];
 #pragma unroll
     for (int nb = 0; nb < NB; ++nb) {
+        if constexpr (SP) {
+            const int px = nb >> 1;
+            const int j = (wave * 2 + (nb & 1)) * 32 + l31;
+            int x = j & (A.TX - 1);
+            int y = (j >> A.lTX) & (A.TY - 1);
+            int z = j >> (A.lTX + A.lTY);
+            const int gx = 2 * (ox0 + x) + px, gy = 2 * (oy0 + y) + py, gz = 2 * (oz0 + z) + pz;
+            const bool v = (z < A.TZ) && (gx < A.OW) && (gy < A.OH) && (gz < A.OD);
+            if (!v) { x = 0; y = 0; z = 0; }
+            voff[nb] = (z * A.HY + y) * A.HX + x + px + kh * A.CS;
+            ovox[nb] = v ? (gz * A.OH + gy) * A.OW + gx : 0;
+            valid[nb] = v;
+            continue;
+        }
         const int j = (wave * NB + nb) * 32 + l31;
         int x = j & (A.TX - 1);
         int y = (j >> A.lTX) & (A.TY - 1);
@@ -124,8 +144,8 @@
 
     const int KG = A.cin >> 3;
     const size_t tap_stride = (size_t)KG * A.coutp;
-    const size_t plane = (size_t)(KS * KS * KS) * tap_stride;
-    const uint4* wHi = A.w16 + kW16HeaderU4 + (size_t)kh * A.coutp + cout0 + l31;
+    const size_t plane = (size_t)(SP ? 64 : KS * KS * KS) * tap_stride;
+    const uint4* wHi = A.w16 + kW16HeaderU4 + (size_t)kh * A.coutp + cout0 + l31 + (size_t)(par * 16) * tap_stride;
     const uint4* wLo = wHi + plane;
     const float* wF = A.wf + (size_t)kh * A.coutp + cout0 + l31;
 
@@ -267,6 +287,56 @@
         const uint4* ldsLo = buf + 2 * A.CS;
         const uint4* wh = wHi + (size_t)(c_base >> 3) * A.coutp;
         const uint4* wl = wLo + (size_t)(c_base >> 3) * A.coutp;
+        if constexpr (SP) {
+            f16x8 ah[MB], al[MB];
+#pragma unroll
+            for (int mb = 0; mb < MB; ++mb) {
+                ah[mb] = __builtin_bit_cast(f16x8, wh[mb * 32]);
+                al[mb] = __builtin_bit_cast(f16x8, wl[mb * 32]);
+            }
+#pragma unroll 1
+            for (int zy = 0; zy < 4; ++zy) {
+                const int rowoff = ((zy >> 1) * A.HY + (zy & 1)) * A.HX;
+                const int zyn = zy < 3 ? zy + 1 : 3;
+#pragma unroll
+                for (int q = 0; q < 4; ++q) {
+                    const int ex = q >> 1, px = q & 1;
+                    const size_t nxt = (q < 3) ? (size_t)(((q + 1) & 1) * 8 + zy * 2 + ((q + 1) >> 1)) * tap_stride : (size_t)(zyn * 2) * tap_stride;
+                    f16x8 ahn[MB], aln[MB];
+#pragma unroll
+                    for (int mb = 0; mb < MB; ++mb) {
+                        ahn[mb] = __builtin_bit_cast(f16x8, wh[nxt + mb * 32]);
+                        aln[mb] = __builtin_bit_cast(f16x8, wl[nxt + mb * 32]);
+                    }
+                    __builtin_amdgcn_sched_barrier(0);
+                    f16x8 bh[2], bl[2];
+#pragma unroll
+                    for (int s = 0; s < 2; ++s) {
+                        bh[s] = __builtin_bit_cast(f16x8, ldsHi[voff[px * 2 + s] + rowoff + ex]);
+                        bl[s] = __builtin_bit_cast(f16x8, ldsLo[voff[px * 2 + s] + rowoff + ex]);
+                    }
+#pragma unroll
+                    for (int mb = 0; mb < MB; ++mb)
+#pragma unroll
+                        for (int s = 0; s < 2; ++s)
+                            acc[mb][px * 2 + s] = __builtin_amdgcn_mfma_f32_32x32x16_f16(al[mb], bh[s], acc[mb][px * 2 + s], 0, 0, 0);
+#pragma unroll
+                    for (int mb = 0; mb < MB; ++mb)
+#pragma unroll
+                        for (int s = 0; s < 2; ++s)
+                            acc[mb][px * 2 + s] = __builtin_amdgcn_mfma_f32_32x32x16_f16(ah[mb], bl[s], acc[mb][px * 2 + s], 0, 0, 0);
+#pragma unroll
+                    for (int mb = 0; mb < MB; ++mb)
+#pragma unroll
+                        for (int s = 0; s < 2; ++s)
+                            acc[mb][px * 2 + s] = __builtin_amdgcn_mfma_f32_32x32x16_f16(ah[mb], bh[s], acc[mb][px * 2 + s], 0, 0, 0);
+#pragma unroll
+                    for (int mb = 0; mb < MB; ++mb) { ah[mb] = ahn[mb]; al[mb] = aln[mb]; }
+                }
+            }
+            __builtin_amdgcn_s_setprio(0);
+            return;
+        }
         f16x8 ah[MB], al[MB];
 #pragma unroll
         for (int mb = 0; mb < MB; ++mb) {
@@ -326,7 +396,7 @@
             __syncthreads();
             mfma_chunk(c_base, smem16);
         }
-        if (!EX && A.sk_w16) {
+        if (!EX && !SP && A.sk_w16) {
             float sb = __uint_as_float(*A.sk_amax0);
             if (A.sk_amax1) sb = fmaxf(sb, __uint_as_float(*A.sk_amax1));
             const int ex2 = scale_exponent(sb);
@@ -424,8 +494,10 @@
     }
     float* red = reinterpret_cast<float*>(smem16);
     float wmax = 0.0f;
-    const bool full = A.epi_lds && cout0 + MB * 32 <= A.cout && (A.TX & 3) == 0 && (A.OW & 3) == 0 && NW * NB * 32 <= A.TX * A.TY * A.TZ &&
-                      ox0 + A.TX <= A.OW && oy0 + A.TY <= A.OH && oz0 + A.TZ <= A.OD;
+    const bool full = SP ? (A.epi_lds && cout0 + MB * 32 <= A.cout && (A.TX & 1) == 0 && (A.OW & 3) == 0 && NW * 64 <= A.TX * A.TY * A.TZ &&
+                            2 * (ox0 + A.TX) <= A.OW && 2 * (oy0 + A.TY) <= A.OH && 2 * (oz0 + A.TZ) <= A.OD)
+                         : (A.epi_lds && cout0 + MB * 32 <= A.cout && (A.TX & 3) == 0 && (A.OW & 3) == 0 && NW * NB * 32 <= A.TX * A.TY * A.TZ &&
+                            ox0 + A.TX <= A.OW && oy0 + A.TY <= A.OH && oz0 + A.TZ <= A.OD);
     if (full) {
         __syncthreads();
         constexpr int LDO = NB * 32 + 4;
@@ -434,16 +506,18 @@
         constexpr int LPR = NB * 8;
         constexpr int RPI = 32 / LPR;
         const int rsub = l31 / LPR, colq = 4 * (l31 % LPR), nbq = colq >> 5;
-        const int jq = (wave * NB + nbq) * 32 + (colq & 31);
+        const int jq = SP ? wave * 64 + (colq >> 1) : (wave * NB + nbq) * 32 + (colq & 31);
         const int xq = jq & (A.TX - 1), yq = (jq >> A.lTX) & (A.TY - 1), zq = jq >> (A.lTX + A.lTY);
-        const size_t ovq = ((size_t)(oz0 + zq) * A.OH + (oy0 + yq)) * A.OW + ox0 + xq;
+        const size_t ovq = SP ? ((size_t)(2 * (oz0 + zq) + pz) * A.OH + (2 * (oy0 + yq) + py)) * A.OW + 2 * (ox0 + xq)
+                              : ((size_t)(oz0 + zq) * A.OH + (oy0 + yq)) * A.OW + ox0 + xq;
         const bool has_res = A.residual != nullptr, has_stats = A.stats != nullptr;
 #pragma unroll
         for (int mb = 0; mb < MB; ++mb) {
 #pragma unroll
             for (int r = 0; r < 16; ++r)
 #pragma unroll
-                for (int nb = 0; nb < NB; ++nb) ldsO[((r & 3) + 8 * (r >> 2) + 4 * kh) * LDO + nb * 32 + l31] = acc[mb][nb][r];
+                for (int nb = 0; nb < NB; ++nb)
+                    ldsO[((r & 3) + 8 * (r >> 2) + 4 * kh) * LDO + (SP ? 2 * ((nb & 1) * 32 + l31) + (nb >> 1) : nb * 32 + l31)] = acc[mb][nb][r];
 #pragma unroll 4
             for (int it = 0; it < 16 / RPI; ++it) {
                 const int rowl = (2 * it + kh) * RPI + rsub;
@@ -521,6 +595,10 @@
 template <int KS, int MB, int NB>
 __global__ __launch_bounds__(256, 2) void conv3d_exact_kernel(Conv16Args A) {
     conv3d_f16x3_body<KS, MB, NB, true>(A);
+}
+template <int MB>
+__global__ __launch_bounds__(256, 2) void conv3d_f16x3_subpixel_kernel(Conv16Args A) {
+    conv3d_f16x3_body<3, MB, 4, false, true>(A);
 }
 __global__ __launch_bounds__(256, 2) void conv3d_f16x3_c64_fullres_kernel(Conv16Args A) {
     conv3d_f16x3_body<3, 2, 4>(A);
@@ -594,9 +672,70 @@
     dst[kW16HeaderU4 + total + i] = __builtin_bit_cast(uint4, vl);
 }
 
+__device__ __forceinline__ float subpixel_weight(const float* __restrict__ w27, int par, int tap) {
+    int lo[3], hi[3];
+#pragma unroll
+    for (int ax = 0; ax < 3; ++ax) {
+        const int p = (par >> (2 - ax)) & 1, e = (tap >> (2 - ax)) & 1;
+        lo[ax] = e ? (p ? 2 : 1) : 0;
+        hi[ax] = e ? 2 : (p ? 1 : 0);
+    }
+    float sum = 0.0f;
+    for (int dz = lo[0]; dz <= hi[0]; ++dz)
+        for (int dy = lo[1]; dy <= hi[1]; ++dy)
+            for (int dx = lo[2]; dx <= hi[2]; ++dx) sum += w27[(dz * 3 + dy) * 3 + dx];
+    return sum;
+}
+__global__ __launch_bounds__(256) void subpixel_amax_kernel(const float* __restrict__ src, long pairs, unsigned* __restrict__ slot) {
+    const long i = (long)blockIdx.x * 256 + threadIdx.x;
+    float m = 0.0f;
+    if (i < pairs)
+        for (int pt = 0; pt < 64; ++pt) m = fmaxf(m, fabsf(subpixel_weight(src + i * 27, pt >> 3, pt & 7)));
+    for (int off = 32; off > 0; off >>= 1) m = fmaxf(m, __shfl_down(m, off, 64));
+    if ((threadIdx.x & 63) == 0 && m > 0.0f) atomicMax(slot, __float_as_uint(m));
+}
+__global__ void pack_weights_subpixel_kernel(const float* __restrict__ src, uint4* __restrict__ dst, int cout, int cin, int coutp,
+                                             const unsigned* __restrict__ amax_bits) {
+    const int KG = cin >> 3;
+    const long total = 64L * KG * coutp;
+    const long i = (long)blockIdx.x * blockDim.x + threadIdx.x;
+    const int e = scale_exponent(__uint_as_float(*amax_bits));
+    if (i == 0) dst[0] = make_uint4(__float_as_uint(pow2i(-e)), (unsigned)cout, (unsigned)cin, 64u);
+    if (i >= total) return;
+    const float s = pow2i(e);
+    const int co = (int)(i % coutp);
+    const long row = i / coutp;
+    const int kg = (int)(row % KG);
+    const int pt = (int)(row / KG);
+    f16x8 vh, vl;
+#pragma unroll
+    for (int j = 0; j < 8; ++j) {
+        float w = 0.0f;
+        if (co < cout) w = subpixel_weight(src + ((long)co * cin + kg * 8 + j) * 27, pt >> 3, pt & 7) * s;
+        const _Float16 h = (_Float16)w;
+        vh[j] = h;
+        vl[j] = (_Float16)(w - (float)h);
+    }
+    dst[kW16HeaderU4 + i] = __builtin_bit_cast(uint4, vh);
+    dst[kW16HeaderU4 + total + i] = __builtin_bit_cast(uint4, vl);
+}
+
 static unsigned magic_of16(int d) { return d <= 1 ? 0u : (unsigned)((0x100000000ull + (unsigned long long)d - 1) / (unsigned long long)d); }
 static int ilog2_16(int v) { int l = 0; while ((1 << l) < v) ++l; return l; }
 static int pow2_le16(int v, int cap) { int p = 1; while (p * 2 <= v && p * 2 <= cap) p *= 2; return p; }
+
+template <int MB>
+static int launch_subpixel(const Conv16Args& a, size_t lds_bytes, dim3 grid, hipStream_t st) {
+    auto kern = conv3d_f16x3_subpixel_kernel<MB>;
+    PX_CHECK_HIP(allow_max_dynamic_lds(reinterpret_cast<const void*>(kern)));
+    hipLaunchKernelGGL(kern, grid, dim3(256), lds_bytes, st, a);
+    PX_CHECK_HIP(hipGetLastError());
+    return 0;
+}
+
+static bool conv16_subpixel(const pixie_conv_desc* d) {
+    return d->d_w16 && d->w16_subpixel && d->upsample == 1 && d->ksize == 3 && d->stride == 1;
+}
 
 template <int KS, int MB, int NB>
 static int launch_f16x3(const Conv16Args& a, size_t lds_bytes, dim3 grid, hipStream_t st) {
@@ -618,6 +757,27 @@
     if (d->out_h > 0) a.OH = std::min(a.OH, (int)d->out_h);
     if (d->out_w > 0) a.OW = std::min(a.OW, (int)d->out_w);
     a.cout = d->c_out; a.coutp = pixie_conv_cout_padded(d->c_out);
+    const int chunks = (d->c0 + d->c1) / 16;
+    const int smax = d->d_workspace ? std::min(8, chunks / 2) : 1;
+    if (conv16_subpixel(d)) {
+        a.ups = 0; a.LD = a.ID; a.LH = a.IH; a.LW = a.IW;
+        const int SD = (a.OD + 1) / 2, SH = (a.OH + 1) / 2, SW = (a.OW + 1) / 2;
+        a.TX = pow2_le16(SW, 32);
+        a.TY = pow2_le16(SH, std::max(1, std::min(4, 256 / a.TX)));
+        a.TZ = std::max(1, std::min(SD, 256 / (a.TX * a.TY)));
+        a.lTX = ilog2_16(a.TX); a.lTY = ilog2_16(a.TY);
+        a.tiles_x = (SW + a.TX - 1) / a.TX; a.tiles_y = (SH + a.TY - 1) / a.TY; a.tiles_z = (SD + a.TZ - 1) / a.TZ;
+        a.n_tiles = 4 * a.tiles_x * a.tiles_y * a.tiles_z;
+        a.HX = a.TX + 2; a.HY = a.TY + 1; a.HZ = a.TZ + 1;
+        a.HYX = a.HY * a.HX; a.CS = a.HZ * a.HYX;
+        a.mHX = magic_of16(a.HX); a.mHYX = magic_of16(a.HYX);
+        MB_out = (a.coutp >= 64) ? 2 : 1; NB_out = 4;
+        int sl = 1;
+        const long wgs = (long)a.n_tiles * ((a.coutp + MB_out * 32 - 1) / (MB_out * 32));
+        while (sl * 2 <= smax && wgs * sl < 512) sl *= 2;
+        if (slices_out) *slices_out = sl;
+        return;
+    }
     const long ovol = (long)a.OD * a.OH * a.OW;
     int MB = (a.coutp >= 64) ? 2 : 1;
     int NB = (a.stride == 2) ? 1 : 4;
@@ -626,8 +786,6 @@
         return tiles * ((a.coutp + mb * 32 - 1) / (mb * 32));
     };
     int slices = 1;
-    const int chunks = (d->c0 + d->c1) / 16;
-    const int smax = d->d_workspace ? std::min(8, chunks / 2) : 1;
     if (smax >= 2 && n_wg(MB, NB) < 512) {
         bool found = false;
         for (int nb = NB; nb >= 1 && !found; nb /= 2) {
@@ -678,6 +836,8 @@
     a.stats = d->d_out_stats; a.out_amax = d->d_out_amax;
 
     int MB = 0, NB = 0, slices = 1;
+    const bool sp = d->w16_subpixel != 0;
+    PX_REQUIRE(!sp || (conv16_subpixel(d) && !d->d_skip_w16), "f16x3 conv: sub-pixel weights need upsample = 1, ksize = 3, stride = 1 and no folded skip");
     conv16_tiling(d, a, MB, NB, &slices);
     if (d->d_skip_w16) {
         const int scin = d->skip_c0 + d->skip_c1;
@@ -702,11 +862,15 @@
     const dim3 grid((unsigned)a.n_tiles, (unsigned)((a.coutp + MB * 32 - 1) / (MB * 32)), (unsigned)slices);
     if (slices > 1) {
         int rc = 1;
+        if (sp) {
+            rc = (MB == 2) ? launch_subpixel<2>(a, lds, grid, st) : launch_subpixel<1>(a, lds, grid, st);
+        } else {
 #define PX_CONV16_SK(KS_, MB_, NB_) \
-        if (d->ksize == KS_ && MB == MB_ && NB == NB_) rc = launch_f16x3<KS_, MB_, NB_>(a, lds, grid, st);
-        PX_CONV16_SK(3, 2, 4) PX_CONV16_SK(3, 2, 2) PX_CONV16_SK(3, 2, 1) PX_CONV16_SK(3, 1, 4) PX_CONV16_SK(3, 1, 2) PX_CONV16_SK(3, 1, 1)
-        PX_CONV16_SK(1, 2, 4) PX_CONV16_SK(1, 2, 2) PX_CONV16_SK(1, 2, 1) PX_CONV16_SK(1, 1, 4) PX_CONV16_SK(1, 1, 2) PX_CONV16_SK(1, 1, 1)
+            if (d->ksize == KS_ && MB == MB_ && NB == NB_) rc = launch_f16x3<KS_, MB_, NB_>(a, lds, grid, st);
+            PX_CONV16_SK(3, 2, 4) PX_CONV16_SK(3, 2, 2) PX_CONV16_SK(3, 2, 1) PX_CONV16_SK(3, 1, 4) PX_CONV16_SK(3, 1, 2) PX_CONV16_SK(3, 1, 1)
+            PX_CONV16_SK(1, 2, 4) PX_CONV16_SK(1, 2, 2) PX_CONV16_SK(1, 2, 1) PX_CONV16_SK(1, 1, 4) PX_CONV16_SK(1, 1, 2) PX_CONV16_SK(1, 1, 1)
 #undef PX_CONV16_SK
+        }
         if (rc) return rc;
         const long osp = (long)a.OD * a.OH * a.OW, n_elems = (long)a.cout * osp;
         hipLaunchKernelGGL(splitk_reduce_kernel, dim3((unsigned)((n_elems + 255) / 256)), dim3(256), 0, st, a.partial, slices, n_elems, osp,
@@ -714,6 +878,7 @@
         PX_CHECK_HIP(hipGetLastError());
         return 0;
     }
+    if (sp) return (MB == 2) ? launch_subpixel<2>(a, lds, grid, st) : launch_subpixel<1>(a, lds, grid, st);
     if (d->ksize == 3 && MB == 2 && NB == 4 && cin == 64 && d->c_out == 64 && d->stride == 1 && !d->upsample && d->c1 == 0 && !a.sk_w16 &&
         (long)a.OD * a.OH * a.OW >= 128L * 128 * 128) {
         auto kern = conv3d_f16x3_c64_fullres_kernel;
@@ -804,6 +969,7 @@
     int MB = 0, NB = 0, slices = 1;
     conv16_tiling(d, a, MB, NB, &slices);
     if (slices_out) *slices_out = slices;
+    if (conv16_subpixel(d)) return 8300 + MB * 10 + NB;
     if (d->ksize == 3 && MB == 2 && NB == 4 && d->c0 + d->c1 == 64 && d->c_out == 64 && d->stride == 1 && !d->upsample && d->c1 == 0 && !d->d_skip_w16 &&
         (long)a.OD * a.OH * a.OW >= 128L * 128 * 128)
         return 9324;
@@ -860,3 +1026,25 @@
     PX_CHECK_HIP(hipGetLastError());
     return 0;
 }
+
+extern "C" int64_t pixie_conv_subpixel_bytes(int c_out, int c_in) {
+    if (c_out <= 0 || c_in <= 0 || c_in % 16 != 0) return 0;
+    return ((int64_t)kW16HeaderU4 + 2 * 64 * (int64_t)(c_in / 8) * pixie_conv_cout_padded(c_out)) * (int64_t)sizeof(uint4);
+}
+
+extern "C" int pixie_conv_pack_weights_subpixel(const float* d_w, void* d_packed, int c_out, int c_in, void* stream) {
+    PX_REQUIRE(d_w && d_packed && c_out > 0 && c_in > 0 && c_in % 16 == 0,
+               "pixie_conv_pack_weights_subpixel: bad arguments (c_in must be a multiple of 16)");
+    hipStream_t st = as_stream(stream);
+    const int coutp = pixie_conv_cout_padded(c_out);
+    unsigned* slot = reinterpret_cast<unsigned*>(d_packed) + 15;
+    PX_CHECK_HIP(hipMemsetAsync(d_packed, 0, kW16HeaderU4 * sizeof(uint4), st));
+    const long pairs = (long)c_out * c_in;
+    hipLaunchKernelGGL(subpixel_amax_kernel, dim3(cdiv(pairs, 256)), dim3(256), 0, st, d_w, pairs, slot);
+    PX_CHECK_HIP(hipGetLastError());
+    const long total = 64L * (c_in / 8) * coutp;
+    hipLaunchKernelGGL(pack_weights_subpixel_kernel, dim3(cdiv(total, 256)), dim3(256), 0, st, d_w, reinterpret_cast<uint4*>(d_packed), c_out,
+                       c_in, coutp, slot);
+    PX_CHECK_HIP(hipGetLastError());
+    return 0;
+}
diff --git a/pixie_amd/csrc/conv3d_mfma.hip b/pixie_amd/csrc/conv3d_mfma.hip
--- a/pixie_amd/csrc/conv3d_mfma.hip
+++ b/pixie_amd/csrc/conv3d_mfma.hip
@@ -225,7 +225,8 @@
     PX_REQUIRE(d->c_out > 0 && d->in_d > 0 && d->in_h > 0 && d->in_w > 0, "pixie_conv3d_forward: bad sizes");
     PX_REQUIRE((d->d_pro_a == nullptr) == (d->d_pro_b == nullptr), "pixie_conv3d_forward: pro_a/pro_b must come together");
     PX_REQUIRE((d->d_gamma == nullptr) == (d->d_beta == nullptr), "pixie_conv3d_forward: gamma/beta must come together");
-    PX_REQUIRE(!(d->d_gamma && d->upsample), "pixie_conv3d_forward: spatial affine with upsample is not in the reference graph");
+    PX_REQUIRE(!(d->d_gamma && d->upsample) || (d->d_w16 && d->w16_subpixel),
+               "pixie_conv3d_forward: spatial affine with upsample needs the sub-pixel path (w16_subpixel), with gamma/beta of the stored grid");
 
     if (d->d_w16) return conv3d_f16x3_forward(d, as_stream(stream));
     PX_REQUIRE(!d->d_skip_w16, "pixie_conv3d_forward: a folded skip convolution needs the f16x3 path (d_w16)");
diff --git a/pixie_amd/csrc/unet_exec.hip b/pixie_amd/csrc/unet_exec.hip
--- a/pixie_amd/csrc/unet_exec.hip
+++ b/pixie_amd/csrc/unet_exec.hip
@@ -240,7 +240,7 @@
     uint32_t* d_bound_slots = nullptr;
     std::vector<uint32_t> h_bound_slots;
     std::map<std::tuple<int, int, int, bool>, Sized> sized;
-    bool fuse_stats = true, split_k = true, fold_skip = true;
+    bool fuse_stats = true, split_k = true, fold_skip = true, subpixel = true;
     struct Replay { const float* feat; const float* proj0; float* out; void* ws; int d; uint64_t epoch; hipGraph_t graph; hipGraphExec_t exec; };
     bool use_graph = false;
     uint64_t epoch = 0;
@@ -300,17 +300,18 @@
         if (!dry && !p.d) fail("pixie_unet_forward: parameter '%s' was never set", key.c_str());
         return p.d;
     }
-    const void* w16(const std::string& key) {
+    const void* w16(const std::string& key, bool subpixel = false) {
         const Param& p = net->param(key + ".weight");
         if (dry) return nullptr;
-        Packed& e = net->packed16[key];
+        Packed& e = net->packed16[subpixel ? key + "#subpixel" : key];
         if (e.version != p.version) {
             const int cout = (int)p.shape[0], cin = (int)p.shape[1], k = (int)p.shape[2];
-            const int64_t nb = pixie_conv_packed16_bytes(cout, cin, k);
+            const int64_t nb = subpixel ? (k == 3 ? pixie_conv_subpixel_bytes(cout, cin) : 0) : pixie_conv_packed16_bytes(cout, cin, k);
             if (nb <= 0) fail("pixie_unet: '%s' cannot take the f16x3 packing (c_in %d)", key.c_str(), cin);
             if (!e.d && hipMalloc(&e.d, (size_t)nb) != hipSuccess) fail("pixie_unet: hipMalloc of %lld bytes failed", (long long)nb);
             if (!p.d) fail("pixie_unet_forward: parameter '%s.weight' was never set", key.c_str());
-            ok(pixie_conv_pack_weights_f16x2(p.d, e.d, cout, cin, k, stream), "pixie_conv_pack_weights_f16x2");
+            if (subpixel) ok(pixie_conv_pack_weights_subpixel(p.d, e.d, cout, cin, stream), "pixie_conv_pack_weights_subpixel");
+            else ok(pixie_conv_pack_weights_f16x2(p.d, e.d, cout, cin, k, stream), "pixie_conv_pack_weights_f16x2");
             e.version = p.version;
         }
         return e.d;
@@ -417,7 +418,9 @@
             if (!dry) ok(pixie_conv3d_forward(&desc, stream), "pixie_conv3d_forward");
             return out;
         }
-        desc.d_w16 = w16(wkey);
+        const bool sub = net->subpixel && o.upsample && ksize == 3 && o.stride == 1;
+        desc.d_w16 = w16(wkey, sub);
+        desc.w16_subpixel = sub ? 1 : 0;
         if (o.skip_parts) {
             const std::vector<TP>& sp = *o.skip_parts;
             desc.d_skip_in0 = sp[0]->p; desc.skip_c0 = sp[0]->c;
@@ -686,6 +689,7 @@
         const char* fs = getenv("PIXIE_FUSE_STATS"); n->fuse_stats = !(fs && fs[0] == '0');
         const char* sk = getenv("PIXIE_CONV_SPLIT_K"); n->split_k = !(sk && sk[0] == '0');
         const char* fk = getenv("PIXIE_FOLD_SKIP"); n->fold_skip = !(fk && fk[0] == '0');
+        const char* sx = getenv("PIXIE_CONV_SUBPIXEL"); n->subpixel = !(sx && sx[0] == '0');
         *out = n.release();
         return 0;
     });
diff --git a/pixie_amd/unet.py b/pixie_amd/unet.py
--- a/pixie_amd/unet.py
+++ b/pixie_amd/unet.py
@@ -61,6 +61,16 @@
         check(self.lib.pixie_conv_pack_weights_f16x2(_ptr(w), _ptr(packed), cout, cin, k, self.stream), "pixie_conv_pack_weights_f16x2")
         return packed
 
+    def pack_conv_subpixel(self, weight: torch.Tensor) -> torch.Tensor:
+        cout, cin = weight.shape[0], weight.shape[1]
+        nbytes = self.lib.pixie_conv_subpixel_bytes(cout, cin) if tuple(weight.shape[2:]) == (3, 3, 3) else 0
+        if nbytes <= 0:
+            raise _lib.PixieHipError(f"sub-pixel packing needs a 3x3x3 weight with c_in % 16 == 0 (got {tuple(weight.shape)})")
+        w = weight.detach().to(self.device, torch.float32).contiguous()
+        packed = torch.empty(nbytes, device=self.device, dtype=torch.uint8)
+        check(self.lib.pixie_conv_pack_weights_subpixel(_ptr(w), _ptr(packed), cout, cin, self.stream), "pixie_conv_pack_weights_subpixel")
+        return packed
+
     @staticmethod
     def f16x3_ok(parts: Sequence[torch.Tensor], stride: int) -> bool:
         cin = sum(int(p.shape[0]) for p in parts)
@@ -72,7 +82,7 @@
              residual: Optional[torch.Tensor] = None, w16: Optional[torch.Tensor] = None,
              in_amax: Optional[Sequence[torch.Tensor]] = None, in_bound: float = 0.0,
              out_amax: Optional[torch.Tensor] = None, out_size: Optional[Tuple[int, int, int]] = None,
-             skip: Optional[dict] = None):
+             skip: Optional[dict] = None, subpixel: bool = False):
         x0 = parts[0]
         x1 = parts[1] if len(parts) > 1 else None
         cin0, d, h, w = x0.shape
@@ -100,6 +110,7 @@
         desc.act = act
         desc.d_w = packed_w.data_ptr() if packed_w is not None else None
         desc.d_w16 = w16.data_ptr() if w16 is not None else None
+        desc.w16_subpixel = 1 if subpixel else 0
         desc.d_in_amax0 = in_amax[0].data_ptr() if in_amax else None
         desc.d_in_amax1 = in_amax[1].data_ptr() if in_amax and len(in_amax) > 1 else None
         desc.in_bound = float(in_bound)
@@ -214,6 +225,7 @@
         self._bounds: Dict[str, Tuple[int, int, float, float]] = {}
         self.fuse_stats = os.environ.get("PIXIE_FUSE_STATS", "1") != "0"
         self.fold_skip = os.environ.get("PIXIE_FOLD_SKIP", "1") != "0"
+        self.subpixel = os.environ.get("PIXIE_CONV_SUBPIXEL", "1") != "0"
 
     @property
     def _f16x3(self) -> bool:
@@ -226,12 +238,13 @@
             self._packed[key] = (t.data_ptr(), t._version, self.ops.pack_conv(t))
         return self._packed[key][2]
 
-    def _w16(self, key: str) -> torch.Tensor:
+    def _w16(self, key: str, subpixel: bool = False) -> torch.Tensor:
         t = self.p[key + ".weight"]
-        ent = self._packed16.get(key)
+        ck = key + "#subpixel" if subpixel else key
+        ent = self._packed16.get(ck)
         if ent is None or ent[0] != t.data_ptr() or ent[1] != t._version:
-            self._packed16[key] = (t.data_ptr(), t._version, self.ops.pack_conv16(t))
-        return self._packed16[key][2]
+            self._packed16[ck] = (t.data_ptr(), t._version, self.ops.pack_conv_subpixel(t) if subpixel else self.ops.pack_conv16(t))
+        return self._packed16[ck][2]
 
     def _b(self, key: str) -> torch.Tensor:
         return self.p[key + ".bias"]
@@ -298,15 +311,18 @@
             kw["out_size"] = out_size
         if skip is not None:
             kw["skip"] = skip
+        sub = self.subpixel and upsample and ksize == 3 and stride == 1 and hasattr(ops, "pack_conv_subpixel")
+        if sub:
+            kw["subpixel"] = True
         if self.fuse_stats:
             slot = self._new_slot(cache, parts[0].device)
             out, sums = ops.conv(parts, None, self._b(wkey), cout, ksize, stride=stride, upsample=upsample, pro=pro, affine=affine,
-                                 act=act, residual=residual, w16=self._w16(wkey), out_amax=slot, **kw)
+                                 act=act, residual=residual, w16=self._w16(wkey, sub), out_amax=slot, **kw)
             if sums is not None:
                 self._remember(cache, out, sums, slot)
             return out
         return ops.conv(parts, None, self._b(wkey), cout, ksize, stride=stride, upsample=upsample, pro=pro, affine=affine,
-                        act=act, residual=residual, w16=self._w16(wkey), **kw)
+                        act=act, residual=residual, w16=self._w16(wkey, sub), **kw)
 
     def _res(self, b: Block, parts: List[torch.Tensor], cache: dict) -> torch.Tensor:
         ops, p = self.ops, b.prefix
```

Result: faster. 24.13 million voxels/s, median of 6 (+2.8%).
